# rbesenczi/newMSM

Hardware: AMD Instinct MI355X
Metric: label-cost evals/sec (higher is better)
Workload: dtype f64; 1 GPU; pairwise sulc (D=1) unary label-cost table, ico6 data grid / ico4 control grid, 19 labels, 48678 evals = 3187573 point samples per step (BASELINE config 2); kind=univariate, simmeasure=correlation, replicas=1

## Files before the change

### include/msmhip.h

```cpp
#ifndef MSMHIP_H
#define MSMHIP_H

#include <stddef.h>
#include <stdint.h>

#ifdef __cplusplus
extern "C" {
#endif

#define MSM_ABI_VERSION 11

#define MSM_OK 0
#define MSM_ERR_INVALID (-1)
#define MSM_ERR_HIP (-2)
#define MSM_ERR_OUTSIDE (-3)
#define MSM_ERR_NOTFOUND (-4)
#define MSM_ERR_NOGPU (-5)
#define MSM_ERR_STATE (-6)
#define MSM_ERR_CAPACITY (-7)
#define MSM_ERR_ROTATION (-8)

#define MSM_RAD 100.0
#define MSM_FOLDING 1e7

typedef struct msm_ctx msm_ctx;
typedef struct msm_mesh msm_mesh;
typedef struct msm_cost msm_cost;

int         msm_abi_version(void);
const char *msm_last_error(void);
int         msm_device_count(void);

int msm_icosphere_counts(int order, int32_t *V, int32_t *T);
int msm_icosphere(int order, double radius, double *xyz, int32_t *tri);
int msm_mesh_adjacency(const int32_t *tri, int32_t V, int32_t T, int32_t *nbr_ptr, int32_t *nbr, int32_t *tid_ptr, int32_t *tid);
int msm_vertex_areas(const double *xyz, const int32_t *tri, int32_t V, int32_t T, double *area);
int msm_resample_anatomy_grid(const double *cp_xyz, int32_t N, const int32_t *cp_tri, int32_t Tc, int32_t levels, double rad, int32_t *Va, int32_t *Ta,
                              double *axyz, int32_t *atri, int32_t *w_ptr, int32_t *w_cp, double *w_val, int32_t *face_ptr, int32_t *face_idx);
int msm_cp_spacings(const double *xyz, const int32_t *tri, int32_t V, int32_t T, double *maxsep, double *mvdmax);
int msm_label_sampling_grid(int sg_order, double max_dist, int abs_is_int, int32_t cap,
                            double *samples, int32_t *nsamples, double *barycentres, int32_t *nbarycentres);
int msm_rescale_sampling_grid(const double *samples, int32_t n, double *scale, double *labels);
int msm_rotation_matrix(const double ci[3], const double index[3], double R[9]);
int msm_cp_rotations(const double centre[3], const double *cp_xyz, int32_t N, double *rot);
int msm_estimate_triplets(const int32_t *tri, int32_t T, int32_t *triplets);
int msm_estimate_pairs(const int32_t *tri, int32_t V, int32_t T, int32_t *pairs);
int msm_octree_signature(const double *xyz, const int32_t *tri, int32_t V, int32_t T, int64_t stats[5], uint64_t *signature);
int msm_ray_table_check(const double *xyz, const int32_t *tri, int32_t V, int32_t T, int32_t nsamples, uint64_t seed, int64_t report[10]);

msm_ctx *msm_ctx_create(int device);
msm_ctx *msm_ctx_create_on_stream(int device, void *hip_stream);
void     msm_ctx_destroy(msm_ctx *ctx);
int      msm_ctx_synchronize(msm_ctx *ctx);
void    *msm_ctx_stream(msm_ctx *ctx);
void     msm_store_release_i64(int64_t *addr, int64_t value);
int64_t  msm_load_acquire_i64(const int64_t *addr);
int64_t  msm_min_acquire_i64(const int64_t *addr, int32_t n);
int      msm_ctx_wait_stream(msm_ctx *ctx, void *hip_stream);
int      msm_ctx_staging_stats(msm_ctx *ctx, int64_t out[4]);
int      msm_ctx_time_queries(msm_ctx *ctx, int enable);
int      msm_ctx_query_kernel_ms(msm_ctx *ctx, double *ms);
int      msm_query_lanes(int64_t n_queries);
void    *msm_host_alloc(msm_ctx *ctx, size_t bytes);
void     msm_host_free(msm_ctx *ctx, void *p);
int      msm_host_register(msm_ctx *ctx, void *p, size_t bytes);

msm_mesh *msm_mesh_create(msm_ctx *ctx, const double *xyz, int32_t V, const int32_t *tri, int32_t T);
void      msm_mesh_destroy(msm_mesh *m);
int       msm_mesh_update_coords(msm_mesh *m, const double *xyz);
int       msm_mesh_get_coords(msm_mesh *m, double *xyz);
int       msm_mesh_set_features(msm_mesh *m, const double *feat, int32_t D);
int       msm_mesh_sizes(const msm_mesh *m, int32_t *V, int32_t *T, int32_t *D);
int       msm_mesh_octree_stats(msm_mesh *m, int64_t stats[5]);
int       msm_mesh_octree_signature(msm_mesh *m, int64_t stats[5], uint64_t *signature);
int       msm_octree_forest_signatures(msm_ctx *ctx, const double *xyz, int32_t V, const int32_t *tri, int32_t T, int32_t B, uint64_t *signatures);
int       msm_mesh_prepare_search(msm_mesh *m, int wait, int32_t *ready);

#define MSM_WEIGHTS_PROJECTED 0
#define MSM_WEIGHTS_RAW 1
int msm_query_triangles(msm_mesh *target, const double *q_xyz, int32_t N, int32_t *tri_id, int32_t *v_id, double *w, int weight_mode);
int msm_closest_vertex(msm_mesh *target, const double *q_xyz, int32_t N, int32_t *v_id);
int msm_adaptive_barycentric_weights(msm_mesh *in_mesh, msm_mesh *new_mesh, const double *excl,
                                     int32_t *row_ptr, int32_t *col, double *val, int64_t cap, int64_t *nnz);
int msm_metric_resample(msm_mesh *in_mesh, const double *data, int32_t D, msm_mesh *new_mesh, const double *excl, double *out, double *excl_out);
int msm_sphere_project_warp(msm_mesh *from, const double *to_xyz, double *sphere_xyz, int32_t N);
int msm_mesh_sphere_project_warp(msm_mesh *sphere, msm_mesh *from, const double *to_xyz);
int msm_barycentric_coords_resample(msm_mesh *from, const double *coords_xyz, const double *q_xyz, int32_t N, double *out_xyz);
int msm_smooth_data(msm_mesh *orig, const double *data, int32_t D, msm_mesh *sphlow, double sigma, const double *excl, double *out, double *excl_out);
int msm_nearest_neighbour(msm_mesh *orig, const double *data, int32_t D, const double *q_xyz, int32_t N, const double *excl, double *out, double *excl_out);
int msm_create_exclusion(const double *data, int32_t D, int32_t V, double thrl, double thru, double *excl);

int msm_mesh_unfold(msm_mesh *m, double radius, int32_t *passes, int32_t *first_folded);
int msm_variance_normalise(double *data, int32_t D, int32_t V, const double *excl);
int msm_mcmc_optimise(const double *unary, const double *tcosts, const int32_t *triplets, int32_t N, int32_t L, int32_t T, double mcparam,
                      int32_t iters, uint64_t seed, int32_t *labeling);
int msm_fusion_icm_step(const double *unary2 , const double *quads , const int32_t *pairs , int32_t P,
                        const double *octets , const int32_t *triplets , int32_t T, int32_t N, int32_t max_passes,
                        int32_t *x );
int msm_pairwise_icm(const double *unary, const double *paircosts, const int32_t *pairs, int32_t N, int32_t L, int32_t P, int32_t max_passes, int32_t *labeling);

#define MSM_COST_UNIVARIATE 0
#define MSM_COST_MULTIVARIATE 1
#define MSM_COST_PATCHWISE 2
#define MSM_COST_HO_UNIVARIATE 3
#define MSM_COST_HO_MULTIVARIATE 4

typedef struct msm_cost_params {
    int32_t kind;
    int32_t simmeasure;
    int32_t rmode;
    int32_t reserved;
    double  lambda;
    double  mu;
    double  kappa;
    double  k_exp;
    double  rexp;
    double  range;
    double  percentile;
} msm_cost_params;

msm_cost *msm_cost_create(msm_ctx *ctx, const msm_cost_params *params);
void      msm_cost_destroy(msm_cost *c);
int msm_cost_set_anatomical(msm_cost *c, msm_mesh *sphere, const double *atarget_xyz, const double *asource_xyz, int32_t Vs,
                            const int32_t *asource_tri, int32_t Ts, const int32_t *w_ptr, const int32_t *w_cp, const double *w_val,
                            const int32_t *face_ptr, const int32_t *face_idx);
int msm_cost_set_meshes(msm_cost *c, msm_mesh *target, msm_mesh *source, msm_mesh *cpgrid);
int msm_cost_reset_source(msm_cost *c, msm_mesh *source);
int msm_cost_reset_cpgrid(msm_cost *c, msm_mesh *cpgrid);
int msm_cost_set_source_features(msm_cost *c, const double *feat, int32_t D);
int msm_cost_set_cfweight(msm_cost *c, const double *w, int32_t rows);
int msm_cost_set_spacings(msm_cost *c, const double *maxsep, double mvdmax);
int msm_cost_set_labels(msm_cost *c, const double *labels, int32_t L, const double *rot);
int msm_cost_set_triplets(msm_cost *c, const int32_t *triplets, int32_t T);
int msm_cost_set_pairs(msm_cost *c, const int32_t *pairs, int32_t P);
int msm_cost_get_source_data(msm_cost *c);
int msm_cost_patches(msm_cost *c, int32_t *ngroups, int32_t *ptr, int32_t *idx, int64_t cap);
int msm_cost_absolute_weights(msm_cost *c, double *absw );
int msm_cost_unary_table(msm_cost *c, double *U);
int msm_cost_unary_table_async(msm_cost *c);
int msm_cost_unary_table_fetch(msm_cost *c, double *U);
int msm_cost_unary_batch(msm_cost *c, const int32_t *nodes, const int32_t *labels, int32_t n, double *out);
int msm_cost_triplet_batch(msm_cost *c, const int32_t *triplet, const int32_t *la, const int32_t *lb, const int32_t *lc, int32_t n, double *out);
int msm_cost_triplet_octets(msm_cost *c, const int32_t *labeling, int32_t label, double *E);
int msm_cost_triplet_octets_prefetch(msm_cost *c, const int32_t *labeling, int32_t label, double *E);
int msm_cost_prefetch_stats(msm_cost *c, int64_t *taken, int64_t *dropped);
int msm_cost_pairwise_batch(msm_cost *c, const int32_t *pair, const int32_t *la, const int32_t *lb, int32_t n, double *out);
int msm_cost_pairwise_table(msm_cost *c, double *paircosts);
int msm_cost_triplet_table(msm_cost *c, int32_t t0, int32_t t1, double *tcosts);
int msm_cost_total(msm_cost *c, const int32_t *labeling, double *total, double parts[3]);
int msm_cost_enable_timing(msm_cost *c, int enable);
int msm_cost_kernel_times(msm_cost *c, double *ms, int32_t cap, int32_t *n);
int msm_cost_counters(msm_cost *c, int64_t counters[4]);

typedef struct msm_group msm_group;
typedef struct msm_group_params {
    int32_t simmeasure;
    int32_t fixnan;
    double  lambda, mu, kappa, k_exp, rexp, range;
    double  percentile;
} msm_group_params;
msm_group *msm_group_create(msm_ctx *ctx, const msm_group_params *params, int32_t num_subjects);
msm_ctx   *msm_group_context(msm_group *g);
void       msm_group_destroy(msm_group *g);
int msm_group_set_template(msm_group *g, msm_mesh *template_mesh, const double *mask);
int msm_group_set_controlgrid(msm_group *g, const double *xyz, const int32_t *tri, int32_t N, int32_t Tc);
int msm_group_set_subject(msm_group *g, int32_t subject, msm_mesh *data_mesh, const double *feat, int32_t D);
int msm_group_reset_cpgrid(msm_group *g, int32_t subject, const double *xyz);
int msm_group_set_labels(msm_group *g, const double *labels, int32_t L);
int msm_group_set_pair_layout(msm_group *g, int32_t layout);
int msm_group_set_rotation_mode(msm_group *g, int32_t mode);
int msm_group_setup(msm_group *g);
int msm_group_setup_subjects(msm_group *g, const int32_t *subjects, int32_t n);
int msm_group_export_subject(msm_group *g, int32_t subject, double *F, int32_t *pptr, int32_t *pidx, int64_t cap, int64_t *npidx);
int msm_group_import_subject(msm_group *g, int32_t subject, const double *F, const int32_t *pptr, const int32_t *pidx, int64_t npidx);
int msm_group_export_subject_dev(msm_group *g, int32_t subject, double *F_dev, int32_t *pptr_dev, int32_t *pidx_dev, int64_t cap, int64_t *npidx);
int msm_group_import_subject_dev(msm_group *g, int32_t subject, const double *F_dev, const int32_t *pptr_dev, const int32_t *pidx_dev, int64_t npidx);
int msm_group_export_subjects_dev(msm_group *g, const int32_t *subjects, int32_t n, double *F_dev, int64_t F_stride, int32_t *pptr_dev, int64_t pptr_stride,
                                  int32_t *pidx_dev, int64_t pidx_stride, int64_t *npidx);
int msm_group_import_subjects_dev(msm_group *g, const int32_t *subjects, int32_t n, const double *F_dev, int64_t F_stride, const int32_t *pptr_dev,
                                  int64_t pptr_stride, const int32_t *pidx_dev, int64_t pidx_stride, const int64_t *npidx);
int msm_group_setup_more_subjects(msm_group *g, const int32_t *subjects, int32_t n);
int msm_group_finalize(msm_group *g);
int msm_group_sizes(msm_group *g, int32_t *nodes, int32_t *pairs, int32_t *triplets);
int msm_group_dims(msm_group *g, int32_t *S, int32_t *N, int32_t *L, int32_t *D, int32_t *Vt);
int msm_group_get_pairs(msm_group *g, int32_t *pairs );
int msm_group_get_triplets(msm_group *g, int32_t *triplets );
int msm_group_patch(msm_group *g, int32_t subject, int32_t cp, int32_t label, int32_t *ids, double *data, int32_t cap, int32_t *n);
int msm_group_pairwise_batch(msm_group *g, const int32_t *pair, const int32_t *la, const int32_t *lb, int32_t n, double *out);
int msm_group_triplet_batch(msm_group *g, const int32_t *triplet, const int32_t *la, const int32_t *lb, const int32_t *lc, int32_t n, double *out);
int msm_group_fusion_move(msm_group *g, const int32_t *labeling, int32_t label, double *pair_quads, double *triplet_octets);

int msm_group_fusion_move_dev(msm_group *g, const int32_t *labeling, int32_t label, int64_t pair0, int64_t pair1, int64_t trip0, int64_t trip1,
                              double *quads_dev, double *octets_dev);
int msm_group_time_moves(msm_group *g, int enable);
int msm_group_move_kernels_ms(msm_group *g, double *ms);


typedef struct msm_rigid msm_rigid;

msm_rigid *msm_rigid_create(msm_ctx *ctx, msm_mesh *target, msm_mesh *source, const double *in_feat, const double *ref_feat, int32_t D,
                            int32_t simmeasure);
void msm_rigid_destroy(msm_rigid *r);
int msm_rigid_set_source(msm_rigid *r, const double *xyz);
int msm_rigid_get_source(msm_rigid *r, double *xyz);
int msm_rigid_cost(msm_rigid *r, const double *euler, int32_t n, double *sums, double *per_vertex);
int msm_rigid_rotate(msm_rigid *r, const double euler[3]);
int msm_rigid_run(msm_rigid *r, int32_t iters, double stepsize, double gradsampling, double *trace, int32_t cap, int32_t *n, double summary[3]);
int msm_rigid_kernel_ms(msm_rigid *r, double ms[2]);

int msm_calculate_strains(msm_mesh *orig, const double *final_xyz, int32_t V, double fit_radius, double *strains, int32_t *kept, double *radius);

typedef struct msm_dedrift msm_dedrift;
msm_dedrift *msm_dedrift_create(msm_ctx *ctx, msm_mesh *template_mesh, int32_t num_subjects);
void msm_dedrift_destroy(msm_dedrift *d);
int msm_dedrift_reset(msm_dedrift *d);
int msm_dedrift_accumulate(msm_dedrift *d, msm_mesh *reg, const double *orig_xyz, int32_t V, int32_t *tri_id, double *w, double *inverse_xyz);
int msm_dedrift_finish(msm_dedrift *d, double *warp_xyz, double *drift_xyz);
int msm_dedrift_correct(msm_dedrift *d, int32_t subject, msm_mesh *reg, const double *orig_xyz, int32_t V, const double *data, int32_t D,
                        double *corrected_xyz, double *resampled, double *distortion, int32_t *tri_id, double *w);
int msm_dedrift_set_map(msm_dedrift *d, int32_t subject, const double *map, int32_t D);
int msm_dedrift_group_stats(msm_dedrift *d, double percentile, double *mean, double *stdev, double *cc, double *dice);

#ifdef __cplusplus
}
#endif
#endif
```

### newmsm_amd/_lib.py

```python
import ctypes as C
import os

_HERE = os.path.dirname(os.path.abspath(__file__))
LIB_PATH = os.environ.get("MSM_LIB_PATH") or os.path.join(_HERE, "libmsmhip.so")

c_dp = C.POINTER(C.c_double)
c_ip = C.POINTER(C.c_int32)
c_lp = C.POINTER(C.c_int64)

MSM_OK = 0
ERR_NAMES = {-1: "MSM_ERR_INVALID", -2: "MSM_ERR_HIP", -3: "MSM_ERR_OUTSIDE", -4: "MSM_ERR_NOTFOUND", -5: "MSM_ERR_NOGPU",
             -6: "MSM_ERR_STATE", -7: "MSM_ERR_CAPACITY", -8: "MSM_ERR_ROTATION"}


class MsmError(RuntimeError):

    def __init__(self, code, message):
        super().__init__("%s (%d): %s" % (ERR_NAMES.get(code, "MSM_ERR"), code, message))
        self.code = code


class GroupParams(C.Structure):
    _fields_ = [("simmeasure", C.c_int32), ("fixnan", C.c_int32), ("lambda_", C.c_double), ("mu", C.c_double),
                ("kappa", C.c_double), ("k_exp", C.c_double), ("rexp", C.c_double), ("range", C.c_double), ("percentile", C.c_double)]


class CostParams(C.Structure):
    _fields_ = [("kind", C.c_int32), ("simmeasure", C.c_int32), ("rmode", C.c_int32), ("reserved", C.c_int32),
                ("lambda_", C.c_double), ("mu", C.c_double), ("kappa", C.c_double), ("k_exp", C.c_double),
                ("rexp", C.c_double), ("range", C.c_double), ("percentile", C.c_double)]


_VP = C.c_void_p
SIGNATURES = {
    "msm_abi_version": (C.c_int, []),
    "msm_last_error": (C.c_char_p, []),
    "msm_device_count": (C.c_int, []),
    "msm_icosphere_counts": (C.c_int, [C.c_int, c_ip, c_ip]),
    "msm_icosphere": (C.c_int, [C.c_int, C.c_double, c_dp, c_ip]),
    "msm_mesh_adjacency": (C.c_int, [c_ip, C.c_int32, C.c_int32, c_ip, c_ip, c_ip, c_ip]),
    "msm_vertex_areas": (C.c_int, [c_dp, c_ip, C.c_int32, C.c_int32, c_dp]),
    "msm_resample_anatomy_grid": (C.c_int, [c_dp, C.c_int32, c_ip, C.c_int32, C.c_int32, C.c_double, c_ip, c_ip, c_dp, c_ip, c_ip, c_ip, c_dp, c_ip, c_ip]),
    "msm_cp_spacings": (C.c_int, [c_dp, c_ip, C.c_int32, C.c_int32, c_dp, c_dp]),
    "msm_label_sampling_grid": (C.c_int, [C.c_int, C.c_double, C.c_int, C.c_int32, c_dp, c_ip, c_dp, c_ip]),
    "msm_rescale_sampling_grid": (C.c_int, [c_dp, C.c_int32, c_dp, c_dp]),
    "msm_rotation_matrix": (C.c_int, [c_dp, c_dp, c_dp]),
    "msm_cp_rotations": (C.c_int, [c_dp, c_dp, C.c_int32, c_dp]),
    "msm_estimate_triplets": (C.c_int, [c_ip, C.c_int32, c_ip]),
    "msm_estimate_pairs": (C.c_int, [c_ip, C.c_int32, C.c_int32, c_ip]),
    "msm_octree_signature": (C.c_int, [c_dp, c_ip, C.c_int32, C.c_int32, C.POINTER(C.c_int64), C.POINTER(C.c_uint64)]),
    "msm_ray_table_check": (C.c_int, [c_dp, c_ip, C.c_int32, C.c_int32, C.c_int32, C.c_uint64, C.POINTER(C.c_int64)]),
    "msm_ctx_create": (_VP, [C.c_int]),
    "msm_ctx_create_on_stream": (_VP, [C.c_int, _VP]),
    "msm_ctx_destroy": (None, [_VP]),
    "msm_ctx_synchronize": (C.c_int, [_VP]),
    "msm_ctx_stream": (_VP, [_VP]),
    "msm_store_release_i64": (None, [_VP, C.c_int64]),
    "msm_load_acquire_i64": (C.c_int64, [_VP]),
    "msm_min_acquire_i64": (C.c_int64, [_VP, C.c_int32]),
    "msm_ctx_time_queries": (C.c_int, [_VP, C.c_int]),
    "msm_ctx_query_kernel_ms": (C.c_int, [_VP, c_dp]),
    "msm_query_lanes": (C.c_int, [C.c_int64]),
    "msm_group_context": (_VP, [_VP]),
    "msm_ctx_wait_stream": (C.c_int, [_VP, _VP]),
    "msm_ctx_staging_stats": (C.c_int, [_VP, C.POINTER(C.c_int64)]),
    "msm_host_alloc": (_VP, [_VP, C.c_size_t]),
    "msm_host_free": (None, [_VP, _VP]),
    "msm_host_register": (C.c_int, [_VP, _VP, C.c_size_t]),
    "msm_mesh_create": (_VP, [_VP, c_dp, C.c_int32, c_ip, C.c_int32]),
    "msm_mesh_destroy": (None, [_VP]),
    "msm_mesh_update_coords": (C.c_int, [_VP, c_dp]),
    "msm_mesh_get_coords": (C.c_int, [_VP, c_dp]),
    "msm_mesh_set_features": (C.c_int, [_VP, c_dp, C.c_int32]),
    "msm_mesh_sizes": (C.c_int, [_VP, c_ip, c_ip, c_ip]),
    "msm_mesh_octree_stats": (C.c_int, [_VP, c_lp]),
    "msm_mesh_octree_signature": (C.c_int, [_VP, c_lp, C.POINTER(C.c_uint64)]),
    "msm_octree_forest_signatures": (C.c_int, [_VP, c_dp, C.c_int32, c_ip, C.c_int32, C.c_int32, C.POINTER(C.c_uint64)]),
    "msm_query_triangles": (C.c_int, [_VP, c_dp, C.c_int32, c_ip, c_ip, c_dp, C.c_int]),
    "msm_closest_vertex": (C.c_int, [_VP, c_dp, C.c_int32, c_ip]),
    "msm_adaptive_barycentric_weights": (C.c_int, [_VP, _VP, c_dp, c_ip, c_ip, c_dp, C.c_int64, c_lp]),
    "msm_metric_resample": (C.c_int, [_VP, c_dp, C.c_int32, _VP, c_dp, c_dp, c_dp]),
    "msm_create_exclusion": (C.c_int, [c_dp, C.c_int32, C.c_int32, C.c_double, C.c_double, c_dp]),
    "msm_sphere_project_warp": (C.c_int, [_VP, c_dp, c_dp, C.c_int32]),
    "msm_mesh_sphere_project_warp": (C.c_int, [_VP, _VP, c_dp]),
    "msm_barycentric_coords_resample": (C.c_int, [_VP, c_dp, c_dp, C.c_int32, c_dp]),
    "msm_smooth_data": (C.c_int, [_VP, c_dp, C.c_int32, _VP, C.c_double, c_dp, c_dp, c_dp]),
    "msm_mesh_unfold": (C.c_int, [_VP, C.c_double, c_ip, c_ip]),
    "msm_mesh_prepare_search": (C.c_int, [_VP, C.c_int, c_ip]),
    "msm_variance_normalise": (C.c_int, [c_dp, C.c_int32, C.c_int32, c_dp]),
    "msm_mcmc_optimise": (C.c_int, [c_dp, c_dp, c_ip, C.c_int32, C.c_int32, C.c_int32, C.c_double, C.c_int32, C.c_uint64, c_ip]),
    "msm_fusion_icm_step": (C.c_int, [c_dp, c_dp, c_ip, C.c_int32, c_dp, c_ip, C.c_int32, C.c_int32, C.c_int32, c_ip]),
    "msm_pairwise_icm": (C.c_int, [c_dp, c_dp, c_ip, C.c_int32, C.c_int32, C.c_int32, C.c_int32, c_ip]),
    "msm_nearest_neighbour": (C.c_int, [_VP, c_dp, C.c_int32, c_dp, C.c_int32, c_dp, c_dp, c_dp]),
    "msm_cost_create": (_VP, [_VP, C.POINTER(CostParams)]),
    "msm_cost_destroy": (None, [_VP]),
    "msm_cost_set_meshes": (C.c_int, [_VP, _VP, _VP, _VP]),
    "msm_cost_set_anatomical": (C.c_int, [_VP, _VP, c_dp, c_dp, C.c_int32, c_ip, C.c_int32, c_ip, c_ip, c_dp, c_ip, c_ip]),
    "msm_cost_reset_source": (C.c_int, [_VP, _VP]),
    "msm_cost_reset_cpgrid": (C.c_int, [_VP, _VP]),
    "msm_cost_set_source_features": (C.c_int, [_VP, c_dp, C.c_int32]),
    "msm_cost_set_cfweight": (C.c_int, [_VP, c_dp, C.c_int32]),
    "msm_cost_set_spacings": (C.c_int, [_VP, c_dp, C.c_double]),
    "msm_cost_set_labels": (C.c_int, [_VP, c_dp, C.c_int32, c_dp]),
    "msm_cost_set_triplets": (C.c_int, [_VP, c_ip, C.c_int32]),
    "msm_cost_set_pairs": (C.c_int, [_VP, c_ip, C.c_int32]),
    "msm_cost_get_source_data": (C.c_int, [_VP]),
    "msm_cost_patches": (C.c_int, [_VP, c_ip, c_ip, c_ip, C.c_int64]),
    "msm_cost_absolute_weights": (C.c_int, [_VP, c_dp]),
    "msm_cost_unary_table": (C.c_int, [_VP, c_dp]),
    "msm_cost_unary_table_async": (C.c_int, [_VP]),
    "msm_cost_unary_table_fetch": (C.c_int, [_VP, c_dp]),
    "msm_cost_unary_batch": (C.c_int, [_VP, c_ip, c_ip, C.c_int32, c_dp]),
    "msm_cost_triplet_batch": (C.c_int, [_VP, c_ip, c_ip, c_ip, c_ip, C.c_int32, c_dp]),
    "msm_cost_triplet_octets_prefetch": (C.c_int, [_VP, _VP, C.c_int32, _VP]),
    "msm_cost_prefetch_stats": (C.c_int, [_VP, C.POINTER(C.c_int64), C.POINTER(C.c_int64)]),
    "msm_cost_triplet_octets": (C.c_int, [_VP, _VP, C.c_int32, _VP]),
    "msm_cost_pairwise_batch": (C.c_int, [_VP, c_ip, c_ip, c_ip, C.c_int32, c_dp]),
    "msm_cost_pairwise_table": (C.c_int, [_VP, c_dp]),
    "msm_cost_triplet_table": (C.c_int, [_VP, C.c_int32, C.c_int32, c_dp]),
    "msm_cost_total": (C.c_int, [_VP, c_ip, c_dp, c_dp]),
    "msm_cost_enable_timing": (C.c_int, [_VP, C.c_int]),
    "msm_cost_kernel_times": (C.c_int, [_VP, c_dp, C.c_int32, c_ip]),
    "msm_cost_counters": (C.c_int, [_VP, c_lp]),
    "msm_group_create": (_VP, [_VP, C.POINTER(GroupParams), C.c_int32]),
    "msm_group_fusion_move": (C.c_int, [_VP, c_ip, C.c_int32, c_dp, c_dp]),
    "msm_group_destroy": (None, [_VP]),
    "msm_group_time_moves": (C.c_int, [_VP, C.c_int]),
    "msm_group_move_kernels_ms": (C.c_int, [_VP, c_dp]),
    "msm_group_set_template": (C.c_int, [_VP, _VP, c_dp]),
    "msm_group_set_controlgrid": (C.c_int, [_VP, c_dp, c_ip, C.c_int32, C.c_int32]),
    "msm_group_set_subject": (C.c_int, [_VP, C.c_int32, _VP, c_dp, C.c_int32]),
    "msm_group_reset_cpgrid": (C.c_int, [_VP, C.c_int32, c_dp]),
    "msm_group_set_labels": (C.c_int, [_VP, c_dp, C.c_int32]),
    "msm_group_set_pair_layout": (C.c_int, [_VP, C.c_int32]),
    "msm_group_set_rotation_mode": (C.c_int, [_VP, C.c_int32]),
    "msm_group_setup": (C.c_int, [_VP]),
    "msm_group_setup_subjects": (C.c_int, [_VP, c_ip, C.c_int32]),
    "msm_group_export_subject": (C.c_int, [_VP, C.c_int32, c_dp, c_ip, c_ip, C.c_int64, c_lp]),
    "msm_group_import_subject": (C.c_int, [_VP, C.c_int32, c_dp, c_ip, c_ip, C.c_int64]),
    "msm_group_export_subject_dev": (C.c_int, [_VP, C.c_int32, _VP, _VP, _VP, C.c_int64, c_lp]),
    "msm_group_import_subject_dev": (C.c_int, [_VP, C.c_int32, _VP, _VP, _VP, C.c_int64]),
    "msm_group_export_subjects_dev": (C.c_int, [_VP, c_ip, C.c_int32, _VP, C.c_int64, _VP, C.c_int64, _VP, C.c_int64, C.POINTER(C.c_int64)]),
    "msm_group_import_subjects_dev": (C.c_int, [_VP, c_ip, C.c_int32, _VP, C.c_int64, _VP, C.c_int64, _VP, C.c_int64, C.POINTER(C.c_int64)]),
    "msm_group_setup_more_subjects": (C.c_int, [_VP, c_ip, C.c_int32]),
    "msm_group_fusion_move_dev": (C.c_int, [_VP, c_ip, C.c_int32, C.c_int64, C.c_int64, C.c_int64, C.c_int64, _VP, _VP]),
    "msm_group_finalize": (C.c_int, [_VP]),
    "msm_group_sizes": (C.c_int, [_VP, c_ip, c_ip, c_ip]),
    "msm_group_dims": (C.c_int, [_VP, c_ip, c_ip, c_ip, c_ip, c_ip]),
    "msm_group_get_pairs": (C.c_int, [_VP, c_ip]),
    "msm_group_get_triplets": (C.c_int, [_VP, c_ip]),
    "msm_group_patch": (C.c_int, [_VP, C.c_int32, C.c_int32, C.c_int32, c_ip, c_dp, C.c_int32, c_ip]),
    "msm_group_pairwise_batch": (C.c_int, [_VP, c_ip, c_ip, c_ip, C.c_int32, c_dp]),
    "msm_group_triplet_batch": (C.c_int, [_VP, c_ip, c_ip, c_ip, c_ip, C.c_int32, c_dp]),
    "msm_rigid_create": (_VP, [_VP, _VP, _VP, c_dp, c_dp, C.c_int32, C.c_int32]),
    "msm_rigid_destroy": (None, [_VP]),
    "msm_rigid_set_source": (C.c_int, [_VP, c_dp]),
    "msm_rigid_get_source": (C.c_int, [_VP, c_dp]),
    "msm_rigid_cost": (C.c_int, [_VP, c_dp, C.c_int32, c_dp, c_dp]),
    "msm_rigid_rotate": (C.c_int, [_VP, c_dp]),
    "msm_rigid_run": (C.c_int, [_VP, C.c_int32, C.c_double, C.c_double, c_dp, C.c_int32, c_ip, c_dp]),
    "msm_rigid_kernel_ms": (C.c_int, [_VP, c_dp]),
    "msm_calculate_strains": (C.c_int, [_VP, c_dp, C.c_int32, C.c_double, c_dp, c_ip, c_dp]),
    "msm_dedrift_create": (_VP, [_VP, _VP, C.c_int32]),
    "msm_dedrift_destroy": (None, [_VP]),
    "msm_dedrift_reset": (C.c_int, [_VP]),
    "msm_dedrift_accumulate": (C.c_int, [_VP, _VP, c_dp, C.c_int32, c_ip, c_dp, c_dp]),
    "msm_dedrift_finish": (C.c_int, [_VP, c_dp, c_dp]),
    "msm_dedrift_correct": (C.c_int, [_VP, C.c_int32, _VP, c_dp, C.c_int32, c_dp, C.c_int32, c_dp, c_dp, c_dp, c_ip, c_dp]),
    "msm_dedrift_set_map": (C.c_int, [_VP, C.c_int32, c_dp, C.c_int32]),
    "msm_dedrift_group_stats": (C.c_int, [_VP, C.c_double, c_dp, c_dp, c_dp, c_dp]),
}

_lib = None


def lib():
    global _lib
    if _lib is None:
        if not os.path.exists(LIB_PATH):
            raise ImportError("newmsm_amd: %s is missing -- run `python -c 'import __graft_entry__ as g; g.build()'` "
                              "(hipcc --offload-arch=gfx950). There is no fallback path." % LIB_PATH)
        L = C.CDLL(LIB_PATH)
        for name, (res, args) in SIGNATURES.items():
            fn = getattr(L, name)
            fn.restype = res
            fn.argtypes = args
        _lib = L
    return _lib


def check(status):
    if status != MSM_OK:
        raise MsmError(status, lib().msm_last_error().decode("utf-8", "replace"))
    return status
```

### newmsm_amd/api.py

```python
import ctypes as C

import numpy as np

from ._lib import CostParams, MsmError, c_dp, c_ip, c_lp, check, lib

WEIGHTS_PROJECTED = 0
WEIGHTS_RAW = 1
KINDS = dict(univariate=0, multivariate=1, patchwise=2, ho_univariate=3, ho_multivariate=4)


def _soa(points):
    a = np.ascontiguousarray(np.asarray(points, dtype=np.float64).reshape(-1, 3).T)
    return a, a.ctypes.data_as(c_dp)


def _aos(soa, n):
    return np.ascontiguousarray(np.asarray(soa).reshape(3, n).T)


def _tri_soa(tri):
    a = np.ascontiguousarray(np.asarray(tri, dtype=np.int32).reshape(-1, 3).T)
    return a, a.ctypes.data_as(c_ip)


def _d(a):
    a = np.ascontiguousarray(a, dtype=np.float64)
    return a, a.ctypes.data_as(c_dp)


def _i(a):
    a = np.ascontiguousarray(a, dtype=np.int32)
    return a, a.ctypes.data_as(c_ip)


def device_count():
    return lib().msm_device_count()


def icosphere_counts(order):
    v, t = C.c_int32(), C.c_int32()
    check(lib().msm_icosphere_counts(order, C.byref(v), C.byref(t)))
    return v.value, t.value


def make_mesh_from_icosa(order, radius=100.0):
    V, T = icosphere_counts(order)
    xyz = np.zeros((3, V))
    tri = np.zeros((3, T), dtype=np.int32)
    check(lib().msm_icosphere(order, float(radius if radius else 0.0), xyz.ctypes.data_as(c_dp), tri.ctypes.data_as(c_ip)))
    return np.ascontiguousarray(xyz.T), np.ascontiguousarray(tri.T)


def mesh_adjacency(tri, V):
    t, pt = _tri_soa(tri)
    T = t.shape[1]
    nbr_ptr = np.zeros(V + 1, dtype=np.int32)
    tid_ptr = np.zeros(V + 1, dtype=np.int32)
    check(lib().msm_mesh_adjacency(pt, V, T, nbr_ptr.ctypes.data_as(c_ip), None, tid_ptr.ctypes.data_as(c_ip), None))
    nbr = np.zeros(nbr_ptr[-1], dtype=np.int32)
    tid = np.zeros(tid_ptr[-1], dtype=np.int32)
    check(lib().msm_mesh_adjacency(pt, V, T, nbr_ptr.ctypes.data_as(c_ip), nbr.ctypes.data_as(c_ip), tid_ptr.ctypes.data_as(c_ip),
                                   tid.ctypes.data_as(c_ip)))
    return nbr_ptr, nbr, tid_ptr, tid


def vertex_areas(xyz, tri):
    x, px = _soa(xyz)
    t, pt = _tri_soa(tri)
    out = np.zeros(x.shape[1])
    check(lib().msm_vertex_areas(px, pt, x.shape[1], t.shape[1], out.ctypes.data_as(c_dp)))
    return out


def cp_spacings(xyz, tri):
    x, px = _soa(xyz)
    t, pt = _tri_soa(tri)
    ms = np.zeros(x.shape[1])
    mvd = C.c_double()
    check(lib().msm_cp_spacings(px, pt, x.shape[1], t.shape[1], ms.ctypes.data_as(c_dp), C.byref(mvd)))
    return ms, mvd.value


def label_sampling_grid(sg_order, max_dist, abs_is_int=False, cap=4096):
    s = np.zeros((3, cap))
    b = np.zeros((3, cap))
    ns, nb = C.c_int32(), C.c_int32()
    check(lib().msm_label_sampling_grid(sg_order, float(max_dist), int(abs_is_int), cap, s.ctypes.data_as(c_dp), C.byref(ns),
                                        b.ctypes.data_as(c_dp), C.byref(nb)))
    return np.ascontiguousarray(s[:, : ns.value].T), np.ascontiguousarray(b[:, : nb.value].T)


def rescale_sampling_grid(samples, scale):
    s, ps = _soa(samples)
    n = s.shape[1]
    out = np.zeros((3, n))
    sc = C.c_double(scale)
    check(lib().msm_rescale_sampling_grid(ps, n, C.byref(sc), out.ctypes.data_as(c_dp)))
    return np.ascontiguousarray(out.T), sc.value


def estimate_rotation_matrix(ci, index):
    R = np.zeros(9)
    check(lib().msm_rotation_matrix(_d(ci)[1], _d(index)[1], R.ctypes.data_as(c_dp)))
    return R.reshape(3, 3)


def cp_rotations(centre, cp_xyz):
    x, px = _soa(cp_xyz)
    rot = np.zeros((x.shape[1], 9))
    check(lib().msm_cp_rotations(_d(centre)[1], px, x.shape[1], rot.ctypes.data_as(c_dp)))
    return rot


def octree_signature(xyz, tri):
    x, px = _soa(xyz)
    t, pt = _tri_soa(tri)
    stats = (C.c_int64 * 5)()
    sig = C.c_uint64(0)
    check(lib().msm_octree_signature(px, pt, x.shape[1], t.shape[1], stats, C.byref(sig)))
    return dict(nodes=stats[0], leaves=stats[1], depth=stats[2], refs=stats[3], max_leaf=stats[4]), sig.value


def ray_table_check(xyz, tri, nsamples=20000, seed=1):
    x, px = _soa(xyz)
    t, pt = _tri_soa(tri)
    rep = (C.c_int64 * 10)()
    check(lib().msm_ray_table_check(px, pt, x.shape[1], t.shape[1], nsamples, seed, rep))
    return dict(points=rep[0], by_float=rep[1], by_fp64=rep[2], open=rep[3], violations=rep[4], unusable=rep[5], with_exclusions=rep[6], simple=bool(rep[7]), boxes_checked=rep[8], refused_by_boxes=rep[9])


def estimate_triplets(tri):
    t, pt = _tri_soa(tri)
    out = np.zeros((t.shape[1], 3), dtype=np.int32)
    check(lib().msm_estimate_triplets(pt, t.shape[1], out.ctypes.data_as(c_ip)))
    return out


def estimate_pairs(tri, V):
    t, pt = _tri_soa(tri)
    n = lib().msm_estimate_pairs(pt, V, t.shape[1], None)
    if n < 0:
        check(n)
    out = np.zeros((n, 2), dtype=np.int32)
    lib().msm_estimate_pairs(pt, V, t.shape[1], out.ctypes.data_as(c_ip))
    return out


class Context:

    def __init__(self, device=0, stream=None):
        L = lib()
        self.h = L.msm_ctx_create(device) if stream is None else L.msm_ctx_create_on_stream(device, C.c_void_p(stream))
        if not self.h:
            raise MsmError(-5, L.msm_last_error().decode())
        self.device = device

    def synchronize(self):
        check(lib().msm_ctx_synchronize(self.h))

    @property
    def stream(self):
        return lib().msm_ctx_stream(self.h)

    def wait_stream(self, hip_stream=None):
        check(lib().msm_ctx_wait_stream(self.h, C.c_void_p(hip_stream or 0)))

    def staging_stats(self):
        out = (C.c_int64 * 4)()
        check(lib().msm_ctx_staging_stats(self.h, out))
        return dict(blocks=int(out[0]), bytes=int(out[1]), allocated=int(out[2]), waits=int(out[3]))

    def host_array(self, shape, dtype=np.float64):
        n = int(np.prod(shape)) * np.dtype(dtype).itemsize
        p = lib().msm_host_alloc(self.h, max(n, 8))
        if not p:
            raise MsmError(-2, lib().msm_last_error().decode())
        buf = (C.c_char * max(n, 8)).from_address(p)
        return np.frombuffer(buf, dtype=dtype, count=int(np.prod(shape))).reshape(shape)

    def scratch_host_array(self, name, shape, dtype=np.float64):
        n = int(np.prod(shape)) * np.dtype(dtype).itemsize
        bufs = self.__dict__.setdefault("_scratch_pinned", {})
        cur = bufs.get(name)
        if cur is None or cur[1] < n:
            cap = max(2 * n, 4096) if cur is not None else max(n + n // 8, 4096)
            p = lib().msm_host_alloc(self.h, cap)
            if not p:
                raise MsmError(-2, lib().msm_last_error().decode())
            cur = bufs[name] = (p, cap)
        buf = (C.c_char * cur[1]).from_address(cur[0])
        return np.frombuffer(buf, dtype=dtype, count=int(np.prod(shape))).reshape(shape)

    def release_host_array(self, arr):
        if getattr(self, "h", None):
            lib().msm_host_free(self.h, C.c_void_p(arr.ctypes.data))

    def time_queries(self, on=True):
        check(lib().msm_ctx_time_queries(self.h, int(on)))

    def query_kernel_ms(self):
        ms = C.c_double(-1.0)
        check(lib().msm_ctx_query_kernel_ms(self.h, C.byref(ms)))
        return ms.value

    @staticmethod
    def query_lanes(n_queries):
        return int(lib().msm_query_lanes(int(n_queries)))

    def forest_signatures(self, xyz_sets, tri):
        sets = [np.ascontiguousarray(np.asarray(x, dtype=np.float64).T) for x in xyz_sets]
        big = np.ascontiguousarray(np.stack(sets))
        t, pt = _tri_soa(tri)
        sig = (C.c_uint64 * len(sets))()
        check(lib().msm_octree_forest_signatures(self.h, big.ctypes.data_as(c_dp), big.shape[2], pt, t.shape[1], len(sets), sig))
        return [int(v) for v in sig]

    def register_host(self, address, nbytes):
        check(lib().msm_host_register(self.h, C.c_void_p(address), nbytes))

    def unregister_host(self, address):
        lib().msm_host_free(self.h, C.c_void_p(address))

    def close(self):
        if getattr(self, "h", None):
            lib().msm_ctx_destroy(self.h)
            self.h = None

    def __del__(self):
        self.close()


class Mesh:

    def __init__(self, ctx, xyz, tri):
        self.ctx = ctx
        x, px = _soa(xyz)
        t, pt = _tri_soa(tri)
        self.V, self.T = x.shape[1], t.shape[1]
        self.tri = np.ascontiguousarray(t.T)
        self.h = lib().msm_mesh_create(ctx.h, px, self.V, pt, self.T)
        if not self.h:
            raise MsmError(-1, lib().msm_last_error().decode())

    def close(self):
        if getattr(self, "h", None) and getattr(self.ctx, "h", None):
            lib().msm_mesh_destroy(self.h)
        self.h = None

    def __del__(self):
        self.close()

    def set_coords(self, xyz):
        check(lib().msm_mesh_update_coords(self.h, _soa(xyz)[1]))

    def get_coords(self):
        out = np.zeros((3, self.V))
        check(lib().msm_mesh_get_coords(self.h, out.ctypes.data_as(c_dp)))
        return np.ascontiguousarray(out.T)

    def prepare_search(self, wait=True):
        ready = C.c_int32()
        check(lib().msm_mesh_prepare_search(self.h, int(bool(wait)), C.byref(ready)))
        return bool(ready.value)

    def unfold(self, radius=100.0):
        passes, first = C.c_int32(), C.c_int32()
        check(lib().msm_mesh_unfold(self.h, float(radius), C.byref(passes), C.byref(first)))
        return passes.value, first.value

    def set_pvalues(self, feat):
        f, pf = _d(np.atleast_2d(feat))
        assert f.shape[1] == self.V
        check(lib().msm_mesh_set_features(self.h, pf, f.shape[0]))

    def octree_stats(self):
        s = (C.c_int64 * 5)()
        check(lib().msm_mesh_octree_stats(self.h, s))
        return dict(nodes=s[0], leaves=s[1], depth=s[2], refs=s[3], max_leaf=s[4])

    def octree_signature(self):
        s = (C.c_int64 * 5)()
        sig = C.c_uint64()
        check(lib().msm_mesh_octree_signature(self.h, s, C.byref(sig)))
        return dict(nodes=s[0], leaves=s[1], depth=s[2], refs=s[3], max_leaf=s[4]), sig.value

    def query_triangles_soa(self, q_soa, tri, vid, w, mode=WEIGHTS_PROJECTED):
        N = q_soa.shape[1]
        assert q_soa.flags.c_contiguous and tri.flags.c_contiguous and vid.flags.c_contiguous and w.flags.c_contiguous and q_soa.dtype == np.float64
        assert tri.shape == (N,) and vid.shape == (3, N) and w.shape == (3, N) and tri.dtype == np.int32 and vid.dtype == np.int32 and w.dtype == np.float64
        return lib().msm_query_triangles(self.h, q_soa.ctypes.data_as(c_dp), N, tri.ctypes.data_as(c_ip), vid.ctypes.data_as(c_ip), w.ctypes.data_as(c_dp), mode)

    def query_triangles(self, q, mode=WEIGHTS_PROJECTED, check_status=True):
        x, px = _soa(q)
        N = x.shape[1]
        tri = np.zeros(N, dtype=np.int32)
        vid = np.zeros((3, N), dtype=np.int32)
        w = np.zeros((3, N))
        st = lib().msm_query_triangles(self.h, px, N, tri.ctypes.data_as(c_ip), vid.ctypes.data_as(c_ip), w.ctypes.data_as(c_dp), mode)
        if check_status:
            check(st)
        return st, tri, np.ascontiguousarray(vid.T), np.ascontiguousarray(w.T)

    def get_closest_vertex_ID(self, q):
        x, px = _soa(q)
        out = np.zeros(x.shape[1], dtype=np.int32)
        check(lib().msm_closest_vertex(self.h, px, x.shape[1], out.ctypes.data_as(c_ip)))
        return out


def get_adaptive_barycentric_weights(in_mesh, new_mesh, excl=None):
    nnz = C.c_int64()
    pe = _d(excl)[1] if excl is not None else None
    check(lib().msm_adaptive_barycentric_weights(in_mesh.h, new_mesh.h, pe, None, None, None, 0, C.byref(nnz)))
    rp = np.zeros(new_mesh.V + 1, dtype=np.int32)
    col = np.zeros(nnz.value, dtype=np.int32)
    val = np.zeros(nnz.value)
    check(lib().msm_adaptive_barycentric_weights(in_mesh.h, new_mesh.h, pe, rp.ctypes.data_as(c_ip), col.ctypes.data_as(c_ip),
                                                 val.ctypes.data_as(c_dp), nnz.value, C.byref(nnz)))
    return rp, col, val


def metric_resample(in_mesh, data, new_mesh, excl=None, out=None):
    d, pd = _d(np.atleast_2d(data))
    if out is None:
        out = np.zeros((d.shape[0], new_mesh.V))
    assert out.shape == (d.shape[0], new_mesh.V) and out.flags.c_contiguous and out.dtype == np.float64
    if excl is None:
        check(lib().msm_metric_resample(in_mesh.h, pd, d.shape[0], new_mesh.h, None, out.ctypes.data_as(c_dp), None))
        return out
    eo = np.zeros(new_mesh.V)
    check(lib().msm_metric_resample(in_mesh.h, pd, d.shape[0], new_mesh.h, _d(excl)[1], out.ctypes.data_as(c_dp), eo.ctypes.data_as(c_dp)))
    return out, eo


def create_exclusion(data, thrl, thru):
    d, pd = _d(np.atleast_2d(data))
    out = np.zeros(d.shape[1])
    check(lib().msm_create_exclusion(pd, d.shape[0], d.shape[1], float(thrl), float(thru), out.ctypes.data_as(c_dp)))
    return out


def sphere_project_warp(sphere, from_mesh, to_xyz):
    s, ps = _soa(sphere)
    s = s.copy()
    check(lib().msm_sphere_project_warp(from_mesh.h, _soa(to_xyz)[1], s.ctypes.data_as(c_dp), s.shape[1]))
    return np.ascontiguousarray(s.T)


def sphere_project_warp_mesh(sphere_mesh, from_mesh, to_xyz):
    check(lib().msm_mesh_sphere_project_warp(sphere_mesh.h, from_mesh.h, _soa(to_xyz)[1]))


def resample_anatomy_grid(cp_xyz, cp_tri, levels, rad=100.0):
    x, px = _soa(cp_xyz)
    t, pt = _tri_soa(cp_tri)
    N, Tc = x.shape[1], t.shape[1]
    va, ta = C.c_int32(), C.c_int32()
    check(lib().msm_resample_anatomy_grid(px, N, pt, Tc, int(levels), float(rad), C.byref(va), C.byref(ta), None, None, None, None, None, None, None))
    Va, Ta = va.value, ta.value
    axyz, atri = np.zeros((3, Va)), np.zeros((3, Ta), dtype=np.int32)
    w_ptr, w_cp, w_val = np.zeros(Va + 1, dtype=np.int32), np.zeros(3 * Va, dtype=np.int32), np.zeros(3 * Va)
    face_ptr, face_idx = np.zeros(Tc + 1, dtype=np.int32), np.zeros(Ta, dtype=np.int32)
    check(lib().msm_resample_anatomy_grid(px, N, pt, Tc, int(levels), float(rad), C.byref(va), C.byref(ta), axyz.ctypes.data_as(c_dp), atri.ctypes.data_as(c_ip),
                                          w_ptr.ctypes.data_as(c_ip), w_cp.ctypes.data_as(c_ip), w_val.ctypes.data_as(c_dp), face_ptr.ctypes.data_as(c_ip),
                                          face_idx.ctypes.data_as(c_ip)))
    n = int(w_ptr[-1])
    return dict(sphere_xyz=np.ascontiguousarray(axyz.T), sphere_tri=np.ascontiguousarray(atri.T), w_ptr=w_ptr, w_cp=w_cp[:n].copy(), w_val=w_val[:n].copy(),
                face_ptr=face_ptr, face_idx=face_idx)


def barycentric_coords_resample(from_mesh, coords, q):
    x, px = _soa(q)
    out = np.zeros((3, x.shape[1]))
    check(lib().msm_barycentric_coords_resample(from_mesh.h, _soa(coords)[1], px, x.shape[1], out.ctypes.data_as(c_dp)))
    return np.ascontiguousarray(out.T)


def project_anatomical_mesh(sphere_mesh, target_mesh, anat_xyz):
    anat = np.asarray(anat_xyz, dtype=np.float64).reshape(-1, 3)
    coords = anat if len(anat) == target_mesh.V else target_mesh.get_coords()
    return barycentric_coords_resample(target_mesh, coords, sphere_mesh.get_coords())


def calculate_strains(orig_mesh, final_xyz, fit_radius=2.0, with_neighbourhoods=False):
    x, px = _soa(final_xyz)
    V = x.shape[1]
    strains = np.zeros((4, V))
    kept = np.zeros(V, dtype=np.int32)
    radius = np.zeros(V)
    check(lib().msm_calculate_strains(orig_mesh.h, px, V, float(fit_radius), strains.ctypes.data_as(c_dp), kept.ctypes.data_as(c_ip),
                                      radius.ctypes.data_as(c_dp)))
    return (strains, kept, radius) if with_neighbourhoods else strains


def smooth_data(orig_mesh, data, sph_low, sigma, excl=None):
    d, pd = _d(np.atleast_2d(data))
    assert d.shape[1] == orig_mesh.V
    out = np.zeros((d.shape[0], sph_low.V))
    if excl is None:
        check(lib().msm_smooth_data(orig_mesh.h, pd, d.shape[0], sph_low.h, float(sigma), None, out.ctypes.data_as(c_dp), None))
        return out
    e, pe = _d(excl)
    eo = np.zeros(sph_low.V)
    check(lib().msm_smooth_data(orig_mesh.h, pd, d.shape[0], sph_low.h, float(sigma), pe, out.ctypes.data_as(c_dp), eo.ctypes.data_as(c_dp)))
    return out, eo


def variance_normalise(data, excl=None):
    out = np.array(np.atleast_2d(data), dtype=np.float64, order="C")
    pe = _d(excl)[1] if excl is not None else None
    check(lib().msm_variance_normalise(out.ctypes.data_as(c_dp), out.shape[0], out.shape[1], pe))
    return out


def mcmc_optimise(unary, tcosts, triplets, labeling, mcparam=0.8, iters=100, seed=0):
    U, pu = _d(unary)
    L, N = U.shape
    tc, ptc = _d(tcosts)
    tr = np.ascontiguousarray(triplets, dtype=np.int32)
    T = tr.shape[0]
    assert tc.size == T * L ** 3
    lab = np.array(labeling, dtype=np.int32)
    check(lib().msm_mcmc_optimise(pu, ptc, tr.ctypes.data_as(c_ip), N, L, T, float(mcparam), int(iters), int(seed), lab.ctypes.data_as(c_ip)))
    return lab


def fusion_icm_step(unary2, octets, triplets, passes=5, quads=None, pairs=None):
    if np.ndim(unary2) == 0:
        N, u, pu = int(unary2), None, None
    else:
        u = np.ascontiguousarray(unary2, dtype=np.float64)
        N, pu = u.shape[0], u.ctypes.data_as(c_dp)
        assert u.shape == (N, 2)
    tr = np.ascontiguousarray(triplets if triplets is not None else np.zeros((0, 3)), dtype=np.int32)
    e = np.ascontiguousarray(octets if octets is not None else np.zeros((0, 8)), dtype=np.float64)
    pr = np.ascontiguousarray(pairs if pairs is not None else np.zeros((0, 2)), dtype=np.int32)
    q = np.ascontiguousarray(quads if quads is not None else np.zeros((0, 4)), dtype=np.float64)
    T, P = tr.shape[0], pr.shape[0]
    assert e.size == 8 * T and q.size == 4 * P
    x = np.zeros(N, dtype=np.int32)
    check(lib().msm_fusion_icm_step(pu, q.ctypes.data_as(c_dp), pr.ctypes.data_as(c_ip), P, e.ctypes.data_as(c_dp), tr.ctypes.data_as(c_ip), T, N, int(passes),
                                    x.ctypes.data_as(c_ip)))
    return x


def pairwise_icm(unary, paircosts, pairs, labeling=None, passes=100):
    u = np.ascontiguousarray(unary, dtype=np.float64)
    L, N = u.shape
    pr = np.ascontiguousarray(pairs, dtype=np.int32).reshape(-1, 2)
    pc = np.ascontiguousarray(paircosts, dtype=np.float64)
    assert pc.size == pr.shape[0] * L * L
    lab = np.zeros(N, dtype=np.int32) if labeling is None else np.array(labeling, dtype=np.int32)
    check(lib().msm_pairwise_icm(u.ctypes.data_as(c_dp), pc.ctypes.data_as(c_dp), pr.ctypes.data_as(c_ip), N, L, pr.shape[0], int(passes), lab.ctypes.data_as(c_ip)))
    return lab


def nearest_neighbour_interpolation(orig_mesh, data, q, excl=None):
    d, pd = _d(np.atleast_2d(data))
    x, px = _soa(q)
    out = np.zeros((d.shape[0], x.shape[1]))
    if excl is None:
        check(lib().msm_nearest_neighbour(orig_mesh.h, pd, d.shape[0], px, x.shape[1], None, out.ctypes.data_as(c_dp), None))
        return out
    eo = np.zeros(x.shape[1])
    check(lib().msm_nearest_neighbour(orig_mesh.h, pd, d.shape[0], px, x.shape[1], _d(excl)[1], out.ctypes.data_as(c_dp), eo.ctypes.data_as(c_dp)))
    return out, eo


class DiscreteCostFunction:

    def __init__(self, ctx, kind="univariate", simmeasure=2, rmode=3, lambda_=0.1, mu=0.1, kappa=10.0, k_exp=2.0, rexp=2.0, range_=1.0,
                 percentile=0.75):
        self.ctx = ctx
        self.params = CostParams(KINDS[kind], simmeasure, rmode, 0, lambda_, mu, kappa, k_exp, rexp, range_, percentile)
        self.h = lib().msm_cost_create(ctx.h, C.byref(self.params))
        if not self.h:
            raise MsmError(-1, lib().msm_last_error().decode())
        self._keep = {}

    def close(self):
        if getattr(self, "h", None) and getattr(self.ctx, "h", None):
            lib().msm_cost_destroy(self.h)
        self.h = None

    def __del__(self):
        self.close()

    def set_meshes(self, target, source, cpgrid):
        self._keep.update(target=target, source=source, cpgrid=cpgrid)
        self.N = cpgrid.V
        check(lib().msm_cost_set_meshes(self.h, target.h, source.h, cpgrid.h))

    def set_anatomical(self, sphere, atarget_xyz, asource_xyz, asource_tri, w_ptr, w_cp, w_val, face_ptr, face_idx):
        at, pat = _soa(atarget_xyz)
        asx, pas = _soa(asource_xyz)
        tri, ptri = _tri_soa(asource_tri)
        wp, pwp = _i(w_ptr)
        wc, pwc = _i(w_cp)
        wv, pwv = _d(w_val)
        fp, pfp = _i(face_ptr)
        fi, pfi = _i(face_idx)
        assert at.shape[1] == sphere.V
        self._keep.update(asphere=sphere)
        check(lib().msm_cost_set_anatomical(self.h, sphere.h, pat, pas, asx.shape[1], ptri, tri.shape[1], pwp, pwc, pwv, pfp, pfi))

    def reset_source(self, source):
        self._keep["source"] = source
        check(lib().msm_cost_reset_source(self.h, source.h))

    def reset_CPgrid(self, cpgrid):
        self._keep["cpgrid"] = cpgrid
        check(lib().msm_cost_reset_cpgrid(self.h, cpgrid.h))

    def set_featurespace(self, src_feat, ref_feat=None):
        f, pf = _d(np.atleast_2d(src_feat))
        if ref_feat is not None:
            self._keep["target"].set_pvalues(ref_feat)
        check(lib().msm_cost_set_source_features(self.h, pf, f.shape[0]))

    def set_dataaffintyweighting(self, w):
        if w is None:
            check(lib().msm_cost_set_cfweight(self.h, None, 0))
        else:
            w, pw = _d(np.atleast_2d(w))
            check(lib().msm_cost_set_cfweight(self.h, pw, w.shape[0]))

    def set_spacings(self, maxsep, mvdmax):
        check(lib().msm_cost_set_spacings(self.h, _d(maxsep)[1], float(mvdmax)))

    def set_labels(self, labels, rot):
        l, pl = _soa(labels)
        self.L = l.shape[1]
        check(lib().msm_cost_set_labels(self.h, pl, self.L, _d(rot)[1]))

    def setTriplets(self, triplets):
        t, pt = _i(triplets)
        self.T = len(t)
        check(lib().msm_cost_set_triplets(self.h, pt, self.T))

    def setPairs(self, pairs):
        p, pp = _i(pairs)
        self.P = len(p)
        check(lib().msm_cost_set_pairs(self.h, pp, self.P))

    def get_source_data(self):
        check(lib().msm_cost_get_source_data(self.h))

    def patches(self):
        ng = C.c_int32()
        check(lib().msm_cost_patches(self.h, C.byref(ng), None, None, 0))
        ptr = np.zeros(ng.value + 1, dtype=np.int32)
        check(lib().msm_cost_patches(self.h, C.byref(ng), ptr.ctypes.data_as(c_ip), None, 0))
        idx = np.zeros(max(int(ptr[-1]), 1), dtype=np.int32)
        check(lib().msm_cost_patches(self.h, C.byref(ng), ptr.ctypes.data_as(c_ip), idx.ctypes.data_as(c_ip), len(idx)))
        return ptr, idx[: int(ptr[-1])]

    def absolute_weights(self):
        out = np.zeros(self.N)
        check(lib().msm_cost_absolute_weights(self.h, out.ctypes.data_as(c_dp)))
        return out

    def computeUnaryCosts(self, out=None):
        U = np.zeros((self.L, self.N)) if out is None else out
        assert U.shape == (self.L, self.N) and U.dtype == np.float64 and U.flags.c_contiguous
        check(lib().msm_cost_unary_table(self.h, U.ctypes.data_as(c_dp)))
        return U

    def computeUnaryCosts_async(self):
        check(lib().msm_cost_unary_table_async(self.h))

    def getUnaryCosts(self):
        U = np.zeros((self.L, self.N))
        check(lib().msm_cost_unary_table_fetch(self.h, U.ctypes.data_as(c_dp)))
        return U

    def computeUnaryCost(self, nodes, labels):
        n, pn = _i(np.atleast_1d(nodes))
        l, pl = _i(np.atleast_1d(labels))
        out = np.zeros(len(n))
        check(lib().msm_cost_unary_batch(self.h, pn, pl, len(n), out.ctypes.data_as(c_dp)))
        return out

    def computeTripletCost(self, triplet, la, lb, lc):
        t, pt = _i(np.atleast_1d(triplet))
        a, pa = _i(np.atleast_1d(la))
        b, pb = _i(np.atleast_1d(lb))
        c_, pc = _i(np.atleast_1d(lc))
        out = np.zeros(len(t))
        check(lib().msm_cost_triplet_batch(self.h, pt, pa, pb, pc, len(t), out.ctypes.data_as(c_dp)))
        return out

    def tripletOctets(self, labeling, label, out=None):
        lab = labeling if (type(labeling) is np.ndarray and labeling.dtype == np.int32 and labeling.flags.c_contiguous) else np.ascontiguousarray(labeling, dtype=np.int32)
        assert lab.shape == (self.N,)
        if out is None:
            out = np.zeros((self.T, 8))
        assert out.shape == (self.T, 8) and out.dtype == np.float64 and out.flags.c_contiguous
        st = lib().msm_cost_triplet_octets(self.h, lab.ctypes.data, int(label), out.ctypes.data)
        if st:
            check(st)
        return out

    def prefetchTripletOctets(self, labeling, label, out):
        lab = labeling if (type(labeling) is np.ndarray and labeling.dtype == np.int32 and labeling.flags.c_contiguous) else np.ascontiguousarray(labeling, dtype=np.int32)
        st = lib().msm_cost_triplet_octets_prefetch(self.h, lab.ctypes.data, int(label), out.ctypes.data)
        if st:
            check(st)

    def prefetch_stats(self):
        a, b = C.c_int64(), C.c_int64()
        check(lib().msm_cost_prefetch_stats(self.h, C.byref(a), C.byref(b)))
        return a.value, b.value

    def computeTripletCosts(self, t0=0, t1=None, pinned=False):
        t1 = self.T if t1 is None else t1
        shape = (t1 - t0, self.L, self.L, self.L)
        if pinned:
            out = self.ctx.scratch_host_array("tcosts", shape)
        else:
            out = self._keep.get("tcosts")
            if out is None or out.shape != shape:
                out = self._keep["tcosts"] = np.empty(shape)
        check(lib().msm_cost_triplet_table(self.h, int(t0), int(t1), out.ctypes.data_as(c_dp)))
        return out

    def computePairwiseCost(self, pair, la, lb):
        p, pp = _i(np.atleast_1d(pair))
        a, pa = _i(np.atleast_1d(la))
        b, pb = _i(np.atleast_1d(lb))
        out = np.zeros(len(p))
        check(lib().msm_cost_pairwise_batch(self.h, pp, pa, pb, len(p), out.ctypes.data_as(c_dp)))
        return out

    def computePairwiseCosts(self):
        out = np.zeros(self.P * self.L * self.L)
        check(lib().msm_cost_pairwise_table(self.h, out.ctypes.data_as(c_dp)))
        return out

    def evaluateTotalCostSum(self, labeling):
        lab, pl = _i(labeling)
        tot = C.c_double()
        parts = np.zeros(3)
        check(lib().msm_cost_total(self.h, pl, C.byref(tot), parts.ctypes.data_as(c_dp)))
        return tot.value, parts

    def enable_timing(self, on=True):
        check(lib().msm_cost_enable_timing(self.h, int(on)))

    def kernel_times(self):
        ms = np.zeros(64)
        n = C.c_int32()
        check(lib().msm_cost_kernel_times(self.h, ms.ctypes.data_as(c_dp), 64, C.byref(n)))
        return ms[: n.value].copy()

    def counters(self):
        c = (C.c_int64 * 4)()
        check(lib().msm_cost_counters(self.h, c))
        return dict(samples=c[0], unary=c[1], triplet=c[2], pairwise=c[3])


class DiscreteGroupCostFunction:

    def __init__(self, ctx, num_subjects, simmeasure=2, fixnan=False, lambda_=0.1, mu=0.1, kappa=10.0, k_exp=2.0, rexp=2.0, range_=1.0,
                 percentile=0.75):
        from ._lib import GroupParams

        self.ctx = ctx
        self.S = num_subjects
        self.params = GroupParams(simmeasure, int(fixnan), lambda_, mu, kappa, k_exp, rexp, range_, percentile)
        self.h = lib().msm_group_create(ctx.h, C.byref(self.params), num_subjects)
        if not self.h:
            raise MsmError(-1, lib().msm_last_error().decode())
        self._keep = {}

    def close(self):
        if getattr(self, "h", None) and getattr(self.ctx, "h", None):
            lib().msm_group_destroy(self.h)
        self.h = None

    def __del__(self):
        self.close()

    def set_template(self, mesh, mask=None):
        self._keep["template"] = mesh
        check(lib().msm_group_set_template(self.h, mesh.h, _d(mask)[1] if mask is not None else None))

    def Initialize(self, cp_xyz, cp_tri):
        x, px = _soa(cp_xyz)
        t, pt = _tri_soa(cp_tri)
        self.N, self.Tc = x.shape[1], t.shape[1]
        check(lib().msm_group_set_controlgrid(self.h, px, pt, self.N, self.Tc))

    def reset_meshspace(self, subject, data_mesh, feat):
        f, pf = _d(np.atleast_2d(feat))
        self._keep[("data", subject)] = data_mesh
        self.D = f.shape[0]
        check(lib().msm_group_set_subject(self.h, subject, data_mesh.h, pf, f.shape[0]))

    def reset_CPgrid(self, subject, cp_xyz):
        check(lib().msm_group_reset_cpgrid(self.h, subject, _soa(cp_xyz)[1]))

    def set_labels(self, labels):
        l, pl = _soa(labels)
        self.L = l.shape[1]
        check(lib().msm_group_set_labels(self.h, pl, self.L))

    REFERENCE_ORDER, CP_MAJOR = 0, 1
    DEVICE_ROTATIONS, HOST_ROTATIONS = 0, 1

    def set_rotation_mode(self, mode):
        check(lib().msm_group_set_rotation_mode(self.h, int(mode)))

    def set_pair_layout(self, layout):
        check(lib().msm_group_set_pair_layout(self.h, int(layout)))

    def setupCostFunction(self):
        check(lib().msm_group_setup(self.h))
        n, p, t = C.c_int32(), C.c_int32(), C.c_int32()
        check(lib().msm_group_sizes(self.h, C.byref(n), C.byref(p), C.byref(t)))
        self.num_nodes, self.P, self.T = n.value, p.value, t.value

    def setup_subjects(self, subjects):
        s, ps = _i(np.asarray(list(subjects), dtype=np.int32))
        check(lib().msm_group_setup_subjects(self.h, ps, len(s)))

    def setup_more_subjects(self, subjects):
        s, ps = _i(np.asarray(list(subjects), dtype=np.int32))
        check(lib().msm_group_setup_more_subjects(self.h, ps, len(s)))

    def export_subject(self, subject):
        n = C.c_int64()
        check(lib().msm_group_export_subject(self.h, int(subject), None, None, None, 0, C.byref(n)))
        Vt = self._keep["template"].V
        F = np.zeros((self.L, self.D, Vt))
        pptr = np.zeros(self.N * self.L + 1, dtype=np.int32)
        pidx = np.zeros(max(n.value, 1), dtype=np.int32)
        check(lib().msm_group_export_subject(self.h, int(subject), F.ctypes.data_as(c_dp), pptr.ctypes.data_as(c_ip), pidx.ctypes.data_as(c_ip),
                                             len(pidx), C.byref(n)))
        return F, pptr, pidx[: n.value]

    def import_subject(self, subject, F, pptr, pidx):
        F, pF = _d(F)
        pp, ppp = _i(pptr)
        pi, ppi = _i(pidx)
        check(lib().msm_group_import_subject(self.h, int(subject), pF, ppp, ppi if len(pi) else None, len(pi)))

    def subject_index_count(self, subject):
        n = C.c_int64()
        check(lib().msm_group_export_subject_dev(self.h, int(subject), None, None, None, 0, C.byref(n)))
        return n.value

    def export_subject_dev(self, subject, F_ptr, pptr_ptr, pidx_ptr, cap):
        n = C.c_int64()
        check(lib().msm_group_export_subject_dev(self.h, int(subject), C.c_void_p(F_ptr), C.c_void_p(pptr_ptr), C.c_void_p(pidx_ptr), int(cap), C.byref(n)))
        return n.value

    def import_subject_dev(self, subject, F_ptr, pptr_ptr, pidx_ptr, npidx):
        check(lib().msm_group_import_subject_dev(self.h, int(subject), C.c_void_p(F_ptr), C.c_void_p(pptr_ptr), C.c_void_p(pidx_ptr), int(npidx)))

    def export_subjects_dev(self, subjects, F_ptr, F_stride, pptr_ptr, pptr_stride, pidx_ptr, pidx_stride):
        s, ps = _i(np.asarray(list(subjects), dtype=np.int32))
        n = np.zeros(max(len(s), 1), dtype=np.int64)
        check(lib().msm_group_export_subjects_dev(self.h, ps, len(s), C.c_void_p(F_ptr), int(F_stride), C.c_void_p(pptr_ptr), int(pptr_stride),
                                                  C.c_void_p(pidx_ptr), int(pidx_stride), n.ctypes.data_as(C.POINTER(C.c_int64))))
        return n[: len(s)]

    def import_subjects_dev(self, subjects, F_ptr, F_stride, pptr_ptr, pptr_stride, pidx_ptr, pidx_stride, npidx):
        s, ps = _i(np.asarray(list(subjects), dtype=np.int32))
        n = np.ascontiguousarray(np.asarray(npidx, dtype=np.int64))
        assert len(n) == len(s)
        check(lib().msm_group_import_subjects_dev(self.h, ps, len(s), C.c_void_p(F_ptr), int(F_stride), C.c_void_p(pptr_ptr), int(pptr_stride),
                                                  C.c_void_p(pidx_ptr), int(pidx_stride), n.ctypes.data_as(C.POINTER(C.c_int64))))

    def fusionMove_dev(self, labeling, label, pair_range, triplet_range, quads_ptr, octets_ptr):
        lab, pl = _i(labeling)
        check(lib().msm_group_fusion_move_dev(self.h, pl, int(label), int(pair_range[0]), int(pair_range[1]), int(triplet_range[0]), int(triplet_range[1]),
                                              C.c_void_p(quads_ptr), C.c_void_p(octets_ptr)))

    def time_moves(self, on=True):
        check(lib().msm_group_time_moves(self.h, int(on)))

    def move_kernels_ms(self):
        ms = C.c_double(-1.0)
        check(lib().msm_group_move_kernels_ms(self.h, C.byref(ms)))
        return ms.value

    def finalize(self):
        check(lib().msm_group_finalize(self.h))
        n, p, t = C.c_int32(), C.c_int32(), C.c_int32()
        check(lib().msm_group_sizes(self.h, C.byref(n), C.byref(p), C.byref(t)))
        self.num_nodes, self.P, self.T = n.value, p.value, t.value

    def getPairs(self):
        out = np.zeros((self.P, 2), dtype=np.int32)
        check(lib().msm_group_get_pairs(self.h, out.ctypes.data_as(c_ip)))
        return out

    def fusionMove(self, labeling, label, out=None):
        lab, pl = _i(labeling)
        quads, octets = (np.zeros((self.P, 4)), np.zeros((self.T, 8))) if out is None else out
        assert quads.shape == (self.P, 4) and octets.shape == (self.T, 8) and quads.dtype == octets.dtype == np.float64
        assert quads.flags.c_contiguous and octets.flags.c_contiguous
        check(lib().msm_group_fusion_move(self.h, pl, int(label), quads.ctypes.data_as(c_dp), octets.ctypes.data_as(c_dp)))
        return quads, octets

    def getTriplets(self):
        out = np.zeros((self.T, 3), dtype=np.int32)
        check(lib().msm_group_get_triplets(self.h, out.ctypes.data_as(c_ip)))
        return out

    def patch(self, subject, cp, label):
        subject, cp, label = int(subject), int(cp), int(label)
        n = C.c_int32()
        check(lib().msm_group_patch(self.h, subject, cp, label, None, None, 0, C.byref(n)))
        ids = np.zeros(n.value, dtype=np.int32)
        data = np.zeros((n.value, self.D))
        check(lib().msm_group_patch(self.h, subject, cp, label, ids.ctypes.data_as(c_ip), data.ctypes.data_as(c_dp), n.value, C.byref(n)))
        return ids, data

    def computePairwiseCost(self, pair, la, lb):
        p, pp = _i(np.atleast_1d(pair))
        a, pa = _i(np.atleast_1d(la))
        b, pb = _i(np.atleast_1d(lb))
        out = np.zeros(len(p))
        check(lib().msm_group_pairwise_batch(self.h, pp, pa, pb, len(p), out.ctypes.data_as(c_dp)))
        return out

    def computeTripletCost(self, t, la, lb, lc):
        t_, pt = _i(np.atleast_1d(t))
        a, pa = _i(np.atleast_1d(la))
        b, pb = _i(np.atleast_1d(lb))
        c_, pc = _i(np.atleast_1d(lc))
        out = np.zeros(len(t_))
        check(lib().msm_group_triplet_batch(self.h, pt, pa, pb, pc, len(t_), out.ctypes.data_as(c_dp)))
        return out


def rigid_loops(gradsampling):
    n, spacing = 0, float(gradsampling)
    while spacing > 0.05:
        n, spacing = n + 1, spacing * 0.5
    return n


class RigidCostFunction:

    def __init__(self, ctx, target, source, in_feat, ref_feat, simmeasure=1):
        self.ctx, self.target, self.source = ctx, target, source
        self.in_feat = np.ascontiguousarray(np.atleast_2d(in_feat), dtype=np.float64)
        self.ref_feat = np.ascontiguousarray(np.atleast_2d(ref_feat), dtype=np.float64)
        if self.in_feat.shape != (self.ref_feat.shape[0], source.V) or self.ref_feat.shape[1] != target.V:
            raise ValueError("RigidCostFunction: features must be D x V of the source and of the target")
        self.simmeasure = int(simmeasure)
        self.V = source.V
        self.h = None

    def initialise(self):
        self.close()
        self.h = lib().msm_rigid_create(self.ctx.h, self.target.h, self.source.h, self.in_feat.ctypes.data_as(c_dp),
                                        self.ref_feat.ctypes.data_as(c_dp), self.in_feat.shape[0], self.simmeasure)
        if not self.h:
            raise MsmError(-1, lib().msm_last_error().decode())
        return self

    def close(self):
        if getattr(self, "h", None) and getattr(self.ctx, "h", None):
            lib().msm_rigid_destroy(self.h)
        self.h = None

    def __del__(self):
        self.close()

    def update_source(self, xyz):
        check(lib().msm_rigid_set_source(self.h, _soa(xyz)[1]))

    def get_source(self):
        out = np.zeros((3, self.V))
        check(lib().msm_rigid_get_source(self.h, out.ctypes.data_as(c_dp)))
        return np.ascontiguousarray(out.T)

    def cost(self, euler, per_vertex=False):
        e, pe = _d(np.atleast_2d(euler))
        n = e.shape[0]
        sums = np.zeros(n)
        pv = np.zeros((n, self.V)) if per_vertex else None
        check(lib().msm_rigid_cost(self.h, pe, n, sums.ctypes.data_as(c_dp), pv.ctypes.data_as(c_dp) if pv is not None else None))
        return (sums, pv) if per_vertex else sums

    def rotate(self, euler):
        check(lib().msm_rigid_rotate(self.h, _d(np.asarray(euler, dtype=np.float64).reshape(3))[1]))

    def run(self, iters=20, stepsize=0.01, gradsampling=0.5):
        cap = max(1, rigid_loops(gradsampling) * int(iters))
        trace = np.zeros((cap, 6))
        n = C.c_int32()
        summary = np.zeros(3)
        check(lib().msm_rigid_run(self.h, int(iters), float(stepsize), float(gradsampling), trace.ctypes.data_as(c_dp), cap, C.byref(n),
                                  summary.ctypes.data_as(c_dp)))
        return self.get_source(), trace[: n.value].copy(), dict(RECinit=summary[0], RECfinal=summary[1], evaluations=int(summary[2]))

    def kernel_ms(self):
        ms = np.zeros(2)
        check(lib().msm_rigid_kernel_ms(self.h, ms.ctypes.data_as(c_dp)))
        return float(ms[0]), int(ms[1])
```

### newmsm_amd/csrc/cost.cpp

```cpp
#include <algorithm>
#include <chrono>
#include <cmath>
#include <cstdio>
#include <cstdlib>
#include <cstring>

#include "cost_internal.hpp"
#include "host_parallel.hpp"

using namespace msm;

namespace msm {
int ensure_vertex_major(msm_cost *c) {
    if (c->vm_valid) return MSM_OK;
    msm_ctx *ctx = c->ctx;
    const int Ns = c->source->V, D = c->D, R = c->cfw_rows;
    std::vector<double> vm((size_t)Ns * D);
    for (int d = 0; d < D; ++d)
        for (int v = 0; v < Ns; ++v) vm[(size_t)v * D + d] = c->sfeat[(size_t)d * Ns + v];
    MSM_HIP(c->d_sfeat_vm.ensure(vm.size()));
    {
        const int st = upload_staged(ctx, c->d_sfeat_vm.p, vm.data(), sizeof(double) * vm.size());
        if (st) return st;
    }
    if (!c->cfw.empty()) {
        std::vector<double> wm((size_t)Ns * R);
        for (int r = 0; r < R; ++r)
            for (int v = 0; v < Ns; ++v) wm[(size_t)v * R + r] = c->cfw[(size_t)r * Ns + v];
        MSM_HIP(c->d_cfw_vm.ensure(wm.size()));
        const int st = upload_staged(ctx, c->d_cfw_vm.p, wm.data(), sizeof(double) * wm.size());
        if (st) return st;
    }
    MSM_TRY(ctx_sync(ctx));
    c->vm_valid = true;
    return MSM_OK;
}

int ensure_label_rotations(msm_cost *c) {
    if (c->rotations_valid) return MSM_OK;
    if (c->L <= 0 || !c->cpgrid) return fail(MSM_ERR_STATE, "msm_cost: labels must be set first");
    const int N = c->cpgrid->V;
    MSM_HIP(c->d_rnl.ensure((size_t)N * c->L * 9));
    MSM_HIP(c->d_moved.ensure((size_t)N * c->L * 3));
    int st = launch_label_rotations(c->ctx, c->cpgrid->d_xyz.p, N, c->d_rot.p, c->d_labels.p, c->L, c->d_rnl.p, c->d_moved.p);
    if (st) return st;
    c->rotations_valid = true;
    return MSM_OK;
}
}

namespace {

void invalidate_table(msm_cost *c) {
    (void)drop_pending_move(c);
    c->move_valid = false;
    c->table_valid = false;
    c->rotations_valid = false;
    c->h_U.clear();
}

bool is_ho(const msm_cost *c) { return cost_is_ho(c); }

int need(const msm_cost *c, bool cond, const char *what) {
    if (!cond) return fail(MSM_ERR_STATE, "msm_cost: %s must be set first", what);
    return MSM_OK;
}

inline double cfw_at(const msm_cost *c, int row, int i) { return c->cfw.empty() ? 1.0 : c->cfw[(size_t)row * c->source->V + i]; }
inline int cfw_nrows(const msm_cost *c) { return c->cfw.empty() ? 1 : c->cfw_rows; }

int patches_by_range(msm_cost *c) {
    msm_ctx *ctx = c->ctx;
    const int N = c->cpgrid->V, Ns = c->source->V;
    MSM_TRY(c->d_maxsep.upload(c->maxsep.data(), N, ctx));
    MSM_HIP(c->d_counts.ensure((size_t)N + 1));
    MSM_HIP(c->d_chunkb.ensure((size_t)(Ns + 63) / 64 + 1));
    int cap = std::max(128, c->patch_cap_hint);
    std::vector<int> counts((size_t)N + 1);
    std::vector<uint32_t> slots;
    c->pidx_asc_on_device = false;
    for (int attempt = 0; attempt < 3; ++attempt) {
        MSM_HIP(c->d_slots.ensure((size_t)N * cap));
        int st = launch_range(ctx, c->cpgrid->d_xyz.p, N, c->source->d_xyz.p, Ns, c->d_maxsep.p, c->p.range, cap, c->d_slots.p, c->d_counts.p, c->d_chunkb.p,
                              c->d_counts.p + N);
        if (st) return st;
        MSM_TRY(c->d_counts.download(counts.data(), (size_t)N + 1, ctx));
        MSM_TRY(ctx_sync(ctx));
        const int mx = *std::max_element(counts.begin(), counts.begin() + N);
        c->patch_cap_hint = std::max(c->patch_cap_hint, mx + 16);
        if (mx <= cap) break;
        if (attempt == 2) return fail(MSM_ERR_CAPACITY, "patch capacity");
        cap = mx + 16;
    }
    if (counts[N] == 0) {
        c->pptr.assign((size_t)N + 1, 0);
        for (int k = 0; k < N; ++k) c->pptr[k + 1] = c->pptr[k] + counts[k];
        const size_t total = (size_t)c->pptr[N];
        MSM_TRY(c->d_pptr.upload(c->pptr.data(), c->pptr.size(), ctx));
        MSM_HIP(c->d_pidx_asc.ensure(std::max<size_t>(total, 1)));
        int st = launch_patch_compact(ctx, c->d_slots.p, cap, c->d_pptr.p, N, c->d_pidx_asc.p);
        if (st) return st;
        c->pidx.resize(total);
        if (total) MSM_TRY(c->d_pidx_asc.download(c->pidx.data(), total, ctx));
        MSM_TRY(ctx_sync(ctx));
        c->pidx_asc_on_device = true;
        c->ngroups = N;
        return MSM_OK;
    }
    slots.resize((size_t)N * cap);
    MSM_TRY(c->d_slots.download(slots.data(), slots.size(), ctx));
    MSM_TRY(ctx_sync(ctx));
    const double *cp = c->cpgrid->xyz.data(), *src = c->source->xyz.data();
    c->pptr.assign(N + 1, 0);
    c->pidx.clear();
    for (int k = 0; k < N; ++k) {
        c->pptr[k] = (int32_t)c->pidx.size();
        const V3 ck = mk(cp[k], cp[N + k], cp[2 * N + k]);
        for (int j = 0; j < counts[k]; ++j) {
            const uint32_t e = slots[(size_t)k * cap + j];
            const int i = (int)(e & 0x7fffffffu);
            if (e & 0x80000000u) {
                const double arc = chord_to_arc(norm(sub(ck, mk(src[i], src[Ns + i], src[2 * Ns + i]))));
                if (!(arc < c->p.range * c->maxsep[k])) continue;
            }
            c->pidx.push_back(i);
        }
    }
    c->pptr[N] = (int32_t)c->pidx.size();
    c->ngroups = N;
    return MSM_OK;
}

int patches_by_triangle(msm_cost *c) {
    const int Ns = c->source->V, Tc = c->cpgrid->T;
    std::vector<int> tri(Ns);
    int st = mesh_tree_on_gpu(c->cpgrid) ? MSM_OK : ensure_tree_begin(c->source);
    if (st) return st;
    st = query_host(c->cpgrid, c->source->xyz.data(), Ns, tri.data(), nullptr, nullptr, MSM_WEIGHTS_RAW, "get_source_data (HO)",
                    c->source->ctx == c->cpgrid->ctx ? c->source->d_xyz.p : nullptr);
    if (st) return st;
    if (mesh_tree_on_gpu(c->cpgrid)) {
        st = ensure_tree_begin(c->source);
        if (st) return st;
    }
    c->pptr.assign(Tc + 1, 0);
    for (int i = 0; i < Ns; ++i) c->pptr[tri[i] + 1]++;
    for (int t = 0; t < Tc; ++t) c->pptr[t + 1] += c->pptr[t];
    c->pidx.resize(Ns);
    std::vector<int32_t> fill(c->pptr.begin(), c->pptr.end() - 1);
    for (int i = 0; i < Ns; ++i) c->pidx[fill[tri[i]]++] = i;
    c->ngroups = Tc;
    return MSM_OK;
}

int resample_weights(msm_cost *c) {
    const int Ns = c->source->V, N = c->cpgrid->V;
    std::vector<double> mw(Ns);
    for (int k = 0; k < Ns; ++k) {
        double best = -DBL_MAX;
        for (int j = 0; j < cfw_nrows(c); ++j)
            if (cfw_at(c, j, k) > best) best = cfw_at(c, j, k);
        mw[k] = best;
    }
    msm_ctx *ctx = c->ctx;
    AdaptiveDev w;
    int st = adaptive_weights_dev(c->source, c->cpgrid, w);
    if (st) return st;
    MSM_HIP(c->d_maxw.ensure(Ns));
    MSM_HIP(c->d_absw.ensure(N));
    st = upload_staged(ctx, c->d_maxw.p, mw.data(), sizeof(double) * (size_t)Ns);
    if (st) return st;
    st = apply_weights_dev(ctx, w, c->d_maxw.p, 1, c->d_absw.p);
    if (st) return st;
    c->absw.resize(N);
    MSM_TRY(stage_d2h(ctx, c->absw.data(), c->d_absw.p, sizeof(double) * (size_t)N));
    MSM_TRY(ctx_sync(ctx));
    return MSM_OK;
}

int ensure_unary_table(msm_cost *c) {
    if (c->table_valid) return MSM_OK;
    int st = need(c, c->have_source, "get_source_data()");
    if (st) return st;
    st = need(c, c->L > 0, "labels");
    if (st) return st;
    st = need(c, c->target->d_feat.p != nullptr && c->target->D == c->D, "target features matching the source features");
    if (st) return st;
    msm_ctx *ctx = c->ctx;
    const int N = c->cpgrid->V;
    MSM_HIP(c->d_U.ensure((size_t)c->L * N));
    if (is_ho(c)) {
        MSM_HIP(hipMemsetAsync(c->d_U.p, 0, sizeof(double) * (size_t)c->L * N, ctx->stream));
        c->table_valid = true;
        return MSM_OK;
    }
    st = ensure_rays(c->target);
    if (st) return st;
    UnaryLaunch u;
    u.tree = dev_tree(c->target);
    u.tfeat = c->target->d_feat.p;
    u.D = c->D;
    u.N = N;
    u.L = c->L;
    u.cp = c->cpgrid->d_xyz.p;
    st = ensure_label_rotations(c);
    if (st) return st;
    u.rnl = c->d_rnl.p;
    u.labels = c->d_labels.p;
    u.src = c->source->d_xyz.p;
    u.Nsrc = c->source->V;
    u.sfeat = c->d_sfeat.p;
    u.cfw = c->cfw.empty() ? nullptr : c->d_cfw.p;
    u.cfw_rows = c->cfw_rows;
    u.pptr = c->d_pptr.p;
    u.pidx = c->d_pidx.p;
    u.order = c->d_order.p;
    u.absw = c->d_absw.p;
    u.pmax = c->pmax;
    u.simmeasure = c->p.simmeasure;
    u.percentile = c->p.percentile;
    u.U = c->d_U.p;
    const size_t nsamp = (size_t)c->L * c->pidx.size();
    MSM_HIP(c->d_tval.ensure(nsamp));
    MSM_HIP(c->d_fix_list.ensure(nsamp));
    MSM_HIP(c->d_fix_pt.ensure(3 * nsamp));
    if (!c->d_fix_count.p) MSM_HIP(c->d_fix_count.zero(unary_fix_counter_words(), ctx->stream));
    if (!c->fix_off_valid) {
        std::vector<uint32_t> off;
        unary_fix_offsets(N, c->L, c->pmax, c->pptr.data(), c->order.data(), off);
        MSM_TRY(c->d_fix_off.upload(off.data(), off.size(), ctx));
        MSM_TRY(ctx_sync(ctx));
        c->fix_off_valid = true;
    }
    MSM_HIP(c->d_queues.ensure(N));
    u.ntri = c->target->T;
    u.tval = c->d_tval.p;
    u.fix_list = c->d_fix_list.p;
    u.fix_pt = c->d_fix_pt.p;
    u.fix_cnt = c->d_fix_count.p;
    u.fix_off = c->d_fix_off.p;
    u.redo_list = c->d_queues.p;
    if (c->timing) {
        u.ev_start = c->ev0[c->ev_next];
        u.ev_stop = c->ev1[c->ev_next];
        c->ev_next = (c->ev_next + 1) % (int)c->ev0.size();
        c->ev_count = std::min(c->ev_count + 1, (int)c->ev0.size());
    }
    switch (c->p.kind) {
        case MSM_COST_UNIVARIATE: st = launch_unary_univariate(ctx, u); break;
        case MSM_COST_MULTIVARIATE:
        case MSM_COST_PATCHWISE: {
            {
                st = ensure_vertex_major(c);
                if (st) return st;
                u.sfeat_vm = c->d_sfeat_vm.p;
                u.cfw_vm = c->cfw.empty() ? nullptr : c->d_cfw_vm.p;
            }
            MSM_HIP(c->d_stri.ensure(nsamp));
            MSM_HIP(c->d_sw3.ensure(3 * nsamp));
            UnaryWeightsScratch w{c->d_stri.p, c->d_sw3.p};
            st = launch_unary_multivariate(ctx, u, w, c->p.kind == MSM_COST_PATCHWISE);
            break;
        }
        default: return fail(MSM_ERR_INVALID, "unknown cost kind %d", c->p.kind);
    }
    if (st) return st;
    c->counters[0] += (int64_t)nsamp;
    c->counters[1] += (int64_t)c->L * N;
    c->table_valid = true;
    return MSM_OK;
}

}

extern "C" {

msm_cost *msm_cost_create(msm_ctx *ctx, const msm_cost_params *params) {
    if (!ctx || !params) {
        fail(MSM_ERR_INVALID, "msm_cost_create: null argument");
        return nullptr;
    }
    if (params->kind < MSM_COST_UNIVARIATE || params->kind > MSM_COST_HO_MULTIVARIATE) {
        fail(MSM_ERR_INVALID, "msm_cost_create: unknown cost kind %d", params->kind);
        return nullptr;
    }
    if (params->simmeasure != 1 && params->simmeasure != 2 && params->simmeasure != 4 && params->simmeasure != 5) {
        fail(MSM_ERR_INVALID, "Unknown similarity metric");
        return nullptr;
    }
    if ((params->simmeasure == 4 || params->simmeasure == 5) && !(params->percentile > 0.0 + kEps && params->percentile < 1.0 - kEps)) {
        fail(MSM_ERR_INVALID, "Percentile must be between 0 and 1.");
        return nullptr;
    }
    msm_cost *c = new msm_cost();
    c->ctx = ctx;
    c->p = *params;
    (void)hipSetDevice(ctx->device);
    if (c->d_counters.zero(4, ctx->stream) != hipSuccess) {
        fail(MSM_ERR_HIP, "msm_cost_create: allocation failed");
        delete c;
        return nullptr;
    }
    return c;
}

void msm_cost_destroy(msm_cost *c) {
    if (!c) return;
    (void)hipSetDevice(c->ctx->device);
    (void)drop_pending_move(c);
    (void)hipStreamSynchronize(c->ctx->stream);
    for (hipEvent_t e : c->ev0) (void)hipEventDestroy(e);
    for (hipEvent_t e : c->ev1) (void)hipEventDestroy(e);
    delete c;
}

int msm_cost_set_meshes(msm_cost *c, msm_mesh *target, msm_mesh *source, msm_mesh *cpgrid) {
    if (!c || !target || !source || !cpgrid) return fail(MSM_ERR_INVALID, "msm_cost_set_meshes: null argument");
    if (target->ctx != c->ctx || source->ctx != c->ctx || cpgrid->ctx != c->ctx) return fail(MSM_ERR_INVALID, "meshes belong to another context");
    if (source->V < cpgrid->V) return fail(MSM_ERR_INVALID, "source mesh has fewer vertices than the control grid");
    c->target = target;
    c->source = source;
    c->cpgrid = cpgrid;
    c->cp_conn_valid = false;
    c->orig_xyz = source->xyz;
    c->ocp_xyz = cpgrid->xyz;
    MSM_TRY(c->d_orig.upload(c->orig_xyz.data(), c->orig_xyz.size(), c->ctx));
    MSM_TRY(c->d_ocp.upload(c->ocp_xyz.data(), c->ocp_xyz.size(), c->ctx));
    MSM_TRY(ctx_sync(c->ctx));
    c->have_source = false;
    invalidate_table(c);
    return MSM_OK;
}

int msm_cost_reset_source(msm_cost *c, msm_mesh *source) {
    if (!c || !source) return fail(MSM_ERR_INVALID, "msm_cost_reset_source: null argument");
    if (source->ctx != c->ctx) return fail(MSM_ERR_INVALID, "msm_cost_reset_source: the mesh belongs to another context");
    if (c->source && source->V != c->source->V) return fail(MSM_ERR_INVALID, "source mesh size changed");
    c->source = source;
    c->have_source = false;
    invalidate_table(c);
    return MSM_OK;
}

int msm_cost_reset_cpgrid(msm_cost *c, msm_mesh *cpgrid) {
    if (!c || !cpgrid) return fail(MSM_ERR_INVALID, "msm_cost_reset_cpgrid: null argument");
    if (cpgrid->ctx != c->ctx) return fail(MSM_ERR_INVALID, "msm_cost_reset_cpgrid: the mesh belongs to another context");
    if (c->cpgrid && cpgrid->V != c->cpgrid->V) return fail(MSM_ERR_INVALID, "control grid size changed");
    c->cpgrid = cpgrid;
    c->cp_conn_valid = false;
    c->have_source = false;
    invalidate_table(c);
    return MSM_OK;
}

int msm_cost_set_source_features(msm_cost *c, const double *feat, int32_t D) {
    if (!c || !feat || D <= 0) return fail(MSM_ERR_INVALID, "msm_cost_set_source_features: bad arguments");
    int st = need(c, c->source != nullptr, "meshes");
    if (st) return st;
    c->D = D;
    MSM_TRY(ctx_sync(c->ctx));
    c->sfeat.assign(feat, feat + (size_t)D * c->source->V);
    c->vm_valid = false;
    MSM_HIP(c->d_sfeat.ensure(c->sfeat.size()));
    {
        const int st = upload_staged(c->ctx, c->d_sfeat.p, c->sfeat.data(), sizeof(double) * c->sfeat.size());
        if (st) return st;
        MSM_TRY(ctx_sync(c->ctx));
    }
    invalidate_table(c);
    return MSM_OK;
}

int msm_cost_set_cfweight(msm_cost *c, const double *w, int32_t rows) {
    if (!c) return fail(MSM_ERR_INVALID, "null cost");
    int st = need(c, c->source != nullptr, "meshes");
    if (st) return st;
    MSM_TRY(ctx_sync(c->ctx));
    if (!w) {
        c->cfw.clear();
        c->cfw_rows = 0;
        c->vm_valid = false;
    } else {
        if (rows <= 0) return fail(MSM_ERR_INVALID, "msm_cost_set_cfweight: rows must be positive");
        if (rows != 1 && c->D > 0 && rows != c->D)
            return fail(MSM_ERR_INVALID, "DiscreteModel ERROR:: costfunction weighting has dimensions incompatible with data");
        c->cfw.assign(w, w + (size_t)rows * c->source->V);
        c->cfw_rows = rows;
        c->vm_valid = false;
        MSM_HIP(c->d_cfw.ensure(c->cfw.size()));
        st = upload_staged(c->ctx, c->d_cfw.p, c->cfw.data(), sizeof(double) * c->cfw.size());
        if (st) return st;
        MSM_TRY(ctx_sync(c->ctx));
    }
    c->have_source = false;
    invalidate_table(c);
    return MSM_OK;
}

int msm_cost_set_spacings(msm_cost *c, const double *maxsep, double mvdmax) {
    if (!c || !maxsep) return fail(MSM_ERR_INVALID, "msm_cost_set_spacings: null argument");
    int st = need(c, c->cpgrid != nullptr, "meshes");
    if (st) return st;
    c->maxsep.assign(maxsep, maxsep + c->cpgrid->V);
    c->mvdmax = mvdmax;
    c->have_source = false;
    invalidate_table(c);
    return MSM_OK;
}

int msm_cost_set_labels(msm_cost *c, const double *labels, int32_t L, const double *rot) {
    if (!c || !labels || !rot || L <= 0) return fail(MSM_ERR_INVALID, "msm_cost_set_labels: bad arguments");
    int st = need(c, c->cpgrid != nullptr, "meshes");
    if (st) return st;
    MSM_TRY(ctx_sync(c->ctx));
    c->L = L;
    c->fix_off_valid = false;
    c->labels.assign(labels, labels + 3 * (size_t)L);
    c->rot.assign(rot, rot + 9 * (size_t)c->cpgrid->V);
    MSM_TRY(c->d_labels.upload(c->labels.data(), c->labels.size(), c->ctx));
    MSM_TRY(c->d_rot.upload(c->rot.data(), c->rot.size(), c->ctx));
    invalidate_table(c);
    return MSM_OK;
}

int msm_cost_set_triplets(msm_cost *c, const int32_t *triplets, int32_t T) {
    if (!c || (!triplets && T > 0) || T < 0) return fail(MSM_ERR_INVALID, "msm_cost_set_triplets: bad arguments");
    int st = need(c, c->cpgrid != nullptr, "meshes");
    if (st) return st;
    for (int64_t i = 0; i < 3 * (int64_t)T; ++i)
        if (triplets[i] < 0 || triplets[i] >= c->cpgrid->V) return fail(MSM_ERR_INVALID, "triplet node id out of range");
    MSM_TRY(ctx_sync(c->ctx));
    c->triplets.assign(triplets, triplets + 3 * (size_t)T);
    c->move_valid = false;
    if (T > 0) MSM_TRY(c->d_triplets.upload(c->triplets.data(), c->triplets.size(), c->ctx));
    return MSM_OK;
}

int msm_cost_set_pairs(msm_cost *c, const int32_t *pairs, int32_t P) {
    if (!c || (!pairs && P > 0) || P < 0) return fail(MSM_ERR_INVALID, "msm_cost_set_pairs: bad arguments");
    int st = need(c, c->cpgrid != nullptr, "meshes");
    if (st) return st;
    for (int64_t i = 0; i < 2 * (int64_t)P; ++i)
        if (pairs[i] < 0 || pairs[i] >= c->cpgrid->V) return fail(MSM_ERR_INVALID, "pair node id out of range");
    MSM_TRY(ctx_sync(c->ctx));
    c->pairs.assign(pairs, pairs + 2 * (size_t)P);
    if (P > 0) MSM_TRY(c->d_pairs.upload(c->pairs.data(), c->pairs.size(), c->ctx));
    return MSM_OK;
}

int msm_cost_get_source_data(msm_cost *c) {
    if (!c) return fail(MSM_ERR_INVALID, "null cost");
    (void)drop_pending_move(c);
    int st = need(c, c->target && c->source && c->cpgrid, "meshes");
    if (st) return st;
    st = need(c, c->D > 0, "source features");
    if (st) return st;
    st = need(c, (int)c->maxsep.size() == c->cpgrid->V, "spacings");
    if (st) return st;
    if (c->target->V == 0 || c->source->V == 0) return fail(MSM_ERR_STATE, "CostFunction::You must supply source and target meshes.");
    const bool timing = std::getenv("MSMHIP_TIMING") != nullptr;
    auto tick = std::chrono::steady_clock::now();
    auto lap = [&](const char *what) {
        if (!timing) return;
        const auto now = std::chrono::steady_clock::now();
        fprintf(stderr, "  get_source_data: %s %.1f ms\n", what, std::chrono::duration<double, std::milli>(now - tick).count());
        tick = now;
    };
    st = is_ho(c) ? patches_by_triangle(c) : patches_by_range(c);
    if (st) return st;
    lap("patches");
    c->pmax = 1;
    for (int g = 0; g < c->ngroups; ++g) c->pmax = std::max(c->pmax, c->pptr[g + 1] - c->pptr[g]);
    st = resample_weights(c);
    if (st) return st;
    lap("resample_weights");
    msm_ctx *ctx = c->ctx;
    MSM_TRY(c->d_pptr.upload(c->pptr.data(), c->pptr.size(), ctx));
    if (is_ho(c)) {
        MSM_TRY(c->d_pidx.upload_vec(c->pidx, ctx));
    } else {
        if (!c->pidx_asc_on_device) MSM_TRY(c->d_pidx_asc.upload_vec(c->pidx, ctx));
        MSM_HIP(c->d_pidx.ensure(std::max<size_t>(c->pidx.size(), 1)));
        MSM_HIP(c->d_code.ensure(c->source->V));
        st = launch_sort_patches(ctx, c->source->d_xyz.p, c->source->V, c->d_pptr.p, c->ngroups, c->d_pidx_asc.p, c->d_code.p, c->d_pidx.p);
        if (st) return st;
    }
    MSM_TRY(c->d_absw.upload(c->absw.data(), c->absw.size(), ctx));
    {
        const int N = c->cpgrid->V;
        const double *cp = c->cpgrid->xyz.data();
        auto spread = [](uint32_t v) {
            v &= 0x3ff;
            v = (v | (v << 16)) & 0x030000ff;
            v = (v | (v << 8)) & 0x0300f00f;
            v = (v | (v << 4)) & 0x030c30c3;
            v = (v | (v << 2)) & 0x09249249;
            return v;
        };
        std::vector<std::pair<uint32_t, int32_t>> key(N);
        for (int i = 0; i < N; ++i) {
            uint32_t q[3];
            for (int a = 0; a < 3; ++a) {
                const double u = (cp[(size_t)a * N + i] + kBounds) / (2 * kBounds);
                q[a] = (uint32_t)std::max(0.0, std::min(1023.0, u == u ? u * 1024.0 : 0.0));
            }
            key[i] = {spread(q[0]) << 2 | spread(q[1]) << 1 | spread(q[2]), i};
        }
        std::sort(key.begin(), key.end());
        c->order.resize(N);
        for (int i = 0; i < N; ++i) c->order[i] = key[i].second;
        MSM_TRY(c->d_order.upload(c->order.data(), c->order.size(), ctx));
        c->fix_off_valid = false;
    }
    MSM_TRY(ctx_sync(ctx));
    lap("orders + uploads");
    c->have_source = true;
    invalidate_table(c);
    return MSM_OK;
}

int msm_cost_patches(msm_cost *c, int32_t *ngroups, int32_t *ptr, int32_t *idx, int64_t cap) {
    if (!c) return fail(MSM_ERR_INVALID, "null cost");
    int st = need(c, c->have_source, "get_source_data()");
    if (st) return st;
    if (ngroups) *ngroups = c->ngroups;
    if (ptr) std::copy(c->pptr.begin(), c->pptr.end(), ptr);
    if (idx) {
        if ((int64_t)c->pidx.size() > cap) return fail(MSM_ERR_CAPACITY, "patch index buffer too small");
        std::copy(c->pidx.begin(), c->pidx.end(), idx);
    }
    return MSM_OK;
}

int msm_cost_absolute_weights(msm_cost *c, double *absw) {
    if (!c || !absw) return fail(MSM_ERR_INVALID, "msm_cost_absolute_weights: null argument");
    int st = need(c, c->have_source, "get_source_data()");
    if (st) return st;
    std::copy(c->absw.begin(), c->absw.end(), absw);
    return MSM_OK;
}

int msm_cost_unary_table_async(msm_cost *c) {
    if (!c) return fail(MSM_ERR_INVALID, "null cost");
    MSM_TRY(drop_ctx_pending(c->ctx));
    c->table_valid = false;
    c->rotations_valid = false;
    c->h_U.clear();
    return ensure_unary_table(c);
}

int msm_cost_unary_table_fetch(msm_cost *c, double *U) {
    if (!c || !U) return fail(MSM_ERR_INVALID, "msm_cost_unary_table_fetch: null argument");
    MSM_TRY(drop_ctx_pending(c->ctx));
    int st = need(c, c->table_valid, "msm_cost_unary_table_async()");
    if (st) return st;
    msm_ctx *ctx = c->ctx;
    const size_t n = (size_t)c->L * c->cpgrid->V;
    void *mapped = ctx_mapped(ctx, U, sizeof(double) * n);
    if (mapped && reinterpret_cast<uintptr_t>(mapped) % 16 == 0) {
        st = ctx_flag(ctx);
        if (st) return st;
        st = launch_copy_to_mapped(ctx, c->d_U.p, static_cast<double *>(mapped), n, ctx->d_flag_map);
        if (st) return st;
        MSM_TRY(ctx_sync(ctx));
        volatile int *flags = ctx->h_flag;
        if (flags[0] != 0) {
            flags[0] = 0;
            return check_status(ctx, "computeUnaryCosts");
        }
        return MSM_OK;
    }
    MSM_TRY(c->d_U.download(U, n, ctx));
    return check_status(ctx, "computeUnaryCosts");
}

int msm_cost_unary_table(msm_cost *c, double *U) {
    int st = msm_cost_unary_table_async(c);
    if (st) return st;
    return msm_cost_unary_table_fetch(c, U);
}

int msm_cost_unary_batch(msm_cost *c, const int32_t *nodes, const int32_t *labels, int32_t n, double *out) {
    if (!c || !nodes || !labels || !out || n < 0) return fail(MSM_ERR_INVALID, "msm_cost_unary_batch: bad arguments");
    MSM_TRY(drop_ctx_pending(c->ctx));
    if (!c->table_valid || c->h_U.size() != (size_t)c->L * c->cpgrid->V) {
        int st = ensure_unary_table(c);
        if (st) return st;
        c->h_U.resize((size_t)c->L * c->cpgrid->V);
        st = msm_cost_unary_table_fetch(c, c->h_U.data());
        if (st) return st;
    }
    const int N = c->cpgrid->V;
    for (int i = 0; i < n; ++i) {
        if (nodes[i] < 0 || nodes[i] >= N || labels[i] < 0 || labels[i] >= c->L) return fail(MSM_ERR_INVALID, "unary query %d out of range", i);
        out[i] = c->h_U[(size_t)labels[i] * N + nodes[i]];
    }
    return MSM_OK;
}

int msm_cost_enable_timing(msm_cost *c, int enable) {
    if (!c) return fail(MSM_ERR_INVALID, "null cost");
    if (enable && c->ev0.empty()) {
        c->ev0.resize(64);
        c->ev1.resize(64);
        for (size_t i = 0; i < c->ev0.size(); ++i) {
            MSM_HIP(hipEventCreate(&c->ev0[i]));
            MSM_HIP(hipEventCreate(&c->ev1[i]));
        }
    }
    c->timing = enable != 0;
    c->ev_next = 0;
    c->ev_count = 0;
    return MSM_OK;
}

int msm_cost_kernel_times(msm_cost *c, double *ms, int32_t cap, int32_t *n) {
    if (!c || !ms || !n) return fail(MSM_ERR_INVALID, "msm_cost_kernel_times: null argument");
    MSM_TRY(drop_ctx_pending(c->ctx));
    MSM_TRY(ctx_sync(c->ctx));
    const int total = (int)c->ev0.size(), cnt = std::min(c->ev_count, (int)cap);
    for (int k = 0; k < cnt; ++k) {
        const int slot = ((c->ev_next - cnt + k) % total + total) % total;
        float f = 0.f;
        MSM_HIP(hipEventElapsedTime(&f, c->ev0[slot], c->ev1[slot]));
        ms[k] = f;
    }
    *n = cnt;
    return MSM_OK;
}

int msm_cost_counters(msm_cost *c, int64_t counters[4]) {
    if (!c || !counters) return fail(MSM_ERR_INVALID, "msm_cost_counters: null argument");
    counters[0] = c->counters[0];
    counters[1] = c->counters[1];
    counters[2] = c->counters[2];
    counters[3] = c->counters[3];
    return MSM_OK;
}


}
```

### newmsm_amd/csrc/cost_internal.hpp

```cpp
#pragma once

#include <vector>

#include "devbuf.hpp"
#include "kernels.hpp"

using msm::DevBuf;

struct msm_cost {
    msm_ctx *ctx = nullptr;
    msm_cost_params p{};
    msm_mesh *target = nullptr, *source = nullptr, *cpgrid = nullptr;
    std::vector<double> orig_xyz;
    std::vector<double> ocp_xyz;
    int D = 0;
    std::vector<double> sfeat;
    DevBuf<double> d_sfeat;
    DevBuf<double> d_sfeat_vm, d_cfw_vm;
    bool vm_valid = false;
    std::vector<double> cfw;
    int cfw_rows = 0;
    DevBuf<double> d_cfw;
    std::vector<double> maxsep;
    double mvdmax = 0;
    DevBuf<double> d_maxsep;
    int L = 0;
    std::vector<double> labels, rot;
    DevBuf<double> d_labels, d_rot;
    DevBuf<double> d_rnl, d_moved;
    std::vector<int32_t> triplets, pairs;
    DevBuf<int32_t> d_triplets, d_pairs;
    DevBuf<double> d_orig, d_ocp;
    DevBuf<int32_t> d_cp_tri, d_cp_tid_ptr, d_cp_tid;
    bool cp_conn_valid = false;
    DevBuf<int32_t> d_labeling;
    DevBuf<double> d_clique_out;
    DevBuf<double> d_ho_vals, d_ho_big;
    DevBuf<unsigned> d_ho_pending, d_ho_count;
    DevBuf<int32_t> d_slot_tri;
    DevBuf<int4> d_blk;
    DevBuf<double> d_slot_w, d_slot_sf, d_slot_cw, d_slot_wda, d_tri_frame, d_tri_stat;
    int64_t move_tails = 0;
    struct PendingMove {
        bool valid = false;
        int kind = 0;
        int label = 0;
        double *E = nullptr;
        uint64_t epoch = 0;
        std::vector<int32_t> labeling;
        msm::CliqueArgs a;
        msm::MoveArgs m;
        msm::MoveLabels lab;
    } pending;
    int64_t prefetch_hits = 0, prefetch_drops = 0;
    DevBuf<unsigned> d_defer_list, d_defer_cnt;
    int move_nblk = 0, move_cap = 0, move_parity = 0;
    bool move_valid = false;
    bool have_source = false;
    int ngroups = 0, pmax = 0;
    std::vector<int32_t> pptr, pidx;
    DevBuf<int32_t> d_pptr, d_pidx;
    std::vector<int32_t> order;
    DevBuf<int32_t> d_order;
    DevBuf<uint32_t> d_fix_off;
    bool fix_off_valid = false;
    std::vector<double> absw;
    DevBuf<int32_t> d_pidx_asc;
    DevBuf<uint32_t> d_code;
    DevBuf<double4> d_chunkb;
    bool pidx_asc_on_device = false;
    int patch_cap_hint = 0;
    DevBuf<double> d_absw, d_maxw;
    DevBuf<double> d_U;
    bool table_valid = false;
    bool rotations_valid = false;
    std::vector<double> h_U;
    DevBuf<unsigned long long> d_counters;
    int64_t counters[4] = {0, 0, 0, 0};
    DevBuf<uint32_t> d_slots;
    DevBuf<double> d_tval;
    DevBuf<int> d_stri;
    DevBuf<double> d_sw3;
    DevBuf<unsigned long long> d_fix_list;
    DevBuf<double> d_fix_pt;
    DevBuf<unsigned int> d_fix_count;
    msm_mesh *asphere = nullptr;
    int aVs = 0, aTs = 0;
    DevBuf<double> d_atarget, d_asrc, d_aw_val;
    DevBuf<int32_t> d_asrc_tri, d_aw_ptr, d_aw_cp, d_af_ptr, d_af_idx;
    bool have_anat = false;
    bool timing = false;
    std::vector<hipEvent_t> ev0, ev1;
    int ev_next = 0, ev_count = 0;
    DevBuf<int> d_queues;
    DevBuf<int> d_counts;
};


namespace msm {
int query_host(msm_mesh *target, const double *q, int N, int *tri_id, int *vid, double *w, int mode, const char *what, const double *q_on_device = nullptr);
const Adjacency &mesh_adjacency(msm_mesh *m);
int ensure_label_rotations(msm_cost *c);
int drop_pending_move(msm_cost *c);
int ensure_vertex_major(msm_cost *c);
inline bool cost_is_ho(const msm_cost *c) { return c->p.kind == MSM_COST_HO_UNIVARIATE || c->p.kind == MSM_COST_HO_MULTIVARIATE; }
}
```

### newmsm_amd/csrc/kernels.hpp

```cpp
#pragma once

#include "internal.hpp"

namespace msm {

int launch_build_masks(msm_ctx *ctx, const DevTree &T, const double4 *d_nodebox, unsigned long long *d_mask);
int launch_build_recs(msm_ctx *ctx, const double *d_xyz, int V, const int32_t *d_tri, int T, TriRec *d_rec, float4 *d_tcone, const int32_t *d_leaf_tri,
                      int nentries, float4 *d_cone);
int launch_build_recs_forest(msm_ctx *ctx, const double *d_xyz, size_t comp_stride, size_t tree_stride, const int32_t *d_tri, int T, int B, TriRec *d_rec, float4 *d_tcone,
                             size_t s_rec, const int32_t *d_leaf_tri, float4 *d_cone, size_t s_leaf, const int *d_entries, size_t entries_stride);
int launch_build_raytri(msm_ctx *ctx, const TriRec *d_rec, const float4 *d_edge, int T, const double *d_feat1, int D, float4 *d_out);
struct AdaptiveDevArgs {
    int nOld, nNew;
    const int *fvid, *rvid;
    const double *fw, *rw;
    const double *oldA, *newA;
    int *roff, *rfill, *rkey;
    double *rwt;
    int *coff, *cfill, *ckey;
    double *cval, *correction;
    int *scan_tmp;
    int *long_flag;
    int *tkey;
    double *tval;
    int *row_ptr, *col;
    double *val;
    int B = 1;
    size_t fstride = 0, rstride = 0;
    size_t s_f = 0, s_r = 0, s_oldA = 0, s_newA = 0, s_roff = 0, s_rfill = 0, s_r3 = 0, s_coff = 0, s_cfill = 0, s_cap = 0, s_corr = 0, s_rowptr = 0, s_scan = 0;
};
int launch_vertex_areas_batch(msm_ctx *ctx, const double *d_xyz, size_t comp, size_t set, int V, const int32_t *d_tri, int T, const int32_t *d_tid_ptr, const int32_t *d_tid,
                              int B, double *d_ta, double *d_area);
int launch_apply_rows_batch(msm_ctx *ctx, const AdaptiveDevArgs &a, int D, const double *d_data, double *d_out, size_t out_stride);
int launch_vertex_areas(msm_ctx *ctx, const double *d_xyz, int V, const int32_t *d_tri, int T, const int32_t *d_tid_ptr, const int32_t *d_tid, double *d_ta,
                        double *d_area);
int launch_adaptive_surgery(msm_ctx *ctx, const AdaptiveDevArgs &a);
int launch_apply_rows(msm_ctx *ctx, int nNew, int nOld, int D, const int *row_ptr, const int *col, const double *val, const double *d_data, double *d_out);
int launch_copy_to_mapped(msm_ctx *ctx, const double *d_src, double *mapped_dst, size_t n, int *flags_mapped);
int launch_query(msm_ctx *ctx, const DevTree &T, const double *d_q, int N, int *d_tri, int *d_vid, double *d_w, int mode);
int launch_query_rays(msm_ctx *ctx, const DevTree &T, const double *d_q, int N, int *d_tri, int *d_vid, double *d_w, int mode, int *d_open);
int launch_closest_vertex(msm_ctx *ctx, const DevTree &T, const double *d_q, int N, int *d_out);
int launch_warp(msm_ctx *ctx, const DevTree &T, const double *d_q, int N, const double *d_to, int V, bool to_sphere, double *d_out);
int query_lanes(long long N);
inline size_t smooth_bounds_offset(int N) { return ((size_t)3 * N + 3) / 4 * 4; }
inline size_t smooth_scratch_doubles(int N) { return smooth_bounds_offset(N) + 4 * (((size_t)N + 63) / 64) + 4; }
int launch_smooth(msm_ctx *ctx, const double *d_xyz, int N, double *d_unit, const int *d_cv, const double *d_data, int Vorig, int D, double sigma,
                  double cosang, const double *d_excl, double *d_out, double *d_excl_out);
int launch_fold_detect(msm_ctx *ctx, const double *d_xyz, int V, const int32_t *d_tri, int T, const int32_t *d_tid_ptr, const int32_t *d_tid, int32_t *d_fold);
int launch_sort_patches(msm_ctx *ctx, const double *d_xyz, int n, const int32_t *d_pptr, int ngroups, const int32_t *d_pidx, uint32_t *d_code,
                        int32_t *d_sorted);
struct RangeGrid {
    const int *start = nullptr, *ids = nullptr, *bad = nullptr;
    int G = 0;
    double origin = 0.0, inv_h = 0.0;
};
int launch_range_grid_build(msm_ctx *ctx, const double *d_src, int Nsrc, int G, double origin, double inv_h, int *d_start, int *d_cursor, int *d_ids, int *d_bad, int *d_tmp);
int launch_range(msm_ctx *ctx, const double *d_cp, int Ncp, const double *d_src, int Nsrc, const double *d_maxsep, double range, int cap,
                 uint32_t *d_slots, int *d_counts, double4 *d_chunk_bounds, int *d_nflag, int cluster = 1, const RangeGrid *grid = nullptr);
int launch_patch_compact(msm_ctx *ctx, const uint32_t *d_slots, int cap, const int32_t *d_pptr, int M, int32_t *d_pidx, size_t pidx_cap = (size_t)-1);
int launch_scan_exclusive(msm_ctx *ctx, int *d_data, int n, int *d_tmp);

int launch_label_rotations(msm_ctx *ctx, const double *d_cp, int N, const double *d_rot, const double *d_labels, int L, double *d_rnl,
                           double *d_moved);

struct UnaryLaunch {
    DevTree tree;
    const double *tfeat;
    int D;
    int N, L;
    const double *cp;
    const double *rnl;
    const double *labels;
    const double *src;
    int Nsrc;
    const double *sfeat;
    const double *cfw;
    int cfw_rows;
    const double *sfeat_vm = nullptr;
    const double *cfw_vm = nullptr;
    const int *pptr, *pidx;
    const int *order;
    const double *absw;
    int pmax;
    int simmeasure;
    double percentile;
    double *U;
    int ntri;
    double *tval;
    unsigned long long *fix_list;
    double *fix_pt;
    unsigned int *fix_cnt;
    const unsigned int *fix_off;
    int *redo_list;
    hipEvent_t ev_start = nullptr, ev_stop = nullptr;
};
int unary_nsplit(int L, int pmax);
int unary_fix_segments();
size_t unary_fix_counter_words();
void unary_fix_offsets(int N, int L, int pmax, const int32_t *pptr, const int32_t *order, std::vector<uint32_t> &off);
int launch_unary_univariate(msm_ctx *ctx, const UnaryLaunch &u);
struct UnaryWeightsScratch {
    int *stri;
    double *sw3;
};
int launch_unary_multivariate(msm_ctx *ctx, const UnaryLaunch &u, const UnaryWeightsScratch &w, bool patchwise);

struct CliqueArgs {
    int kind, simmeasure;
    int N, L, T, P;
    const int *triplets;
    const int *pairs;
    const double *cp;
    const double *ocp;
    const double *orig;
    int Norig;
    const double *moved;
    const double *rnl;
    const int *cp_tri;
    int Tc;
    const int *cp_tid_ptr, *cp_tid;
    double lambda, mu, kappa, k_exp, rexp, mvdmax, percentile;
    DevTree tree;
    const double *tfeat;
    int D;
    const double *src;
    int Nsrc;
    const double *sfeat;
    const double *cfw;
    int cfw_rows;
    const double *sfeat_vm, *cfw_vm;
    const int *bin_ptr, *bin_idx;
    int bin_cap;
    double *ho_big;
    double *ho_vals;
    unsigned *ho_pending;
    unsigned *ho_count;
    const double *absw;
    int rmode;
    DevTree atree;
    const double *atarget;
    int Va;
    const double *asrc;
    int Vs;
    const int *asrc_tri;
    int Ts;
    const int *aw_ptr, *aw_cp;
    const double *aw_val;
    const int *af_ptr, *af_idx;
    int *status;
};
constexpr int kPairSmallPatch = 80;
constexpr int kHoBinMax = 16384;
constexpr int kHoBigBlocks = 512;
constexpr int kMoveLabelWords = 704;
struct MoveLabels {
    uint32_t w[kMoveLabelWords];
};
struct MoveArgs {
    const int *slot_tri;
    const double *slot_w;
    const double *slot_sf;
    const double *slot_cw;
    const double *slot_wda;
    const double *tri_frame;
    const double *tri_stat;
    const int4 *blk;
    int nblk;
    int cap;
    const int *labeling;
    int label;
    double *vals;
    unsigned *defer_list;
    unsigned *defer_cnt;
    int parity;
    double *out;
    int *host_flags;
    int single;
};
int launch_move_prepare(msm_ctx *ctx, const CliqueArgs &a, int nslots, int *slot_tri, double *slot_w, double *slot_sf, double *slot_cw, double *slot_wda,
                        double *tri_frame, double *tri_stat);
int launch_move(msm_ctx *ctx, const CliqueArgs &a, const MoveArgs &m, const MoveLabels *labels, hipEvent_t ev_start, hipEvent_t ev_stop);
int launch_move_tail(msm_ctx *ctx, const CliqueArgs &a, const MoveArgs &m, const MoveLabels *labels);

int launch_triplet_batch(msm_ctx *ctx, const CliqueArgs &a, const int *qt, const int *qa, const int *qb, const int *qc, int n, double *out);
int launch_triplet_octets(msm_ctx *ctx, const CliqueArgs &a, const int *labeling, int label, double *out);
struct MoveLabels;
int launch_triplet_octets_packed(msm_ctx *ctx, const CliqueArgs &a, const MoveLabels &lab, int label, double *out, int *host_flag);
int launch_pairwise_batch(msm_ctx *ctx, const CliqueArgs &a, const int *qp, const int *qa, const int *qb, int n, double *out);
int launch_pairwise_table(msm_ctx *ctx, const CliqueArgs &a, double *out);
int launch_triplet_table(msm_ctx *ctx, const CliqueArgs &a, int t0, int t1, double *out);


struct alignas(32) GroupPatchRef {
    const int *ids;
    const double *vals;
    int begin, count;
    int pad[2];
};

struct GroupArgs {
    int S, N, L, D, Tc, Vt;
    int simmeasure, fixnan;
    const int *pairs;
    const int *triplets;
    const int *const *pptr;
    const int *const *pidx;
    const double *const *F;
    const double *const *pval;
    const GroupPatchRef *dir;
    const double *mask;
    const double *moved;
    const double *cp;
    const double *orig;
    double lambda, mu, kappa, k_exp, rexp, subcorr;
    double percentile;
    const int *move_labeling;
    int move_label, move_offset;
    const int *move_order;
    const int4 *move_order4;
    int move_base;
    int move_combos;
    int move_first, move_count;
    const int *move_prev;
    double *move_e00;
    double *move_e11;
    int patch_cap;
    int pair_lanes;
    int *status;
};
int launch_rotate_to_label(msm_ctx *ctx, const double *d_xyz, int V, const double centre[3], const double label[3], double *d_out, size_t stride = 0);
int launch_rotate_to_labels(msm_ctx *ctx, const double *d_xyz, int V, const double centre[3], const double *d_labels3, int L, const double *d_rot9, double *d_out,
                            size_t stride);
int launch_group_pairwise(msm_ctx *ctx, const GroupArgs &a, const int *qp, const int *qa, const int *qb, int n, double *out);
int launch_group_patch_values(msm_ctx *ctx, const GroupArgs &a, double *const *pval, const int *node_flags = nullptr);
int launch_group_mark_nodes(msm_ctx *ctx, const int *pairs, long long pair0, long long pair1, int *node_flags);
int launch_group_expand_order(msm_ctx *ctx, const int *order, const int *pairs, int n, int4 *out);
int launch_group_patch_dir(msm_ctx *ctx, const GroupArgs &a, double *const *pval, GroupPatchRef *dir);
int launch_group_kept(msm_ctx *ctx, const int *order, int base, const double *kept, int n, double *out);
int launch_group_triplet(msm_ctx *ctx, const GroupArgs &a, const int *qt, const int *qa, const int *qb, const int *qc, int n, double *out);
struct ForestDev {
    const int4 *node;
    const int32_t *parent, *leaf_tri, *grid;
    const float4 *cone;
    const TriRec *rec;
    size_t s_node, s_leaf, s_rec, s_grid;
    const int2 *info;
};
int launch_query_forest(msm_ctx *ctx, const ForestDev &f, int B, const double *d_q, int N, int *d_vid, double *d_w, size_t comp);
int launch_group_pairs(msm_ctx *ctx, const ForestDev &f, const double *d_cp, int S, int N, int *d_pairs);
int launch_group_permute_pairs(msm_ctx *ctx, const int *d_in, const int *d_order, int n, int *d_out);
int launch_group_moved(msm_ctx *ctx, const double *d_rot, int nodes, const double *d_labels , int L, double *d_moved);
int launch_group_centres(msm_ctx *ctx, const double *d_moved_subject, const double *d_spacing_subject, int N, int L, double *d_centres, double *d_sep);

}
```

### newmsm_amd/csrc/unary_kernels.hip

```cpp
#include <algorithm>
#include <cstdlib>

#include "kernels.hpp"
#include "search_device.hpp"
#include "similarity_device.hpp"

#ifndef MSM_VARIANT
#define MSM_VARIANT 0
#endif

namespace msm {

namespace {

constexpr int kFixSegs = 64;
constexpr int kCntStride = 32;
constexpr int kChunk = 768;
constexpr int kQueueCap = 3072;
constexpr int kDeferred = 1 << 20;
constexpr unsigned kInvalidPair = 0xffffffffu;
constexpr int kTriBits = 22;

__device__ __forceinline__ void raise_status(int *status, int code) { atomicMin(status, code); }

__device__ __forceinline__ double wave_sum(double v) {
#pragma unroll
    for (int off = 32; off > 0; off >>= 1) v += __shfl_xor(v, off, 64);
    return v;
}

struct SamplesArgs {
    DevTree tree;
    const double *tfeat;
    int tD;
    int N, L;
    const double *rnl;
    const double *src;
    int Nsrc;
    const int *pptr, *pidx;
    const int *order;
    int pmax;
    int nsplit;
    double *tval;
    int *stri;
    double *sw3;
    unsigned long long *fix_list;
    double *fix_pt;
    unsigned int *fix_cnt;
    const unsigned int *fix_off;
    const double *sfeat;
    const double *cfw;
    const double *absw;
    int simmeasure;
    double percentile;
    double *U;
    int *redo_list;
    unsigned int *redo_count;
    int *status;
};

__device__ __forceinline__ int fast_div(int s, int P, float invP) {
    int q = (int)((float)s * invP);
    if (q * P > s) --q;
    else if ((q + 1) * P <= s) ++q;
    return q;
}

__device__ __forceinline__ double emit_sample(const SamplesArgs &a, size_t g, const V3 &p, int t) {
    const TriRec &r = a.tree.rec[t];
    double wa, wb, wc;
    area_weights(rec_v0(r), rec_v1(r), rec_v2(r), p, wa, wb, wc);
    if (a.tval) {
        const double v = wa * a.tfeat[(size_t)r.id[0] * a.tD] + wb * a.tfeat[(size_t)r.id[1] * a.tD] + wc * a.tfeat[(size_t)r.id[2] * a.tD];
        a.tval[g] = v;
        return v;
    } else {
        a.stri[g] = t;
        a.sw3[3 * g] = wa;
        a.sw3[3 * g + 1] = wb;
        a.sw3[3 * g + 2] = wc;
    }
    return 0.0;
}

__device__ __forceinline__ void emit_failure(const SamplesArgs &a, size_t g, int code) {
    raise_status(a.status, code);
    const double nan = __longlong_as_double(0x7ff8000000000000ll);
    if (a.tval) {
        a.tval[g] = nan;
    } else {
        a.stri[g] = code;
        a.sw3[3 * g] = a.sw3[3 * g + 1] = a.sw3[3 * g + 2] = nan;
    }
}

__device__ __forceinline__ double patch_similarity(const double *A, const double *W, const double *B, int P, int lane, int simmeasure, double percentile) {
    if (simmeasure == 4 || simmeasure == 5) return patch_dice(A, B, P, lane, simmeasure, percentile);
    if (simmeasure == 2) {
        double sw = 0, ma = 0, mb = 0;
        for (int i = lane; i < P; i += 64) {
            sw += W[i];
            ma += W[i] * A[i];
            mb += W[i] * B[i];
        }
        sw = wave_sum(sw);
        ma = wave_sum(ma);
        mb = wave_sum(mb);
        if (sw > 0.0) {
            ma /= sw;
            mb /= sw;
        }
        double pr = 0, va = 0, vb = 0;
        for (int i = lane; i < P; i += 64) {
            const double da = A[i] - ma, db = B[i] - mb;
            pr += W[i] * da * db;
            va += W[i] * da * da;
            vb += W[i] * db * db;
        }
        pr = wave_sum(pr);
        va = wave_sum(va);
        vb = wave_sum(vb);
        if (sw > 0.0) {
            pr /= sw;
            va /= sw;
            vb /= sw;
        }
        const double r = (va == 0.0 || vb == 0.0) ? 0.0 : pr / (sqrt(va) * sqrt(vb));
        return 1 - (1 + r) * 0.5;
    }
    double pr = 0;
    for (int i = lane; i < P; i += 64) {
        const double df = A[i] - B[i];
        pr += W[i] * df * df;
    }
    pr = wave_sum(pr);
    return sqrt(pr) / P;
}

}

__global__ __launch_bounds__(256) void k_unary_samples(SamplesArgs a) {
    extern __shared__ __align__(16) double lds[];
    double *sx = lds, *sy = sx + a.pmax, *sz = sy + a.pmax;
    double *sA = sz + a.pmax, *sW = sA + a.pmax;
    double *sR = sW + a.pmax;
    const int lper_all = (a.L + a.nsplit - 1) / a.nsplit;
    double *sT = sR + 9 * a.L;
    unsigned *queue = reinterpret_cast<unsigned *>(sT + (size_t)lper_all * a.pmax);
    int *nin = reinterpret_cast<int *>(queue + kQueueCap);
    int *win = nin + kChunk;
    __shared__ int s_qn, s_ndefer;
    const int tid = threadIdx.x, lane = tid & 63;
    const int per = (a.N + 7) >> 3;
    const int slots = 8 * per;

    {
        const int part = blockIdx.x / slots, slot = blockIdx.x - part * slots;
        const int at = (slot & 7) * per + (slot >> 3);
        if (at >= a.N) return;
        const int node = a.order[at];
        const int lper = (a.L + a.nsplit - 1) / a.nsplit;
        const int l_beg = part * lper, l_end = min(a.L, l_beg + lper);
        if (l_beg >= l_end) return;
        const int beg = a.pptr[node], P = a.pptr[node + 1] - beg;
        const size_t gbase = (size_t)a.L * beg;
        for (int i = tid; i < P; i += 256) {
            const int s = a.pidx[beg + i];
            sx[i] = a.src[s];
            sy[i] = a.src[a.Nsrc + s];
            sz[i] = a.src[2 * a.Nsrc + s];
            if (a.U) {
                sA[i] = a.sfeat[s];
                sW[i] = a.cfw ? a.cfw[s] : 1.0;
            }
        }
        for (int k = tid; k < 9 * a.L; k += 256) sR[k] = a.rnl[(size_t)node * a.L * 9 + k];
        if (tid == 0) s_ndefer = 0;
        const int sbeg = l_beg * P, send = l_end * P;
        const float invP = 1.0f / (float)max(P, 1);

        for (int base = sbeg; base < send; base += kChunk) {
            const int nchunk = min(kChunk, send - base);
            for (int k = tid; k < kChunk; k += 256) nin[k] = 0;
            if (tid == 0) s_qn = 0;
            __syncthreads();

            for (int r0 = 0; r0 < nchunk; r0 += 256) {
                const int sl = r0 + tid;
                unsigned long long pm = 0ull;
                int lbeg = 0;
                bool defer = false;
                if (sl < nchunk) {
                    const int s = base + sl;
                    const int l = fast_div(s, P, invP), i = s - l * P;
                    const V3 p = rotate(sR + 9 * l, mk(sx[i], sy[i], sz[i]));
                    if (outside_root(p)) {
                        nin[sl] = -1;
                    } else {
                        int sub;
                        const int4 leaf = locate_leaf(a.tree, p, sub);
                        lbeg = leaf.y;
                        if (leaf.z < 0) {
                            defer = (-leaf.x - 1) > 64;
                        } else {
                            const float qx = (float)p.x, qy = (float)p.y, qz = (float)p.z;
                            const float inv = rsqrtf(qx * qx + qy * qy + qz * qz);
                            const float fx = qx * inv, fy = qy * inv, fz = qz * inv;
                            const float4 *cone = a.tree.cone + leaf.y;
                            unsigned long long mm = a.tree.mask[(size_t)leaf.z * 64 + sub];
                            while (mm) {
                                int e[4];
                                bool v[4];
#pragma unroll
                                for (int k = 0; k < 4; ++k) {
                                    v[k] = mm != 0ull;
                                    e[k] = v[k] ? __ffsll((long long)mm) - 1 : 0;
                                    mm &= mm - 1ull;
                                }
                                float4 c[4];
#pragma unroll
                                for (int k = 0; k < 4; ++k) c[k] = cone[e[k]];
#pragma unroll
                                for (int k = 0; k < 4; ++k) {
                                    const float dt = fabsf(__builtin_fmaf(c[k].z, fz, __builtin_fmaf(c[k].y, fy, c[k].x * fx)));
                                    if (v[k] && dt >= c[k].w) pm |= 1ull << e[k];
                                }
                            }
                        }
                    }
                }
                const int cntp = __popcll(pm);
                int incl = cntp;
#pragma unroll
                for (int off = 1; off < 64; off <<= 1) {
                    const int up = __shfl_up(incl, off, 64);
                    if (lane >= off) incl += up;
                }
                int wbase = 0;
                if (lane == 63 && incl > 0) wbase = atomicAdd(&s_qn, incl);
                wbase = __shfl(wbase, 63, 64);
                int pos = wbase + incl - cntp;
                if (cntp > 0) {
                    if (pos + cntp > kQueueCap) {
                        defer = true;
                        for (int j = pos; j < kQueueCap; ++j) queue[j] = kInvalidPair;
                    } else {
                        const int *lt = a.tree.leaf_tri + lbeg;
                        const unsigned tag = (unsigned)sl << kTriBits;
                        while (pm) {
                            const int e = __ffsll((long long)pm) - 1;
                            pm &= pm - 1ull;
                            queue[pos++] = tag | (unsigned)lt[e];
                        }
                    }
                }
                if (defer) nin[sl] = kDeferred;
            }
            __syncthreads();

#if !(MSM_VARIANT & 1)
            const int qn = min(s_qn, kQueueCap);
            for (int j = tid; j < qn; j += 256) {
                const unsigned e = queue[j];
                if (e == kInvalidPair) continue;
                const int sl = (int)(e >> kTriBits), t = (int)(e & ((1u << kTriBits) - 1));
                const int s = base + sl;
                const int l = fast_div(s, P, invP), i = s - l * P;
                const V3 p = rotate(sR + 9 * l, mk(sx[i], sy[i], sz[i]));
                V3 mp;
                if (inside_test(a.tree.rec[t], p, mp)) {
                    win[sl] = t;
                    atomicAdd(&nin[sl], 1);
                }
            }
            __syncthreads();

#endif
#if !(MSM_VARIANT & 3)
            for (int sl = tid; sl < nchunk; sl += 256) {
                const int s = base + sl;
                const int n = nin[sl];
                if (n == 1) {
                    const int l = fast_div(s, P, invP), i = s - l * P;
                    const V3 p = rotate(sR + 9 * l, mk(sx[i], sy[i], sz[i]));
                    const double v = emit_sample(a, gbase + s, p, win[sl]);
                    if (a.U) sT[(l - l_beg) * a.pmax + i] = v;
                } else if (n < 0) {
                    emit_failure(a, gbase + s, MSM_ERR_OUTSIDE);
                    atomicAdd(&s_ndefer, 1);
                } else {
                    atomicAdd(&s_ndefer, 1);
                    const int seg = blockIdx.x % kFixSegs;
                    const unsigned slot = a.fix_off[seg] + atomicAdd(&a.fix_cnt[kCntStride * (1 + seg)], 1u);
                    if (slot < a.fix_off[seg + 1]) {
                        const int l = fast_div(s, P, invP), i = s - l * P;
                        const V3 p = rotate(sR + 9 * l, mk(sx[i], sy[i], sz[i]));
                        a.fix_list[slot] = gbase + (unsigned long long)s;
                        a.fix_pt[3 * (size_t)slot] = p.x;
                        a.fix_pt[3 * (size_t)slot + 1] = p.y;
                        a.fix_pt[3 * (size_t)slot + 2] = p.z;
                    } else {
                        raise_status(a.status, MSM_ERR_CAPACITY);
                    }
                }
            }
            __syncthreads();
#endif
        }
        if (a.U) {
            __syncthreads();
            if (s_ndefer == 0) {
                const double absw = a.absw[node];
                for (int l = l_beg + (tid >> 6); l < l_end; l += 4) {
                    const double cost = patch_similarity(sA, sW, sT + (l - l_beg) * a.pmax, P, lane, a.simmeasure, a.percentile);
                    if (lane == 0) a.U[(size_t)l * a.N + node] = absw * cost;
                }
            } else if (tid == 0) {
                a.redo_list[atomicAdd(a.redo_count, 1u)] = node;
            }
        }
    }
}

__global__ __launch_bounds__(256) void k_unary_rays(SamplesArgs a) {
    extern __shared__ __align__(16) double lds[];
    double *sx = lds, *sy = sx + a.pmax, *sz = sy + a.pmax, *sR = sz + a.pmax;
    const int tid = threadIdx.x, lane = tid & 63;
    const int per = (a.N + 7) >> 3;
    const int slots = 8 * per;
    const int part = blockIdx.x / slots, slot = blockIdx.x - part * slots;
    const int at = (slot & 7) * per + (slot >> 3);
    if (at >= a.N) return;
    const int node = a.order[at];
    const int lper = (a.L + a.nsplit - 1) / a.nsplit;
    const int l_beg = part * lper, l_end = min(a.L, l_beg + lper);
    if (l_beg >= l_end) return;
    const int beg = a.pptr[node], P = a.pptr[node + 1] - beg;
    const size_t gbase = (size_t)a.L * beg;
    for (int i = tid; i < P; i += 256) {
        const int s = a.pidx[beg + i];
        sx[i] = a.src[s];
        sy[i] = a.src[a.Nsrc + s];
        sz[i] = a.src[2 * a.Nsrc + s];
    }
    for (int k = 9 * l_beg + tid; k < 9 * l_end; k += 256) sR[k] = a.rnl[(size_t)node * a.L * 9 + k];
    const int sbeg = l_beg * P, send = l_end * P;
    const float invP = 1.0f / (float)max(P, 1);
    int *sleft = reinterpret_cast<int *>(sR + 9 * a.L);
    __shared__ int s_nleft;
    __shared__ unsigned s_base;
    if (tid == 0) s_nleft = 0;
    __syncthreads();
    for (int s0 = sbeg; s0 < send; s0 += 256) {
        const int s = s0 + tid;
        const bool act = s < send;
        bool done = false;
        V3 p = mk(0.0, 0.0, 0.0);
        float fx = 0.f, fy = 0.f, fz = 0.f;
        int4 c = make_int4(-1, -1, -1, -1);
        if (act) {
            const int l = fast_div(s, P, invP), i = s - l * P;
            p = rotate(sR + 9 * l, mk(sx[i], sy[i], sz[i]));
            c = ray_cell_of(a.tree, p, fx, fy, fz);
        }
        if (act) {
            if (c.x >= 0) {
                const float4 *rec = a.tree.ray_tri + (size_t)kRayPieces * c.x;
                const float4 e0 = rec[0], e1 = rec[1], e2 = rec[2];
                const double2 *dv = reinterpret_cast<const double2 *>(rec + 3);
                double2 d0 = dv[0], d1 = dv[1], d2 = dv[2], d3 = dv[3], d4 = dv[4], d5 = dv[5];
                int t = c.x;
                bool vouch_needed = __float_as_int(e1.w) >= 0;
                float4 ev = e1;
                if (!ray_accepts(e0, e1, e2, fx, fy, fz)) {
                    t = -1;
                    int4 mo = make_int4(c.w, -1, -1, -1);
                    if (c.w < -1) mo = a.tree.ray_more[-2 - c.w];
#pragma unroll 1
                    for (int k = 0; k < 6 && t < 0; ++k) {
                        const int ck = k == 0 ? c.y : (k == 1 ? c.z : (k == 2 ? mo.x : (k == 3 ? mo.y : (k == 4 ? mo.z : mo.w))));
                        if (ck < 0) break;
                        const float4 *r2 = a.tree.ray_tri + (size_t)kRayPieces * ck;
                        const float4 g0 = r2[0], g1 = r2[1], g2 = r2[2];
                        if (ray_accepts(g0, g1, g2, fx, fy, fz)) {
                            t = ck;
                            ev = g1;
                            vouch_needed = __float_as_int(g1.w) >= 0;
                        }
                    }
                    if (t >= 0) {
                        dv = reinterpret_cast<const double2 *>(a.tree.ray_tri + (size_t)kRayPieces * t + 3);
                        d0 = dv[0], d1 = dv[1], d2 = dv[2], d3 = dv[3], d4 = dv[4], d5 = dv[5];
                    }
                }
                if (t >= 0 && vouch_needed && !ray_vouches(a.tree, ev, p)) t = -1;
                if (t >= 0) {
                    double wa, wb, wc;
                    area_weights(mk(d0.x, d0.y, d1.x), mk(d1.y, d2.x, d2.y), mk(d3.x, d3.y, d4.x), p, wa, wb, wc);
                    const size_t g = gbase + s;
                    if (a.tval) {
                        a.tval[g] = wa * d4.y + wb * d5.x + wc * d5.y;
                    } else {
                        a.stri[g] = t;
                        a.sw3[3 * g] = wa;
                        a.sw3[3 * g + 1] = wb;
                        a.sw3[3 * g + 2] = wc;
                    }
                    done = true;
                }
            }
        }
        const bool left = act && !done;
        const unsigned long long bal = __ballot(left);
        if (bal) {
            const int leader = __ffsll((long long)bal) - 1;
            int base = 0;
            if (lane == leader) base = atomicAdd(&s_nleft, __popcll(bal));
            base = __shfl(base, leader, 64);
            if (left) sleft[base + __popcll(bal & ((1ull << lane) - 1ull))] = s;
        }
    }
    __syncthreads();
    const int nleft = s_nleft;
    if (nleft > 0) {
        const int seg = blockIdx.x % kFixSegs;
        if (tid == 0) s_base = a.fix_off[seg] + atomicAdd(&a.fix_cnt[kCntStride * (1 + seg)], (unsigned)nleft);
        __syncthreads();
        const unsigned base = s_base, end = a.fix_off[seg + 1];
        for (int j = tid; j < nleft; j += 256) {
            if (base + j < end) {
                const int s = sleft[j];
                const int l = fast_div(s, P, invP), i = s - l * P;
                const V3 p = rotate(sR + 9 * l, mk(sx[i], sy[i], sz[i]));
                a.fix_list[base + j] = gbase + (unsigned long long)s;
                a.fix_pt[3 * (size_t)(base + j)] = p.x;
                a.fix_pt[3 * (size_t)(base + j) + 1] = p.y;
                a.fix_pt[3 * (size_t)(base + j) + 2] = p.z;
            } else {
                raise_status(a.status, MSM_ERR_CAPACITY);
            }
        }
    }
}

__global__ __launch_bounds__(256) void k_unary_fixup(SamplesArgs a) {
    __shared__ unsigned s_pre[kFixSegs + 1];
    if (threadIdx.x < kFixSegs) {
        const int seg = threadIdx.x;
        const unsigned cnt = min(a.fix_cnt[kCntStride * (1 + seg)], a.fix_off[seg + 1] - a.fix_off[seg]);
        unsigned incl = cnt;
#pragma unroll
        for (int off = 1; off < 64; off <<= 1) {
            const unsigned up = __shfl_up(incl, off, 64);
            if (seg >= off) incl += up;
        }
        s_pre[seg + 1] = incl;
        if (seg == 0) s_pre[0] = 0;
    }
    __syncthreads();
    const unsigned n = s_pre[kFixSegs];
    const int lane = threadIdx.x & 63, sub = lane & 7, grp = lane >> 3;
    const unsigned per_block = 256 / 8, stride = gridDim.x * per_block;
    for (unsigned j0 = blockIdx.x * per_block + (threadIdx.x >> 6) * 8; j0 < n; j0 += stride) {
        const unsigned j = j0 + grp;
        const bool valid = j < n;
        V3 p = mk(0.0, 0.0, 0.0);
        size_t g = 0;
        if (valid) {
            int seg = 0;
#pragma unroll
            for (int step = kFixSegs / 2; step > 0; step >>= 1)
                if (s_pre[seg + step] <= j) seg += step;
            const size_t slot = a.fix_off[seg] + (j - s_pre[seg]);
            g = (size_t)a.fix_list[slot];
            p = mk(a.fix_pt[3 * slot], a.fix_pt[3 * slot + 1], a.fix_pt[3 * slot + 2]);
        }
        const int found = group8_find(a.tree, valid, p, lane);
        if (valid && sub == 0) {
            const int t = found == kGroupUndecided ? find_closest_triangle(a.tree, p) : found;
            if (t < 0) emit_failure(a, g, t);
            else emit_sample(a, g, p, t);
        }
    }
}

struct ReduceArgs {
    int N, L, Nsrc;
    const double *sfeat;
    const double *cfw;
    int cfw_rows;
    const int *pptr, *pidx;
    const double *absw;
    const double *tval;
    int pmax;
    int simmeasure;
    double percentile;
    double *U;
    const int *redo_list;
    const unsigned int *redo_count;
};

__global__ __launch_bounds__(256) void k_unary_reduce_univariate(ReduceArgs a) {
    extern __shared__ __align__(16) double lds[];
    double *sA = lds, *sW = sA + a.pmax;
    const int tid = threadIdx.x, lane = tid & 63, wave = tid >> 6;
    const unsigned n = a.redo_count ? *a.redo_count : (unsigned)a.N;
    for (unsigned k = blockIdx.x; k < n; k += gridDim.x) {
        const int node = a.redo_list ? a.redo_list[k] : (int)k;
        const int beg = a.pptr[node], P = a.pptr[node + 1] - beg;
        __syncthreads();
        for (int i = tid; i < P; i += 256) {
            const int s = a.pidx[beg + i];
            sA[i] = a.sfeat[s];
            sW[i] = (a.cfw && a.cfw_rows >= 1) ? a.cfw[s] : 1.0;
        }
        __syncthreads();
        const double absw = a.absw[node];
        for (int l = wave; l < a.L; l += 4) {
            const double cost = patch_similarity(sA, sW, a.tval + (size_t)a.L * beg + (size_t)l * P, P, lane, a.simmeasure, a.percentile);
            if (lane == 0) a.U[(size_t)l * a.N + node] = absw * cost;
        }
    }
}

constexpr int kRedLanes = 8;
constexpr int kRedKeep = 12;

__device__ __forceinline__ double group_sum(double v) {
#pragma unroll
    for (int off = kRedLanes / 2; off > 0; off >>= 1) v += __shfl_xor(v, off, kRedLanes);
    return v;
}

__global__ __launch_bounds__(256) void k_unary_reduce_flat(ReduceArgs a, unsigned int *clear, int clear_words) {
    extern __shared__ __align__(16) double lds[];
    double *sA = lds, *sW = sA + a.pmax;
    __shared__ double s_stat[3];
    const int tid = threadIdx.x, sub = tid & (kRedLanes - 1), grp = tid / kRedLanes;
    if (blockIdx.x == 0 && clear)
        for (int k = tid; k < clear_words; k += 256) clear[k] = 0u;
    const int node = a.redo_list ? a.redo_list[blockIdx.x] : (int)blockIdx.x;
    const int beg = a.pptr[node], P = a.pptr[node + 1] - beg;
    const bool has_w = a.cfw && a.cfw_rows >= 1;
    const bool in_regs = true;
    double breg[kRedKeep];
#pragma unroll
    for (int k = 0; k < kRedKeep; ++k) breg[k] = 0.0;
    if (grp < a.L) {
        const double *B = a.tval + (size_t)a.L * beg + (size_t)grp * P;
#pragma unroll
        for (int k = 0; k < kRedKeep; ++k) breg[k] = (sub + kRedLanes * k < P) ? B[sub + kRedLanes * k] : 0.0;
    }
    for (int i = tid; i < P; i += 256) {
        const int s = a.pidx[beg + i];
        sA[i] = a.sfeat[s];
        sW[i] = has_w ? a.cfw[s] : 1.0;
    }
    __syncthreads();
    if (a.simmeasure == 2) {
        if (tid < 64) {
            double sw = 0, ma = 0;
            for (int i = tid; i < P; i += 64) {
                sw += sW[i];
                ma += sW[i] * sA[i];
            }
            sw = wave_sum(sw);
            ma = wave_sum(ma);
            if (sw > 0.0) ma /= sw;
            double va = 0;
            for (int i = tid; i < P; i += 64) {
                const double da = sA[i] - ma;
                va += sW[i] * da * da;
            }
            va = wave_sum(va);
            if (tid == 0) s_stat[0] = sw, s_stat[1] = ma, s_stat[2] = va;
        }
        __syncthreads();
    }
    const double absw = a.absw[node];
    for (int l = grp; l < a.L; l += 256 / kRedLanes) {
        const double *B = a.tval + (size_t)a.L * beg + (size_t)l * P;
        if (!(in_regs && l == grp)) {
#pragma unroll
            for (int k = 0; k < kRedKeep; ++k) breg[k] = (sub + kRedLanes * k < P) ? B[sub + kRedLanes * k] : 0.0;
        }
        double cost;
        if (a.simmeasure == 2) {
            const double sw = s_stat[0], ma = s_stat[1];
            double mb = 0;
#pragma unroll
            for (int k = 0; k < kRedKeep; ++k) {
                const int i = sub + kRedLanes * k;
                if (i < P) mb += sW[i] * breg[k];
            }
            for (int i = sub + kRedLanes * kRedKeep; i < P; i += kRedLanes) mb += sW[i] * B[i];
            mb = group_sum(mb);
            if (sw > 0.0) mb /= sw;
            double pr = 0, vb = 0;
#pragma unroll
            for (int k = 0; k < kRedKeep; ++k) {
                const int i = sub + kRedLanes * k;
                if (i < P) {
                    const double da = sA[i] - ma, db = breg[k] - mb;
                    pr += sW[i] * da * db;
                    vb += sW[i] * db * db;
                }
            }
            for (int i = sub + kRedLanes * kRedKeep; i < P; i += kRedLanes) {
                const double da = sA[i] - ma, db = B[i] - mb;
                pr += sW[i] * da * db;
                vb += sW[i] * db * db;
            }
            pr = group_sum(pr);
            vb = group_sum(vb);
            double va = s_stat[2];
            if (sw > 0.0) {
                pr /= sw;
                va /= sw;
                vb /= sw;
            }
            const double r = (va == 0.0 || vb == 0.0) ? 0.0 : pr / (sqrt(va) * sqrt(vb));
            cost = 1 - (1 + r) * 0.5;
        } else {
            double pr = 0;
#pragma unroll
            for (int k = 0; k < kRedKeep; ++k) {
                const int i = sub + kRedLanes * k;
                if (i < P) {
                    const double df = sA[i] - breg[k];
                    pr += sW[i] * df * df;
                }
            }
            for (int i = sub + kRedLanes * kRedKeep; i < P; i += kRedLanes) {
                const double df = sA[i] - B[i];
                pr += sW[i] * df * df;
            }
            pr = group_sum(pr);
            cost = sqrt(pr) / P;
        }
        if (sub == 0) a.U[(size_t)l * a.N + node] = absw * cost;
    }
}

struct ReduceMvArgs {
    int N, L, Nsrc, D;
    const double *tfeat;
    const TriRec *rec;
    const double *sfeat;
    const double *cfw;
    int cfw_rows;
    const int *pptr, *pidx;
    const double *absw;
    const int *stri;
    const double *sw3;
    int simmeasure;
    double percentile;
    int patchwise;
    int pmax;
    double *U;
};

__global__ __launch_bounds__(256) void k_unary_reduce_features(ReduceMvArgs a) {
    const int node = blockIdx.x;
    const int beg = a.pptr[node], P = a.pptr[node + 1] - beg;
    const int tid = threadIdx.x, lane = tid & 63, wave = tid >> 6;
    const double absw = a.absw[node];
    const double nan = __longlong_as_double(0x7ff8000000000000ll);
    const int nwaves = blockDim.x >> 6;
    for (int l = wave; l < a.L; l += nwaves) {
        const size_t g0 = (size_t)a.L * beg + (size_t)l * P;
        double cost;
        if (!a.patchwise) {
            double acc = 0.0;
            bool bad = false;
            for (int i = lane; i < P; i += 64) {
                const int t = a.stri[g0 + i];
                if (t < 0) {
                    bad = true;
                    continue;
                }
                const TriRec &r = a.rec[t];
                const double *f0 = a.tfeat + (size_t)r.id[0] * a.D, *f1 = a.tfeat + (size_t)r.id[1] * a.D, *f2 = a.tfeat + (size_t)r.id[2] * a.D;
                acc += feature_vector_similarity(a.simmeasure, a.percentile, a.sfeat, a.cfw, a.cfw_rows, a.Nsrc, a.pidx[beg + i], a.D, f0, f1, f2,
                                                 a.sw3[3 * (g0 + i)], a.sw3[3 * (g0 + i) + 1], a.sw3[3 * (g0 + i) + 2]);
            }
            acc = wave_sum(acc);
            cost = P > 0 ? acc / P : acc;
            if (__ballot(bad)) cost = nan;
        } else {
            double total = 0.0;
            bool bad = false;
            for (int d = 0; d < a.D; ++d) {
                const double *A = a.sfeat + (size_t)d * a.Nsrc;
                auto Bv = [&](int i) {
                    const int t = a.stri[g0 + i];
                    if (t < 0) {
                        bad = true;
                        return nan;
                    }
                    const TriRec &r = a.rec[t];
                    return a.sw3[3 * (g0 + i)] * a.tfeat[(size_t)r.id[0] * a.D + d] + a.sw3[3 * (g0 + i) + 1] * a.tfeat[(size_t)r.id[1] * a.D + d] +
                           a.sw3[3 * (g0 + i) + 2] * a.tfeat[(size_t)r.id[2] * a.D + d];
                };
                auto Wv = [&](int i) { return (a.cfw && a.cfw_rows >= 1) ? a.cfw[a.pidx[beg + i]] : 1.0; };
                double c;
                if (a.simmeasure == 4 || a.simmeasure == 5) {
                    extern __shared__ __align__(16) double lds[];
                    double *pa = lds + (size_t)wave * 2 * a.pmax, *pb = pa + a.pmax;
                    asm volatile("s_waitcnt lgkmcnt(0)" ::: "memory");
                    for (int i = lane; i < P; i += 64) {
                        pa[i] = A[a.pidx[beg + i]];
                        pb[i] = Bv(i);
                    }
                    asm volatile("s_waitcnt lgkmcnt(0)" ::: "memory");
                    c = patch_dice(pa, pb, P, lane, a.simmeasure, a.percentile);
                } else if (a.simmeasure == 2) {
                    double sw = 0, ma = 0, mb = 0;
                    for (int i = lane; i < P; i += 64) {
                        const double w = Wv(i);
                        sw += w;
                        ma += w * A[a.pidx[beg + i]];
                        mb += w * Bv(i);
                    }
                    sw = wave_sum(sw);
                    ma = wave_sum(ma);
                    mb = wave_sum(mb);
                    if (sw > 0.0) {
                        ma /= sw;
                        mb /= sw;
                    }
                    double pr = 0, va = 0, vb = 0;
                    for (int i = lane; i < P; i += 64) {
                        const double w = Wv(i), da = A[a.pidx[beg + i]] - ma, db = Bv(i) - mb;
                        pr += w * da * db;
                        va += w * da * da;
                        vb += w * db * db;
                    }
                    pr = wave_sum(pr);
                    va = wave_sum(va);
                    vb = wave_sum(vb);
                    if (sw > 0.0) {
                        pr /= sw;
                        va /= sw;
                        vb /= sw;
                    }
                    const double r = (va == 0.0 || vb == 0.0) ? 0.0 : pr / (sqrt(va) * sqrt(vb));
                    c = 1 - (1 + r) * 0.5;
                } else {
                    double pr = 0;
                    for (int i = lane; i < P; i += 64) {
                        const double df = A[a.pidx[beg + i]] - Bv(i);
                        pr += Wv(i) * df * df;
                    }
                    pr = wave_sum(pr);
                    c = sqrt(pr) / P;
                }
                total += c;
            }
            cost = total / a.D;
            if (__ballot(bad)) cost = nan;
        }
        if (lane == 0) a.U[(size_t)l * a.N + node] = absw * cost;
    }
}

struct ReduceMv8Args {
    int N, L, Nsrc, D;
    const double *tfeat;
    const TriRec *rec;
    const double *sfeat_vm;
    const double *cfw_vm;
    int cfw_rows;
    const int *pptr, *pidx;
    const int *order;
    const double *absw;
    const int *stri;
    const double *sw3;
    int simmeasure;
    double *U;
};

__global__ __launch_bounds__(256) void k_unary_reduce_mv8(ReduceMv8Args a) {
    const int node = a.order[blockIdx.x];
    const int beg = a.pptr[node], P = a.pptr[node + 1] - beg;
    const int tid = threadIdx.x, lane = tid & 63, wave = tid >> 6;
    const int grp = lane / kMvLanes, j = lane % kMvLanes;
    const double absw = a.absw[node];
    const double nan = __longlong_as_double(0x7ff8000000000000ll);
    const int D = a.D;
    for (int l = wave; l < a.L; l += 4) {
        const size_t g0 = (size_t)a.L * beg + (size_t)l * P;
        double acc = 0.0;
        bool bad = false;
        for (int i0 = 0; i0 < P; i0 += 64 / kMvLanes) {
            const int i = i0 + grp;
            const bool have = i < P;
            int t = -1, sv = 0;
            double wa = 0, wb = 0, wc = 0;
            if (have) {
                t = a.stri[g0 + i];
                sv = a.pidx[beg + i];
                wa = a.sw3[3 * (g0 + i)], wb = a.sw3[3 * (g0 + i) + 1], wc = a.sw3[3 * (g0 + i) + 2];
            }
            if (have && t < 0) bad = true;
            const bool go = have && t >= 0;
            const double *f0 = a.tfeat, *f1 = a.tfeat, *f2 = a.tfeat, *sa = a.sfeat_vm, *cw = nullptr;
            if (go) {
                const TriRec &r = a.rec[t];
                f0 = a.tfeat + (size_t)r.id[0] * D, f1 = a.tfeat + (size_t)r.id[1] * D, f2 = a.tfeat + (size_t)r.id[2] * D;
                sa = a.sfeat_vm + (size_t)sv * D;
                cw = a.cfw_vm ? a.cfw_vm + (size_t)sv * a.cfw_rows : nullptr;
            }
            const double c = feature_vector_similarity8(a.simmeasure, go, j, D, sa, cw, a.cfw_rows, f0, f1, f2, wa, wb, wc);
            if (go && j == 0) acc += c;
        }
        double tot = (j == 0) ? acc : 0.0;
#pragma unroll
        for (int off = 32; off > 0; off >>= 1) tot += __shfl_xor(tot, off, 64);
        double cost = P > 0 ? tot / P : tot;
        if (__ballot(bad)) cost = nan;
        if (lane == 0) a.U[(size_t)l * a.N + node] = absw * cost;
    }
}

template <int K>
__global__ __launch_bounds__(256) void k_unary_reduce_pw8(ReduceMv8Args a) {
    const int node = a.order[blockIdx.x];
    const int beg = a.pptr[node], P = a.pptr[node + 1] - beg;
    const int tid = threadIdx.x, lane = tid & 63, wave = tid >> 6;
    const int grp = lane / kMvLanes, j = lane % kMvLanes;
    const double absw = a.absw[node];
    const double nan = __longlong_as_double(0x7ff8000000000000ll);
    const int D = a.D;
    auto across_groups = [](double v) {
        v += __shfl_xor(v, 8, 64);
        v += __shfl_xor(v, 16, 64);
        v += __shfl_xor(v, 32, 64);
        return v;
    };
    for (int l = wave; l < a.L; l += 4) {
        const size_t g0 = (size_t)a.L * beg + (size_t)l * P;
        bool bad = false;
        auto fetch = [&](int i, double *A, double *B, double &w) {
            const int t = a.stri[g0 + i];
            const int sv = a.pidx[beg + i];
            w = (a.cfw_vm && a.cfw_rows >= 1) ? a.cfw_vm[(size_t)sv * a.cfw_rows] : 1.0;
            if (t < 0) {
                bad = true;
#pragma unroll
                for (int k = 0; k < K; ++k) A[k] = B[k] = nan;
                return;
            }
            const TriRec &r = a.rec[t];
            const double *f0 = a.tfeat + (size_t)r.id[0] * D, *f1 = a.tfeat + (size_t)r.id[1] * D, *f2 = a.tfeat + (size_t)r.id[2] * D;
            const double *sa = a.sfeat_vm + (size_t)sv * D;
            const double wa = a.sw3[3 * (g0 + i)], wb = a.sw3[3 * (g0 + i) + 1], wc = a.sw3[3 * (g0 + i) + 2];
#pragma unroll
            for (int k = 0; k < K; ++k) {
                const int d = j + kMvLanes * k;
                A[k] = d < D ? sa[d] : 0.0;
                B[k] = d < D ? wa * f0[d] + wb * f1[d] + wc * f2[d] : 0.0;
            }
        };
        double c[K];
        if (a.simmeasure == 2) {
            double sw = 0.0, ma[K], mb[K];
#pragma unroll
            for (int k = 0; k < K; ++k) ma[k] = mb[k] = 0.0;
            for (int i = grp; i < P; i += 64 / kMvLanes) {
                double A[K], B[K], w;
                fetch(i, A, B, w);
                sw += w;
#pragma unroll
                for (int k = 0; k < K; ++k) {
                    ma[k] += w * A[k];
                    mb[k] += w * B[k];
                }
            }
            sw = across_groups(sw);
#pragma unroll
            for (int k = 0; k < K; ++k) {
                ma[k] = across_groups(ma[k]);
                mb[k] = across_groups(mb[k]);
                if (sw > 0.0) {
                    ma[k] /= sw;
                    mb[k] /= sw;
                }
            }
            double pr[K], va[K], vb[K];
#pragma unroll
            for (int k = 0; k < K; ++k) pr[k] = va[k] = vb[k] = 0.0;
            for (int i = grp; i < P; i += 64 / kMvLanes) {
                double A[K], B[K], w;
                fetch(i, A, B, w);
#pragma unroll
                for (int k = 0; k < K; ++k) {
                    const double da = A[k] - ma[k], db = B[k] - mb[k];
                    pr[k] += w * da * db;
                    va[k] += w * da * da;
                    vb[k] += w * db * db;
                }
            }
#pragma unroll
            for (int k = 0; k < K; ++k) {
                double p = across_groups(pr[k]), x = across_groups(va[k]), y = across_groups(vb[k]);
                if (sw > 0.0) {
                    p /= sw;
                    x /= sw;
                    y /= sw;
                }
                const double rr = (x == 0.0 || y == 0.0) ? 0.0 : p / (sqrt(x) * sqrt(y));
                c[k] = 1 - (1 + rr) * 0.5;
            }
        } else {
            double pr[K];
#pragma unroll
            for (int k = 0; k < K; ++k) pr[k] = 0.0;
            for (int i = grp; i < P; i += 64 / kMvLanes) {
                double A[K], B[K], w;
                fetch(i, A, B, w);
#pragma unroll
                for (int k = 0; k < K; ++k) {
                    const double df = A[k] - B[k];
                    pr[k] += w * df * df;
                }
            }
#pragma unroll
            for (int k = 0; k < K; ++k) c[k] = sqrt(across_groups(pr[k])) / P;
        }
        double total = 0.0;
#pragma unroll
        for (int k = 0; k < K; ++k)
            if (j + kMvLanes * k < D) total += c[k];
        total = mv_group_sum(total);
        double cost = total / D;
        if (__ballot(bad)) cost = nan;
        if (lane == 0) a.U[(size_t)l * a.N + node] = absw * cost;
    }
}

static size_t samples_lds(int pmax, int L, int nsplit) {
    const size_t lper = (size_t)(L + nsplit - 1) / nsplit;
    return sizeof(double) * (5 * (size_t)pmax + 9 * (size_t)L + lper * pmax) + sizeof(unsigned) * kQueueCap + sizeof(int) * 2 * kChunk;
}

int unary_nsplit(int L, int pmax) {
    int n = std::max(1, std::min(4, (int)(((size_t)L * pmax + kChunk - 1) / kChunk)));
    while (n < L && samples_lds(pmax, L, n) > 64 * 1024) ++n;
    return std::min(n, std::max(L, 1));
}
int unary_fix_segments() { return kFixSegs; }
size_t unary_fix_counter_words() { return (size_t)kCntStride * (1 + kFixSegs); }
void unary_fix_offsets(int N, int L, int pmax, const int32_t *pptr, const int32_t *order, std::vector<uint32_t> &off) {
    const int nsplit = unary_nsplit(L, pmax), per = (N + 7) >> 3, slots = 8 * per;
    const int lper = (L + nsplit - 1) / nsplit;
    std::vector<uint64_t> size(kFixSegs, 0);
    for (int b = 0; b < nsplit * slots; ++b) {
        const int part = b / slots, slot = b - part * slots;
        const int at = (slot & 7) * per + (slot >> 3);
        if (at >= N) continue;
        const int node = order[at];
        const int l_beg = part * lper, l_end = std::min(L, l_beg + lper);
        if (l_beg >= l_end) continue;
        size[b % kFixSegs] += (uint64_t)(l_end - l_beg) * (pptr[node + 1] - pptr[node]);
    }
    off.assign(kFixSegs + 1, 0);
    for (int s = 0; s < kFixSegs; ++s) off[s + 1] = (uint32_t)std::min<uint64_t>(0xffffffffull, off[s] + size[s]);
}

static bool uses_ray_table(const DevTree &t) { return t.simple && t.ray_G > 0 && t.ray_cell && t.ray_tri; }

static int launch_samples(msm_ctx *ctx, const UnaryLaunch &u, const UnaryWeightsScratch *w, SamplesArgs &a, bool fused_reduction = false) {
    if (u.tree.nnodes <= 0 || !u.tree.mask) return fail(MSM_ERR_STATE, "target search structure missing");
    a.tree = u.tree;
    a.tfeat = u.tfeat;
    a.tD = u.D > 0 ? u.D : 1;
    a.N = u.N;
    a.L = u.L;
    a.rnl = u.rnl;
    a.src = u.src;
    a.Nsrc = u.Nsrc;
    a.pptr = u.pptr;
    a.pidx = u.pidx;
    a.order = u.order;
    a.pmax = u.pmax;
    a.tval = w ? nullptr : u.tval;
    a.stri = w ? w->stri : nullptr;
    a.sw3 = w ? w->sw3 : nullptr;
    a.fix_list = u.fix_list;
    a.fix_pt = u.fix_pt;
    a.fix_cnt = u.fix_cnt;
    a.fix_off = u.fix_off;
    a.sfeat = u.sfeat;
    a.cfw = (u.cfw && u.cfw_rows >= 1) ? u.cfw : nullptr;
    a.absw = u.absw;
    a.simmeasure = u.simmeasure;
    a.percentile = u.percentile;
    a.U = (w || !fused_reduction) ? nullptr : u.U;
    a.redo_list = u.redo_list;
    a.redo_count = u.fix_cnt;
    a.status = ctx->d_status;
    if (u.ntri >= (1 << kTriBits)) return fail(MSM_ERR_CAPACITY, "target mesh has %d triangles; the sample queue packs ids in %d bits", u.ntri, kTriBits);
    a.nsplit = unary_nsplit(u.L, u.pmax);
    const size_t lds = samples_lds(u.pmax, u.L, a.nsplit);
    if (!uses_ray_table(u.tree) && lds > 64 * 1024) {
        if (lds > 160 * 1024) return fail(MSM_ERR_CAPACITY, "a patch of %d points does not fit in LDS", u.pmax);
        MSM_HIP(hipFuncSetAttribute(reinterpret_cast<const void *>(k_unary_samples), hipFuncAttributeMaxDynamicSharedMemorySize, (int)lds));
    }
    const int blocks = a.nsplit * 8 * ((u.N + 7) / 8);
    if (u.ev_start) MSM_HIP(hipEventRecord(u.ev_start, ctx->stream));
    if (uses_ray_table(u.tree)) {
        a.U = nullptr;
        const int lper = (u.L + a.nsplit - 1) / a.nsplit;
        const size_t rays_lds = sizeof(double) * (3 * (size_t)u.pmax + 9 * (size_t)u.L) + sizeof(int) * ((size_t)lper * u.pmax + 4) + 16;
        if (rays_lds > 64 * 1024) MSM_HIP(hipFuncSetAttribute(reinterpret_cast<const void *>(k_unary_rays), hipFuncAttributeMaxDynamicSharedMemorySize, (int)rays_lds));
        hipLaunchKernelGGL(k_unary_rays, dim3(blocks), dim3(256), rays_lds, ctx->stream, a);
    } else {
        hipLaunchKernelGGL(k_unary_samples, dim3(blocks), dim3(256), lds, ctx->stream, a);
    }
    MSM_HIP(hipGetLastError());
    if (u.ev_stop) MSM_HIP(hipEventRecord(u.ev_stop, ctx->stream));
    hipLaunchKernelGGL(k_unary_fixup, dim3(4096), dim3(256), 0, ctx->stream, a);
    MSM_HIP(hipGetLastError());
    return MSM_OK;
}

int launch_unary_univariate(msm_ctx *ctx, const UnaryLaunch &u) {
    SamplesArgs a;
    const bool dice = u.simmeasure == 4 || u.simmeasure == 5;
    int st = launch_samples(ctx, u, nullptr, a, dice);
    if (st) return st;
    ReduceArgs r;
    r.N = u.N;
    r.L = u.L;
    r.Nsrc = u.Nsrc;
    r.sfeat = u.sfeat;
    r.cfw = u.cfw;
    r.cfw_rows = u.cfw_rows;
    r.pptr = u.pptr;
    r.pidx = u.pidx;
    r.absw = u.absw;
    r.tval = u.tval;
    r.pmax = u.pmax;
    r.simmeasure = u.simmeasure;
    r.percentile = u.percentile;
    r.U = u.U;
    r.redo_list = u.redo_list;
    r.redo_count = u.fix_cnt;
    if (uses_ray_table(u.tree) && dice) {
        r.redo_list = nullptr;
        r.redo_count = nullptr;
        hipLaunchKernelGGL(k_unary_reduce_univariate, dim3(std::min(u.N, 2048)), dim3(256), sizeof(double) * 2 * (size_t)u.pmax, ctx->stream, r);
        MSM_HIP(hipMemsetAsync(u.fix_cnt, 0, unary_fix_counter_words() * sizeof(unsigned), ctx->stream));
    } else if (!dice) {
        r.redo_list = u.order;
        hipLaunchKernelGGL(k_unary_reduce_flat, dim3(u.N), dim3(256), sizeof(double) * 2 * (size_t)u.pmax, ctx->stream, r, u.fix_cnt,
                           (int)unary_fix_counter_words());
    } else {
        hipLaunchKernelGGL(k_unary_reduce_univariate, dim3(64), dim3(256), sizeof(double) * 2 * (size_t)u.pmax, ctx->stream, r);
        MSM_HIP(hipMemsetAsync(u.fix_cnt, 0, unary_fix_counter_words() * sizeof(unsigned), ctx->stream));
    }
    MSM_HIP(hipGetLastError());
    return MSM_OK;
}

int launch_unary_multivariate(msm_ctx *ctx, const UnaryLaunch &u, const UnaryWeightsScratch &w, bool patchwise) {
    SamplesArgs a;
    int st = launch_samples(ctx, u, &w, a);
    if (st) return st;
    ReduceMvArgs r;
    r.N = u.N;
    r.L = u.L;
    r.Nsrc = u.Nsrc;
    r.D = u.D;
    r.tfeat = u.tfeat;
    r.rec = u.tree.rec;
    r.sfeat = u.sfeat;
    r.cfw = u.cfw;
    r.cfw_rows = u.cfw_rows;
    r.pptr = u.pptr;
    r.pidx = u.pidx;
    r.absw = u.absw;
    r.stri = w.stri;
    r.sw3 = w.sw3;
    r.simmeasure = u.simmeasure;
    r.patchwise = patchwise ? 1 : 0;
    r.pmax = u.pmax;
    r.percentile = u.percentile;
    r.U = u.U;
    const bool dice = u.simmeasure == 4 || u.simmeasure == 5;
    if (!dice && u.D >= 12 && u.D <= kMvLanes * kMvKeep && u.sfeat_vm) {
        ReduceMv8Args m;
        m.N = u.N, m.L = u.L, m.Nsrc = u.Nsrc, m.D = u.D;
        m.tfeat = u.tfeat;
        m.rec = u.tree.rec;
        m.sfeat_vm = u.sfeat_vm;
        m.cfw_vm = u.cfw_vm;
        m.cfw_rows = u.cfw_rows;
        m.pptr = u.pptr, m.pidx = u.pidx, m.order = u.order;
        m.absw = u.absw;
        m.stri = w.stri, m.sw3 = w.sw3;
        m.simmeasure = u.simmeasure;
        m.U = u.U;
        if (!patchwise) hipLaunchKernelGGL(k_unary_reduce_mv8, dim3(u.N), dim3(256), 0, ctx->stream, m);
        else if (u.D <= 32) hipLaunchKernelGGL(k_unary_reduce_pw8<4>, dim3(u.N), dim3(256), 0, ctx->stream, m);
        else hipLaunchKernelGGL(k_unary_reduce_pw8<8>, dim3(u.N), dim3(256), 0, ctx->stream, m);
    } else {
        size_t flds = (dice && patchwise) ? sizeof(double) * 8 * (size_t)u.pmax : 0;
        int threads = 256;
        if (flds > 160 * 1024) {
            flds /= 4;
            threads = 64;
        }
        if (flds > 160 * 1024) return fail(MSM_ERR_CAPACITY, "a patch of %d points does not fit in LDS (patchwise DICE)", u.pmax);
        if (flds > 64 * 1024) MSM_HIP(hipFuncSetAttribute(reinterpret_cast<const void *>(k_unary_reduce_features), hipFuncAttributeMaxDynamicSharedMemorySize, (int)flds));
        hipLaunchKernelGGL(k_unary_reduce_features, dim3(u.N), dim3(threads), flds, ctx->stream, r);
    }
    MSM_HIP(hipGetLastError());
    MSM_HIP(hipMemsetAsync(u.fix_cnt, 0, unary_fix_counter_words() * sizeof(unsigned), ctx->stream));
    return MSM_OK;
}

}
```

Baseline: 352.9 million evals/s.

## Fuse per-row correlation reduction into the ray sampling kernel for univariate costs

For univariate, non-DICE measures on the ray table path, the ray sampler now computes each label row's cost directly in LDS when every sample of that row settles. Rows with unresolved samples are listed with their offsets for a separate finish kernel. Double-buffered fix counters are cleared by block 0 of the next launch, which replaces the memset and the flat reduce kernel. The aim is to cut the tval round trip through global memory and one or two launches. The price is more LDS per block, a fixed waves_per_eu occupancy hint, and extra bookkeeping for row lists.

```diff
diff --git a/include/msmhip.h b/include/msmhip.h
--- a/include/msmhip.h
+++ b/include/msmhip.h
@@ -151,6 +151,7 @@
 int msm_cost_enable_timing(msm_cost *c, int enable);
 int msm_cost_kernel_times(msm_cost *c, double *ms, int32_t cap, int32_t *n);
 int msm_cost_counters(msm_cost *c, int64_t counters[4]);
+int msm_cost_unary_rows(msm_cost *c, int64_t rows[4]);
 
 typedef struct msm_group msm_group;
 typedef struct msm_group_params {
diff --git a/newmsm_amd/_lib.py b/newmsm_amd/_lib.py
--- a/newmsm_amd/_lib.py
+++ b/newmsm_amd/_lib.py
@@ -122,6 +122,7 @@
     "msm_cost_enable_timing": (C.c_int, [_VP, C.c_int]),
     "msm_cost_kernel_times": (C.c_int, [_VP, c_dp, C.c_int32, c_ip]),
     "msm_cost_counters": (C.c_int, [_VP, c_lp]),
+    "msm_cost_unary_rows": (C.c_int, [_VP, c_lp]),
     "msm_group_create": (_VP, [_VP, C.POINTER(GroupParams), C.c_int32]),
     "msm_group_fusion_move": (C.c_int, [_VP, c_ip, C.c_int32, c_dp, c_dp]),
     "msm_group_destroy": (None, [_VP]),
diff --git a/newmsm_amd/api.py b/newmsm_amd/api.py
--- a/newmsm_amd/api.py
+++ b/newmsm_amd/api.py
@@ -658,6 +658,11 @@
         check(lib().msm_cost_counters(self.h, c))
         return dict(samples=c[0], unary=c[1], triplet=c[2], pairwise=c[3])
 
+    def unary_rows(self):
+        r = (C.c_int64 * 4)()
+        check(lib().msm_cost_unary_rows(self.h, r))
+        return dict(fused=bool(r[0]), rows=r[1], open=r[2], listed=r[3])
+
 
 class DiscreteGroupCostFunction:
 
diff --git a/newmsm_amd/csrc/cost.cpp b/newmsm_amd/csrc/cost.cpp
--- a/newmsm_amd/csrc/cost.cpp
+++ b/newmsm_amd/csrc/cost.cpp
@@ -224,11 +224,14 @@
     MSM_HIP(c->d_tval.ensure(nsamp));
     MSM_HIP(c->d_fix_list.ensure(nsamp));
     MSM_HIP(c->d_fix_pt.ensure(3 * nsamp));
-    if (!c->d_fix_count.p) MSM_HIP(c->d_fix_count.zero(unary_fix_counter_words(), ctx->stream));
+    if (!c->d_fix_count.p) MSM_HIP(c->d_fix_count.zero(2 * unary_fix_counter_words(), ctx->stream));
+    if (!c->d_row_stats.p) MSM_HIP(c->d_row_stats.zero(2, ctx->stream));
+    MSM_HIP(c->d_row_list.ensure((size_t)c->L * N));
     if (!c->fix_off_valid) {
-        std::vector<uint32_t> off;
-        unary_fix_offsets(N, c->L, c->pmax, c->pptr.data(), c->order.data(), off);
+        std::vector<uint32_t> off, row_off;
+        unary_fix_offsets(N, c->L, c->pmax, c->pptr.data(), c->order.data(), off, &row_off);
         MSM_TRY(c->d_fix_off.upload(off.data(), off.size(), ctx));
+        MSM_TRY(c->d_row_off.upload(row_off.data(), row_off.size(), ctx));
         MSM_TRY(ctx_sync(ctx));
         c->fix_off_valid = true;
     }
@@ -238,7 +241,13 @@
     u.fix_list = c->d_fix_list.p;
     u.fix_pt = c->d_fix_pt.p;
     u.fix_cnt = c->d_fix_count.p;
+    u.fix_set = &c->fix_set;
     u.fix_off = c->d_fix_off.p;
+    u.row_list = c->d_row_list.p;
+    u.row_off = c->d_row_off.p;
+    u.row_stats = c->d_row_stats.p;
+    u.rows_fused = &c->rows_fused;
+    c->rows_fused = false;
     u.redo_list = c->d_queues.p;
     if (c->timing) {
         u.ev_start = c->ev0[c->ev_next];
@@ -638,5 +647,20 @@
     return MSM_OK;
 }
 
-
-}
+int msm_cost_unary_rows(msm_cost *c, int64_t rows[4]) {
+    if (!c || !rows) return fail(MSM_ERR_INVALID, "msm_cost_unary_rows: null argument");
+    rows[0] = rows[1] = rows[2] = rows[3] = 0;
+    if (!c->rows_fused || !c->d_row_stats.p) return MSM_OK;
+    unsigned int stats[2] = {0, 0};
+    MSM_TRY(drop_ctx_pending(c->ctx));
+    MSM_TRY(c->d_row_stats.download(stats, 2, c->ctx));
+    MSM_TRY(ctx_sync(c->ctx));
+    rows[0] = 1;
+    rows[1] = (int64_t)c->L * c->cpgrid->V;
+    rows[2] = stats[0];
+    rows[3] = stats[1];
+    return MSM_OK;
+}
+
+
+}
diff --git a/newmsm_amd/csrc/cost_internal.hpp b/newmsm_amd/csrc/cost_internal.hpp
--- a/newmsm_amd/csrc/cost_internal.hpp
+++ b/newmsm_amd/csrc/cost_internal.hpp
@@ -84,6 +84,11 @@
     DevBuf<unsigned long long> d_fix_list;
     DevBuf<double> d_fix_pt;
     DevBuf<unsigned int> d_fix_count;
+    int fix_set = 0;
+    DevBuf<uint4> d_row_list;
+    DevBuf<uint32_t> d_row_off;
+    DevBuf<unsigned int> d_row_stats;
+    bool rows_fused = false;
     msm_mesh *asphere = nullptr;
     int aVs = 0, aTs = 0;
     DevBuf<double> d_atarget, d_asrc, d_aw_val;
diff --git a/newmsm_amd/csrc/kernels.hpp b/newmsm_amd/csrc/kernels.hpp
--- a/newmsm_amd/csrc/kernels.hpp
+++ b/newmsm_amd/csrc/kernels.hpp
@@ -90,14 +90,19 @@
     unsigned long long *fix_list;
     double *fix_pt;
     unsigned int *fix_cnt;
+    int *fix_set = nullptr;
     const unsigned int *fix_off;
+    uint4 *row_list = nullptr;
+    const unsigned int *row_off = nullptr;
+    unsigned int *row_stats = nullptr;
+    bool *rows_fused = nullptr;
     int *redo_list;
     hipEvent_t ev_start = nullptr, ev_stop = nullptr;
 };
 int unary_nsplit(int L, int pmax);
 int unary_fix_segments();
 size_t unary_fix_counter_words();
-void unary_fix_offsets(int N, int L, int pmax, const int32_t *pptr, const int32_t *order, std::vector<uint32_t> &off);
+void unary_fix_offsets(int N, int L, int pmax, const int32_t *pptr, const int32_t *order, std::vector<uint32_t> &off, std::vector<uint32_t> *row_off = nullptr);
 int launch_unary_univariate(msm_ctx *ctx, const UnaryLaunch &u);
 struct UnaryWeightsScratch {
     int *stri;
diff --git a/newmsm_amd/csrc/unary_kernels.hip b/newmsm_amd/csrc/unary_kernels.hip
--- a/newmsm_amd/csrc/unary_kernels.hip
+++ b/newmsm_amd/csrc/unary_kernels.hip
@@ -48,6 +48,11 @@
     double *fix_pt;
     unsigned int *fix_cnt;
     const unsigned int *fix_off;
+    uint4 *row_list;
+    const unsigned int *row_off;
+    unsigned int *row_stats;
+    unsigned int *clear_next;
+    int clear_words;
     const double *sfeat;
     const double *cfw;
     const double *absw;
@@ -322,7 +327,266 @@
     }
 }
 
-__global__ __launch_bounds__(256) void k_unary_rays(SamplesArgs a) {
+constexpr int kRedLanes = 8;
+constexpr int kRedKeep = 12;
+
+__device__ __forceinline__ double group_sum(double v) {
+#pragma unroll
+    for (int off = kRedLanes / 2; off > 0; off >>= 1) v += __shfl_xor(v, off, kRedLanes);
+    return v;
+}
+
+__device__ __forceinline__ void moving_patch_stats(const double *sA, const double *sW, int P, int lane, double &sw, double &ma, double &va) {
+    sw = 0, ma = 0;
+    for (int i = lane; i < P; i += 64) {
+        sw += sW[i];
+        ma += sW[i] * sA[i];
+    }
+    sw = wave_sum(sw);
+    ma = wave_sum(ma);
+    if (sw > 0.0) ma /= sw;
+    va = 0;
+    for (int i = lane; i < P; i += 64) {
+        const double da = sA[i] - ma;
+        va += sW[i] * da * da;
+    }
+    va = wave_sum(va);
+}
+
+__device__ __forceinline__ void row_load(const double *B, int P, int sub, double (&breg)[kRedKeep]) {
+#pragma unroll
+    for (int k = 0; k < kRedKeep; ++k) breg[k] = (sub + kRedLanes * k < P) ? B[sub + kRedLanes * k] : 0.0;
+}
+
+__device__ __forceinline__ double row_cost(const double *sA, const double *sW, const double *B, const double (&breg)[kRedKeep], int P, int sub,
+                                           int simmeasure, double sw, double ma, double va) {
+    if (simmeasure == 2) {
+        double mb = 0;
+#pragma unroll
+        for (int k = 0; k < kRedKeep; ++k) {
+            const int i = sub + kRedLanes * k;
+            if (i < P) mb += sW[i] * breg[k];
+        }
+        for (int i = sub + kRedLanes * kRedKeep; i < P; i += kRedLanes) mb += sW[i] * B[i];
+        mb = group_sum(mb);
+        if (sw > 0.0) mb /= sw;
+        double pr = 0, vb = 0;
+#pragma unroll
+        for (int k = 0; k < kRedKeep; ++k) {
+            const int i = sub + kRedLanes * k;
+            if (i < P) {
+                const double da = sA[i] - ma, db = breg[k] - mb;
+                pr += sW[i] * da * db;
+                vb += sW[i] * db * db;
+            }
+        }
+        for (int i = sub + kRedLanes * kRedKeep; i < P; i += kRedLanes) {
+            const double da = sA[i] - ma, db = B[i] - mb;
+            pr += sW[i] * da * db;
+            vb += sW[i] * db * db;
+        }
+        pr = group_sum(pr);
+        vb = group_sum(vb);
+        if (sw > 0.0) {
+            pr /= sw;
+            va /= sw;
+            vb /= sw;
+        }
+        const double r = (va == 0.0 || vb == 0.0) ? 0.0 : pr / (sqrt(va) * sqrt(vb));
+        return 1 - (1 + r) * 0.5;
+    }
+    double pr = 0;
+#pragma unroll
+    for (int k = 0; k < kRedKeep; ++k) {
+        const int i = sub + kRedLanes * k;
+        if (i < P) {
+            const double df = sA[i] - breg[k];
+            pr += sW[i] * df * df;
+        }
+    }
+    for (int i = sub + kRedLanes * kRedKeep; i < P; i += kRedLanes) {
+        const double df = sA[i] - B[i];
+        pr += sW[i] * df * df;
+    }
+    pr = group_sum(pr);
+    return sqrt(pr) / P;
+}
+
+template <class Emit>
+__device__ __forceinline__ bool ray_settle(const DevTree &tree, const V3 &p, Emit emit) {
+    int t;
+    float fx = 0.f, fy = 0.f, fz = 0.f;
+    const int4 c = ray_cell_of(tree, p, fx, fy, fz);
+    if (c.x < 0) return false;
+    const float4 *rec = tree.ray_tri + (size_t)kRayPieces * c.x;
+    const float4 e0 = rec[0], e1 = rec[1], e2 = rec[2];
+    const double2 *dv = reinterpret_cast<const double2 *>(rec + 3);
+    double2 d0 = dv[0], d1 = dv[1], d2 = dv[2], d3 = dv[3], d4 = dv[4], d5 = dv[5];
+    t = c.x;
+    bool vouch_needed = __float_as_int(e1.w) >= 0;
+    float4 ev = e1;
+    if (!ray_accepts(e0, e1, e2, fx, fy, fz)) {
+        t = -1;
+        int4 mo = make_int4(c.w, -1, -1, -1);
+        if (c.w < -1) mo = tree.ray_more[-2 - c.w];
+#pragma unroll 1
+        for (int k = 0; k < 6 && t < 0; ++k) {
+            const int ck = k == 0 ? c.y : (k == 1 ? c.z : (k == 2 ? mo.x : (k == 3 ? mo.y : (k == 4 ? mo.z : mo.w))));
+            if (ck < 0) break;
+            const float4 *r2 = tree.ray_tri + (size_t)kRayPieces * ck;
+            const float4 g0 = r2[0], g1 = r2[1], g2 = r2[2];
+            if (ray_accepts(g0, g1, g2, fx, fy, fz)) {
+                t = ck;
+                ev = g1;
+                vouch_needed = __float_as_int(g1.w) >= 0;
+            }
+        }
+        if (t >= 0) {
+            dv = reinterpret_cast<const double2 *>(tree.ray_tri + (size_t)kRayPieces * t + 3);
+            d0 = dv[0], d1 = dv[1], d2 = dv[2], d3 = dv[3], d4 = dv[4], d5 = dv[5];
+        }
+    }
+    if (t >= 0 && vouch_needed && !ray_vouches(tree, ev, p)) t = -1;
+    if (t < 0) return false;
+    double wa, wb, wc;
+    area_weights(mk(d0.x, d0.y, d1.x), mk(d1.y, d2.x, d2.y), mk(d3.x, d3.y, d4.x), p, wa, wb, wc);
+    emit(t, wa, wb, wc, d4.y, d5.x, d5.y);
+    return true;
+}
+
+__device__ __forceinline__ void list_left(bool left, int s, int lane, int *s_nleft, int *sleft) {
+    const unsigned long long bal = __ballot(left);
+    if (bal) {
+        const int leader = __ffsll((long long)bal) - 1;
+        int base = 0;
+        if (lane == leader) base = atomicAdd(s_nleft, __popcll(bal));
+        base = __shfl(base, leader, 64);
+        if (left) sleft[base + __popcll(bal & ((1ull << lane) - 1ull))] = s;
+    }
+}
+
+__global__ __launch_bounds__(256) __attribute__((amdgpu_waves_per_eu(7, 7))) void k_unary_rays(SamplesArgs a) {
+    extern __shared__ __align__(16) double lds[];
+    const int tid = threadIdx.x, lane = tid & 63;
+    if (blockIdx.x == 0)
+        for (int k = tid; k < a.clear_words; k += 256) a.clear_next[k] = 0u;
+    const int per = (a.N + 7) >> 3;
+    const int slots = 8 * per;
+    const int part = blockIdx.x / slots, slot = blockIdx.x - part * slots;
+    const int at = (slot & 7) * per + (slot >> 3);
+    if (at >= a.N) return;
+    const int node = a.order[at];
+    const int lper = (a.L + a.nsplit - 1) / a.nsplit;
+    const int l_beg = part * lper, l_end = min(a.L, l_beg + lper);
+    if (l_beg >= l_end) return;
+    double *sx = lds, *sy = sx + a.pmax, *sz = sy + a.pmax, *sA = sz + a.pmax, *sW = sA + a.pmax, *sR = sW + a.pmax;
+    double *sval = sR + 9 * a.L;
+    int *sleft = reinterpret_cast<int *>(sval + (size_t)lper * a.pmax);
+    int *srow_cnt = sleft + (size_t)lper * a.pmax, *srow_off = srow_cnt + lper, *srow_open = srow_off + lper, *srow_fill = srow_open + lper;
+    const int beg = a.pptr[node], P = a.pptr[node + 1] - beg;
+    const size_t gbase = (size_t)a.L * beg;
+    for (int i = tid; i < P; i += 256) {
+        const int s = a.pidx[beg + i];
+        sx[i] = a.src[s];
+        sy[i] = a.src[a.Nsrc + s];
+        sz[i] = a.src[2 * a.Nsrc + s];
+        sA[i] = a.sfeat[s];
+        sW[i] = a.cfw ? a.cfw[s] : 1.0;
+    }
+    for (int k = 9 * l_beg + tid; k < 9 * l_end; k += 256) sR[k] = a.rnl[(size_t)node * a.L * 9 + k];
+    for (int k = tid; k < 4 * lper; k += 256) srow_cnt[k] = 0;
+    const int sbeg = l_beg * P, send = l_end * P, nrows = l_end - l_beg;
+    const float invP = 1.0f / (float)max(P, 1);
+    __shared__ int s_nleft;
+    __shared__ unsigned s_base, s_rbase;
+    __shared__ double s_stat[3];
+    if (tid == 0) s_nleft = 0;
+    __syncthreads();
+    for (int s0 = sbeg; s0 < send; s0 += 256) {
+        const int s = s0 + tid;
+        const bool act = s < send;
+        bool done = false;
+        if (act) {
+            const int l = fast_div(s, P, invP), i = s - l * P;
+            const V3 p = rotate(sR + 9 * l, mk(sx[i], sy[i], sz[i]));
+            done = ray_settle(a.tree, p, [&](int, double wa, double wb, double wc, double f0, double f1, double f2) { sval[s - sbeg] = wa * f0 + wb * f1 + wc * f2; });
+        }
+        list_left(act && !done, s, lane, &s_nleft, sleft);
+    }
+    __syncthreads();
+    const int nleft = s_nleft;
+    for (int j = tid; j < nleft; j += 256) atomicAdd(&srow_cnt[fast_div(sleft[j], P, invP) - l_beg], 1);
+    if (a.simmeasure == 2 && tid >= 192) {
+        double sw, ma, va;
+        moving_patch_stats(sA, sW, P, lane, sw, ma, va);
+        if (lane == 0) s_stat[0] = sw, s_stat[1] = ma, s_stat[2] = va;
+    }
+    __syncthreads();
+    const int seg = blockIdx.x % kFixSegs;
+    if (nleft > 0 && tid < 64) {
+        int run = 0, run_open = 0;
+        for (int r0 = 0; r0 < nrows; r0 += 64) {
+            const int c = r0 + lane < nrows ? srow_cnt[r0 + lane] : 0, o = c > 0 ? 1 : 0;
+            int incl = c, incl_open = o;
+#pragma unroll
+            for (int off = 1; off < 64; off <<= 1) {
+                const int up = __shfl_up(incl, off, 64), up_open = __shfl_up(incl_open, off, 64);
+                if (lane >= off) incl += up, incl_open += up_open;
+            }
+            if (r0 + lane < nrows) srow_off[r0 + lane] = run + incl - c, srow_open[r0 + lane] = run_open + incl_open - o;
+            run += __shfl(incl, 63, 64);
+            run_open += __shfl(incl_open, 63, 64);
+        }
+        if (lane == 0) {
+            unsigned long long *cnt = reinterpret_cast<unsigned long long *>(a.fix_cnt + kCntStride * (1 + seg));
+            const unsigned long long old = atomicAdd(cnt, ((unsigned long long)run_open << 32) | (unsigned)nleft);
+            s_base = a.fix_off[seg] + (unsigned)old;
+            s_rbase = a.row_off[seg] + (unsigned)(old >> 32);
+        }
+    }
+    __syncthreads();
+    if (nleft > 0) {
+        const unsigned base = s_base, end = a.fix_off[seg + 1];
+        for (int j = tid; j < nleft; j += 256) {
+            const int s = sleft[j];
+            const int l = fast_div(s, P, invP), i = s - l * P;
+            const unsigned at_slot = base + srow_off[l - l_beg] + atomicAdd(&srow_fill[l - l_beg], 1);
+            if (at_slot < end) {
+                const V3 p = rotate(sR + 9 * l, mk(sx[i], sy[i], sz[i]));
+                a.fix_list[at_slot] = gbase + (unsigned long long)s;
+                a.fix_pt[3 * (size_t)at_slot] = p.x;
+                a.fix_pt[3 * (size_t)at_slot + 1] = p.y;
+                a.fix_pt[3 * (size_t)at_slot + 2] = p.z;
+            } else {
+                raise_status(a.status, MSM_ERR_CAPACITY);
+            }
+        }
+    }
+    const int sub = tid & (kRedLanes - 1), grp = tid / kRedLanes;
+    const double absw = a.absw[node];
+    double sw = 0, ma = 0, va = 0;
+    if (a.simmeasure == 2) sw = s_stat[0], ma = s_stat[1], va = s_stat[2];
+    for (int r = grp; r < nrows; r += 256 / kRedLanes) {
+        const int l = l_beg + r, cnt = srow_cnt[r];
+        const double *B = sval + (size_t)r * P;
+        if (cnt == 0) {
+            double breg[kRedKeep];
+            row_load(B, P, sub, breg);
+            const double cost = row_cost(sA, sW, B, breg, P, sub, a.simmeasure, sw, ma, va);
+            if (sub == 0) a.U[(size_t)l * a.N + node] = absw * cost;
+        } else {
+            double *out = a.tval + gbase + (size_t)l * P;
+            for (int i = sub; i < P; i += kRedLanes) out[i] = B[i];
+            if (sub == 0) {
+                const unsigned at_row = s_rbase + srow_open[r];
+                if (at_row < a.row_off[seg + 1]) a.row_list[at_row] = make_uint4((unsigned)node, (unsigned)l, s_base + srow_off[r], (unsigned)cnt);
+                else raise_status(a.status, MSM_ERR_CAPACITY);
+            }
+        }
+    }
+}
+
+__global__ __launch_bounds__(256) void k_unary_rays_stored(SamplesArgs a) {
     extern __shared__ __align__(16) double lds[];
     double *sx = lds, *sy = sx + a.pmax, *sz = sy + a.pmax, *sR = sz + a.pmax;
     const int tid = threadIdx.x, lane = tid & 63;
@@ -355,70 +619,22 @@
         const int s = s0 + tid;
         const bool act = s < send;
         bool done = false;
-        V3 p = mk(0.0, 0.0, 0.0);
-        float fx = 0.f, fy = 0.f, fz = 0.f;
-        int4 c = make_int4(-1, -1, -1, -1);
         if (act) {
             const int l = fast_div(s, P, invP), i = s - l * P;
-            p = rotate(sR + 9 * l, mk(sx[i], sy[i], sz[i]));
-            c = ray_cell_of(a.tree, p, fx, fy, fz);
-        }
-        if (act) {
-            if (c.x >= 0) {
-                const float4 *rec = a.tree.ray_tri + (size_t)kRayPieces * c.x;
-                const float4 e0 = rec[0], e1 = rec[1], e2 = rec[2];
-                const double2 *dv = reinterpret_cast<const double2 *>(rec + 3);
-                double2 d0 = dv[0], d1 = dv[1], d2 = dv[2], d3 = dv[3], d4 = dv[4], d5 = dv[5];
-                int t = c.x;
-                bool vouch_needed = __float_as_int(e1.w) >= 0;
-                float4 ev = e1;
-                if (!ray_accepts(e0, e1, e2, fx, fy, fz)) {
-                    t = -1;
-                    int4 mo = make_int4(c.w, -1, -1, -1);
-                    if (c.w < -1) mo = a.tree.ray_more[-2 - c.w];
-#pragma unroll 1
-                    for (int k = 0; k < 6 && t < 0; ++k) {
-                        const int ck = k == 0 ? c.y : (k == 1 ? c.z : (k == 2 ? mo.x : (k == 3 ? mo.y : (k == 4 ? mo.z : mo.w))));
-                        if (ck < 0) break;
-                        const float4 *r2 = a.tree.ray_tri + (size_t)kRayPieces * ck;
-                        const float4 g0 = r2[0], g1 = r2[1], g2 = r2[2];
-                        if (ray_accepts(g0, g1, g2, fx, fy, fz)) {
-                            t = ck;
-                            ev = g1;
-                            vouch_needed = __float_as_int(g1.w) >= 0;
-                        }
-                    }
-                    if (t >= 0) {
-                        dv = reinterpret_cast<const double2 *>(a.tree.ray_tri + (size_t)kRayPieces * t + 3);
-                        d0 = dv[0], d1 = dv[1], d2 = dv[2], d3 = dv[3], d4 = dv[4], d5 = dv[5];
-                    }
+            const V3 p = rotate(sR + 9 * l, mk(sx[i], sy[i], sz[i]));
+            done = ray_settle(a.tree, p, [&](int t, double wa, double wb, double wc, double f0, double f1, double f2) {
+                const size_t g = gbase + s;
+                if (a.tval) {
+                    a.tval[g] = wa * f0 + wb * f1 + wc * f2;
+                } else {
+                    a.stri[g] = t;
+                    a.sw3[3 * g] = wa;
+                    a.sw3[3 * g + 1] = wb;
+                    a.sw3[3 * g + 2] = wc;
                 }
-                if (t >= 0 && vouch_needed && !ray_vouches(a.tree, ev, p)) t = -1;
-                if (t >= 0) {
-                    double wa, wb, wc;
-                    area_weights(mk(d0.x, d0.y, d1.x), mk(d1.y, d2.x, d2.y), mk(d3.x, d3.y, d4.x), p, wa, wb, wc);
-                    const size_t g = gbase + s;
-                    if (a.tval) {
-                        a.tval[g] = wa * d4.y + wb * d5.x + wc * d5.y;
-                    } else {
-                        a.stri[g] = t;
-                        a.sw3[3 * g] = wa;
-                        a.sw3[3 * g + 1] = wb;
-                        a.sw3[3 * g + 2] = wc;
-                    }
-                    done = true;
-                }
-            }
-        }
-        const bool left = act && !done;
-        const unsigned long long bal = __ballot(left);
-        if (bal) {
-            const int leader = __ffsll((long long)bal) - 1;
-            int base = 0;
-            if (lane == leader) base = atomicAdd(&s_nleft, __popcll(bal));
-            base = __shfl(base, leader, 64);
-            if (left) sleft[base + __popcll(bal & ((1ull << lane) - 1ull))] = s;
-        }
+            });
+        }
+        list_left(act && !done, s, lane, &s_nleft, sleft);
     }
     __syncthreads();
     const int nleft = s_nleft;
@@ -484,6 +700,75 @@
     }
 }
 
+__global__ __launch_bounds__(256) void k_unary_finish(SamplesArgs a) {
+    extern __shared__ __align__(16) double lds[];
+    __shared__ unsigned s_pre[kFixSegs + 1];
+    if (threadIdx.x < kFixSegs) {
+        const int seg = threadIdx.x;
+        const unsigned cnt = min(a.fix_cnt[kCntStride * (1 + seg) + 1], a.row_off[seg + 1] - a.row_off[seg]);
+        unsigned incl = cnt, listed = min(a.fix_cnt[kCntStride * (1 + seg)], a.fix_off[seg + 1] - a.fix_off[seg]);
+#pragma unroll
+        for (int off = 1; off < 64; off <<= 1) {
+            const unsigned up = __shfl_up(incl, off, 64);
+            if (seg >= off) incl += up;
+        }
+#pragma unroll
+        for (int off = 32; off > 0; off >>= 1) listed += __shfl_xor(listed, off, 64);
+        s_pre[seg + 1] = incl;
+        if (seg == 0) s_pre[0] = 0;
+        if (blockIdx.x == 0 && seg == kFixSegs - 1) a.row_stats[0] = incl, a.row_stats[1] = listed;
+    }
+    __syncthreads();
+    const unsigned n = s_pre[kFixSegs];
+    const int lane = threadIdx.x & 63, wave = threadIdx.x >> 6, sub = lane & 7, grp = lane >> 3;
+    double *sA = lds + 3 * (size_t)a.pmax * wave, *sW = sA + a.pmax, *sB = sW + a.pmax;
+    const double nan = __longlong_as_double(0x7ff8000000000000ll);
+    for (unsigned j = blockIdx.x * 4 + wave; j < n; j += gridDim.x * 4) {
+        int seg = 0;
+#pragma unroll
+        for (int step = kFixSegs / 2; step > 0; step >>= 1)
+            if (s_pre[seg + step] <= j) seg += step;
+        const uint4 row = a.row_list[a.row_off[seg] + (j - s_pre[seg])];
+        const int node = (int)row.x, l = (int)row.y, cnt = (int)row.w;
+        const int beg = a.pptr[node], P = a.pptr[node + 1] - beg;
+        const size_t g0 = (size_t)a.L * beg + (size_t)l * P;
+        for (int i = lane; i < P; i += 64) {
+            const int s = a.pidx[beg + i];
+            sA[i] = a.sfeat[s];
+            sW[i] = a.cfw ? a.cfw[s] : 1.0;
+            sB[i] = a.tval[g0 + i];
+        }
+        for (int k0 = 0; k0 < cnt; k0 += 8) {
+            const bool valid = k0 + grp < cnt;
+            V3 p = mk(0.0, 0.0, 0.0);
+            size_t g = 0;
+            if (valid) {
+                const size_t at_slot = (size_t)row.z + k0 + grp;
+                g = (size_t)a.fix_list[at_slot];
+                p = mk(a.fix_pt[3 * at_slot], a.fix_pt[3 * at_slot + 1], a.fix_pt[3 * at_slot + 2]);
+            }
+            const int found = group8_find(a.tree, valid, p, lane);
+            if (valid && sub == 0) {
+                const int t = found == kGroupUndecided ? find_closest_triangle(a.tree, p) : found;
+                double v = nan;
+                if (t < 0) emit_failure(a, g, t);
+                else v = emit_sample(a, g, p, t);
+                sB[g - g0] = v;
+            }
+        }
+        __builtin_amdgcn_wave_barrier();
+        double sw = 0, ma = 0, va = 0;
+        if (a.simmeasure == 2) moving_patch_stats(sA, sW, P, lane, sw, ma, va);
+        if (grp == 0) {
+            double breg[kRedKeep];
+            row_load(sB, P, sub, breg);
+            const double cost = row_cost(sA, sW, sB, breg, P, sub, a.simmeasure, sw, ma, va);
+            if (sub == 0) a.U[(size_t)l * a.N + node] = a.absw[node] * cost;
+        }
+        __builtin_amdgcn_wave_barrier();
+    }
+}
+
 struct ReduceArgs {
     int N, L, Nsrc;
     const double *sfeat;
@@ -523,15 +808,6 @@
     }
 }
 
-constexpr int kRedLanes = 8;
-constexpr int kRedKeep = 12;
-
-__device__ __forceinline__ double group_sum(double v) {
-#pragma unroll
-    for (int off = kRedLanes / 2; off > 0; off >>= 1) v += __shfl_xor(v, off, kRedLanes);
-    return v;
-}
-
 __global__ __launch_bounds__(256) void k_unary_reduce_flat(ReduceArgs a, unsigned int *clear, int clear_words) {
     extern __shared__ __align__(16) double lds[];
     double *sA = lds, *sW = sA + a.pmax;
@@ -548,8 +824,7 @@
     for (int k = 0; k < kRedKeep; ++k) breg[k] = 0.0;
     if (grp < a.L) {
         const double *B = a.tval + (size_t)a.L * beg + (size_t)grp * P;
-#pragma unroll
-        for (int k = 0; k < kRedKeep; ++k) breg[k] = (sub + kRedLanes * k < P) ? B[sub + kRedLanes * k] : 0.0;
+        row_load(B, P, sub, breg);
     }
     for (int i = tid; i < P; i += 256) {
         const int s = a.pidx[beg + i];
@@ -559,20 +834,8 @@
     __syncthreads();
     if (a.simmeasure == 2) {
         if (tid < 64) {
-            double sw = 0, ma = 0;
-            for (int i = tid; i < P; i += 64) {
-                sw += sW[i];
-                ma += sW[i] * sA[i];
-            }
-            sw = wave_sum(sw);
-            ma = wave_sum(ma);
-            if (sw > 0.0) ma /= sw;
-            double va = 0;
-            for (int i = tid; i < P; i += 64) {
-                const double da = sA[i] - ma;
-                va += sW[i] * da * da;
-            }
-            va = wave_sum(va);
+            double sw, ma, va;
+            moving_patch_stats(sA, sW, P, tid, sw, ma, va);
             if (tid == 0) s_stat[0] = sw, s_stat[1] = ma, s_stat[2] = va;
         }
         __syncthreads();
@@ -580,64 +843,10 @@
     const double absw = a.absw[node];
     for (int l = grp; l < a.L; l += 256 / kRedLanes) {
         const double *B = a.tval + (size_t)a.L * beg + (size_t)l * P;
-        if (!(in_regs && l == grp)) {
-#pragma unroll
-            for (int k = 0; k < kRedKeep; ++k) breg[k] = (sub + kRedLanes * k < P) ? B[sub + kRedLanes * k] : 0.0;
-        }
-        double cost;
-        if (a.simmeasure == 2) {
-            const double sw = s_stat[0], ma = s_stat[1];
-            double mb = 0;
-#pragma unroll
-            for (int k = 0; k < kRedKeep; ++k) {
-                const int i = sub + kRedLanes * k;
-                if (i < P) mb += sW[i] * breg[k];
-            }
-            for (int i = sub + kRedLanes * kRedKeep; i < P; i += kRedLanes) mb += sW[i] * B[i];
-            mb = group_sum(mb);
-            if (sw > 0.0) mb /= sw;
-            double pr = 0, vb = 0;
-#pragma unroll
-            for (int k = 0; k < kRedKeep; ++k) {
-                const int i = sub + kRedLanes * k;
-                if (i < P) {
-                    const double da = sA[i] - ma, db = breg[k] - mb;
-                    pr += sW[i] * da * db;
-                    vb += sW[i] * db * db;
-                }
-            }
-            for (int i = sub + kRedLanes * kRedKeep; i < P; i += kRedLanes) {
-                const double da = sA[i] - ma, db = B[i] - mb;
-                pr += sW[i] * da * db;
-                vb += sW[i] * db * db;
-            }
-            pr = group_sum(pr);
-            vb = group_sum(vb);
-            double va = s_stat[2];
-            if (sw > 0.0) {
-                pr /= sw;
-                va /= sw;
-                vb /= sw;
-            }
-            const double r = (va == 0.0 || vb == 0.0) ? 0.0 : pr / (sqrt(va) * sqrt(vb));
-            cost = 1 - (1 + r) * 0.5;
-        } else {
-            double pr = 0;
-#pragma unroll
-            for (int k = 0; k < kRedKeep; ++k) {
-                const int i = sub + kRedLanes * k;
-                if (i < P) {
-                    const double df = sA[i] - breg[k];
-                    pr += sW[i] * df * df;
-                }
-            }
-            for (int i = sub + kRedLanes * kRedKeep; i < P; i += kRedLanes) {
-                const double df = sA[i] - B[i];
-                pr += sW[i] * df * df;
-            }
-            pr = group_sum(pr);
-            cost = sqrt(pr) / P;
-        }
+        if (!(in_regs && l == grp)) row_load(B, P, sub, breg);
+        double sw = 0, ma = 0, va = 0;
+        if (a.simmeasure == 2) sw = s_stat[0], ma = s_stat[1], va = s_stat[2];
+        const double cost = row_cost(sA, sW, B, breg, P, sub, a.simmeasure, sw, ma, va);
         if (sub == 0) a.U[(size_t)l * a.N + node] = absw * cost;
     }
 }
@@ -951,10 +1160,10 @@
 }
 int unary_fix_segments() { return kFixSegs; }
 size_t unary_fix_counter_words() { return (size_t)kCntStride * (1 + kFixSegs); }
-void unary_fix_offsets(int N, int L, int pmax, const int32_t *pptr, const int32_t *order, std::vector<uint32_t> &off) {
+void unary_fix_offsets(int N, int L, int pmax, const int32_t *pptr, const int32_t *order, std::vector<uint32_t> &off, std::vector<uint32_t> *row_off) {
     const int nsplit = unary_nsplit(L, pmax), per = (N + 7) >> 3, slots = 8 * per;
     const int lper = (L + nsplit - 1) / nsplit;
-    std::vector<uint64_t> size(kFixSegs, 0);
+    std::vector<uint64_t> size(kFixSegs, 0), rows(kFixSegs, 0);
     for (int b = 0; b < nsplit * slots; ++b) {
         const int part = b / slots, slot = b - part * slots;
         const int at = (slot & 7) * per + (slot >> 3);
@@ -963,14 +1172,27 @@
         const int l_beg = part * lper, l_end = std::min(L, l_beg + lper);
         if (l_beg >= l_end) continue;
         size[b % kFixSegs] += (uint64_t)(l_end - l_beg) * (pptr[node + 1] - pptr[node]);
+        rows[b % kFixSegs] += (uint64_t)(l_end - l_beg);
     }
     off.assign(kFixSegs + 1, 0);
     for (int s = 0; s < kFixSegs; ++s) off[s + 1] = (uint32_t)std::min<uint64_t>(0xffffffffull, off[s] + size[s]);
-}
+    if (row_off) {
+        row_off->assign(kFixSegs + 1, 0);
+        for (int s = 0; s < kFixSegs; ++s) (*row_off)[s + 1] = (uint32_t)((*row_off)[s] + rows[s]);
+    }
+}
+
+static size_t rays_rows_lds(int pmax, int L, int nsplit) {
+    const size_t lper = (size_t)(L + nsplit - 1) / nsplit;
+    return sizeof(double) * (5 * (size_t)pmax + 9 * (size_t)L + lper * pmax) + sizeof(int) * (lper * pmax + 4 * lper);
+}
+static size_t finish_lds(int pmax) { return sizeof(double) * 3 * (size_t)pmax * 4; }
+static bool rows_fit_in_lds(int pmax, int L, int nsplit) { return rays_rows_lds(pmax, L, nsplit) <= 64 * 1024 && finish_lds(pmax) <= 64 * 1024; }
 
 static bool uses_ray_table(const DevTree &t) { return t.simple && t.ray_G > 0 && t.ray_cell && t.ray_tri; }
 
-static int launch_samples(msm_ctx *ctx, const UnaryLaunch &u, const UnaryWeightsScratch *w, SamplesArgs &a, bool fused_reduction = false) {
+static int launch_samples(msm_ctx *ctx, const UnaryLaunch &u, const UnaryWeightsScratch *w, SamplesArgs &a, bool fused_reduction = false,
+                          bool rows_in_sampler = false, bool *rows_done = nullptr) {
     if (u.tree.nnodes <= 0 || !u.tree.mask) return fail(MSM_ERR_STATE, "target search structure missing");
     a.tree = u.tree;
     a.tfeat = u.tfeat;
@@ -989,8 +1211,15 @@
     a.sw3 = w ? w->sw3 : nullptr;
     a.fix_list = u.fix_list;
     a.fix_pt = u.fix_pt;
-    a.fix_cnt = u.fix_cnt;
+    const size_t cnt_words = unary_fix_counter_words();
+    const int set = u.fix_set ? *u.fix_set : 0;
+    a.fix_cnt = u.fix_cnt + cnt_words * set;
     a.fix_off = u.fix_off;
+    a.row_list = u.row_list;
+    a.row_off = u.row_off;
+    a.row_stats = u.row_stats;
+    a.clear_next = u.fix_cnt + cnt_words * (1 - set);
+    a.clear_words = (int)cnt_words;
     a.sfeat = u.sfeat;
     a.cfw = (u.cfw && u.cfw_rows >= 1) ? u.cfw : nullptr;
     a.absw = u.absw;
@@ -998,7 +1227,7 @@
     a.percentile = u.percentile;
     a.U = (w || !fused_reduction) ? nullptr : u.U;
     a.redo_list = u.redo_list;
-    a.redo_count = u.fix_cnt;
+    a.redo_count = a.fix_cnt;
     a.status = ctx->d_status;
     if (u.ntri >= (1 << kTriBits)) return fail(MSM_ERR_CAPACITY, "target mesh has %d triangles; the sample queue packs ids in %d bits", u.ntri, kTriBits);
     a.nsplit = unary_nsplit(u.L, u.pmax);
@@ -1009,12 +1238,23 @@
     }
     const int blocks = a.nsplit * 8 * ((u.N + 7) / 8);
     if (u.ev_start) MSM_HIP(hipEventRecord(u.ev_start, ctx->stream));
+    if (uses_ray_table(u.tree) && rows_in_sampler && !w && u.fix_set && u.row_list && rows_fit_in_lds(u.pmax, u.L, a.nsplit)) {
+        a.U = u.U;
+        hipLaunchKernelGGL(k_unary_rays, dim3(blocks), dim3(256), rays_rows_lds(u.pmax, u.L, a.nsplit), ctx->stream, a);
+        MSM_HIP(hipGetLastError());
+        if (u.ev_stop) MSM_HIP(hipEventRecord(u.ev_stop, ctx->stream));
+        hipLaunchKernelGGL(k_unary_finish, dim3(1024), dim3(256), finish_lds(u.pmax), ctx->stream, a);
+        MSM_HIP(hipGetLastError());
+        *u.fix_set = 1 - set;
+        if (rows_done) *rows_done = true;
+        return MSM_OK;
+    }
     if (uses_ray_table(u.tree)) {
         a.U = nullptr;
         const int lper = (u.L + a.nsplit - 1) / a.nsplit;
         const size_t rays_lds = sizeof(double) * (3 * (size_t)u.pmax + 9 * (size_t)u.L) + sizeof(int) * ((size_t)lper * u.pmax + 4) + 16;
-        if (rays_lds > 64 * 1024) MSM_HIP(hipFuncSetAttribute(reinterpret_cast<const void *>(k_unary_rays), hipFuncAttributeMaxDynamicSharedMemorySize, (int)rays_lds));
-        hipLaunchKernelGGL(k_unary_rays, dim3(blocks), dim3(256), rays_lds, ctx->stream, a);
+        if (rays_lds > 64 * 1024) MSM_HIP(hipFuncSetAttribute(reinterpret_cast<const void *>(k_unary_rays_stored), hipFuncAttributeMaxDynamicSharedMemorySize, (int)rays_lds));
+        hipLaunchKernelGGL(k_unary_rays_stored, dim3(blocks), dim3(256), rays_lds, ctx->stream, a);
     } else {
         hipLaunchKernelGGL(k_unary_samples, dim3(blocks), dim3(256), lds, ctx->stream, a);
     }
@@ -1028,8 +1268,14 @@
 int launch_unary_univariate(msm_ctx *ctx, const UnaryLaunch &u) {
     SamplesArgs a;
     const bool dice = u.simmeasure == 4 || u.simmeasure == 5;
-    int st = launch_samples(ctx, u, nullptr, a, dice);
+    bool rows_done = false;
+    if (u.rows_fused) *u.rows_fused = false;
+    int st = launch_samples(ctx, u, nullptr, a, dice, !dice, &rows_done);
     if (st) return st;
+    if (rows_done) {
+        if (u.rows_fused) *u.rows_fused = true;
+        return MSM_OK;
+    }
     ReduceArgs r;
     r.N = u.N;
     r.L = u.L;
@@ -1046,19 +1292,19 @@
     r.percentile = u.percentile;
     r.U = u.U;
     r.redo_list = u.redo_list;
-    r.redo_count = u.fix_cnt;
+    r.redo_count = a.fix_cnt;
     if (uses_ray_table(u.tree) && dice) {
         r.redo_list = nullptr;
         r.redo_count = nullptr;
         hipLaunchKernelGGL(k_unary_reduce_univariate, dim3(std::min(u.N, 2048)), dim3(256), sizeof(double) * 2 * (size_t)u.pmax, ctx->stream, r);
-        MSM_HIP(hipMemsetAsync(u.fix_cnt, 0, unary_fix_counter_words() * sizeof(unsigned), ctx->stream));
+        MSM_HIP(hipMemsetAsync(a.fix_cnt, 0, unary_fix_counter_words() * sizeof(unsigned), ctx->stream));
     } else if (!dice) {
         r.redo_list = u.order;
-        hipLaunchKernelGGL(k_unary_reduce_flat, dim3(u.N), dim3(256), sizeof(double) * 2 * (size_t)u.pmax, ctx->stream, r, u.fix_cnt,
+        hipLaunchKernelGGL(k_unary_reduce_flat, dim3(u.N), dim3(256), sizeof(double) * 2 * (size_t)u.pmax, ctx->stream, r, a.fix_cnt,
                            (int)unary_fix_counter_words());
     } else {
         hipLaunchKernelGGL(k_unary_reduce_univariate, dim3(64), dim3(256), sizeof(double) * 2 * (size_t)u.pmax, ctx->stream, r);
-        MSM_HIP(hipMemsetAsync(u.fix_cnt, 0, unary_fix_counter_words() * sizeof(unsigned), ctx->stream));
+        MSM_HIP(hipMemsetAsync(a.fix_cnt, 0, unary_fix_counter_words() * sizeof(unsigned), ctx->stream));
     }
     MSM_HIP(hipGetLastError());
     return MSM_OK;
@@ -1117,7 +1363,7 @@
         hipLaunchKernelGGL(k_unary_reduce_features, dim3(u.N), dim3(threads), flds, ctx->stream, r);
     }
     MSM_HIP(hipGetLastError());
-    MSM_HIP(hipMemsetAsync(u.fix_cnt, 0, unary_fix_counter_words() * sizeof(unsigned), ctx->stream));
+    MSM_HIP(hipMemsetAsync(a.fix_cnt, 0, unary_fix_counter_words() * sizeof(unsigned), ctx->stream));
     return MSM_OK;
 }
 
```

Measured after the change: 336.4 million evals/s. 0.953x the previous value.
